# mourisl/T1K

Hardware: AMD Instinct MI355X
Metric: genotyped reads/sec (end-to-end genotyper stage, 2x150 bp HLA) (higher is better)
Workload: dtype u64

## Files before the change

include/t1k_gpu.h:

```cpp
#ifndef T1K_GPU_H
#define T1K_GPU_H

#include <stddef.h>
#include <stdint.h>

#ifdef __cplusplus
extern "C" {
#endif

typedef enum {
  T1K_OK = 0,
  T1K_ERR_ARG = -1,
  T1K_ERR_DEVICE = -2,
  T1K_ERR_CAPACITY = -3,
  T1K_ERR_IO = -4,
  T1K_ERR_STATE = -5,
  T1K_ERR_INTERNAL = -6,
  T1K_ERR_COMMITTED = -7
} t1k_status;

typedef struct t1k_ctx t1k_ctx;
typedef struct t1k_job t1k_job;
typedef struct t1k_rowset t1k_rowset;
typedef struct t1k_comm t1k_comm;
// ... 108 lines not shown
const char *t1k_readset_last_error(const t1k_readset *rs);
void t1k_readset_destroy(t1k_readset *rs);
int t1k_coverage_selected(t1k_ctx *ctx, t1k_readset *rs, const uint8_t *selected, uint64_t *nRecords);
typedef struct t1k_xwin t1k_xwin;
int t1k_xwin_create(t1k_ctx *owner, uint64_t maxReadEnds, uint32_t maxWindows, t1k_xwin **out);
void t1k_xwin_destroy(t1k_xwin *x);
const char *t1k_xwin_last_error(const t1k_xwin *x);
int t1k_xwin_link(t1k_xwin *x, t1k_ctx *reader, uint32_t window, uint32_t *nExternal);
int t1k_xwin_resolve(t1k_xwin *x, t1k_ctx *ctx, uint32_t window);

int t1k_ref_share(t1k_ctx *dst, const t1k_ctx *src);
uint64_t t1k_pool_release(void);
void *t1k_pinned_alloc(uint64_t bytes);
void t1k_pinned_free(void *p);
int t1k_reads_share(t1k_ctx *dst, const t1k_ctx *src);
int t1k_reads_attach(t1k_ctx *dst, const t1k_ctx *src, int storeSlot, int resetStore);
int t1k_coverage_absorb(t1k_ctx *dst, t1k_ctx *src);

int t1k_extract_batch(t1k_ctx *ctx, uint32_t endsPerFragment, uint8_t *good, uint64_t *stats);

int t1k_align_count_batch(t1k_ctx *ctx, const char *text, const uint32_t *tOff, const char *pat, const uint32_t *pOff, const uint32_t *len, uint32_t nJobs,
                          int32_t *nMatch);
int t1k_gap_count_batch(t1k_ctx *ctx, const char *text, const uint32_t *tOff, const uint32_t *tLen, const char *pat, const uint32_t *pOff,
                        const uint32_t *pLen, uint32_t nJobs, int32_t *nMatch);
int t1k_align_batch(t1k_ctx *ctx, const char *text, const uint32_t *tOff, const uint32_t *tLen, const char *pat, const uint32_t *pOff,
                    const uint32_t *pLen, uint32_t nJobs, int32_t *score, int32_t *nMatch, int32_t *nMismatch, int32_t *nIndel, int8_t *ops,
                    const uint32_t *opsOff, uint32_t *nOps);

typedef void (*t1k_allreduce_fn)(void *dev_f64, uint64_t n, void *user);
int t1k_em_setup(t1k_ctx *ctx, const uint64_t *rowPtr, const uint32_t *ecIdx, const double *count, const int32_t *ecLen, uint32_t nGroups,
                 uint32_t nEc, t1k_allreduce_fn allreduce, void *user);
int t1k_em_update(t1k_ctx *ctx, const double *x0, double *x1, double *ecReadCount, double *diff);
void t1k_em_limits(uint32_t out[2]);

int t1k_barcode_em(t1k_ctx *ctx, uint32_t nBarcodes, const uint64_t *bcAllelePtr, const uint32_t *bcAllele, const uint64_t *bcGroupPtr,
                   const double *groupCount, const uint64_t *groupEntryPtr, const uint32_t *entryLocal, const double *rho, uint32_t nAlleles,
                   double alpha, double tol, int32_t maxIter, double *nOut, int32_t *itersOut, double *kernelMs);

typedef struct {
  uint64_t distinct;
  uint64_t keys;
  uint64_t corrected;
  uint64_t split;
  uint64_t no_umi;
  double kernel_ms;
} t1k_umi_stats;
int t1k_umi_collapse(t1k_ctx *ctx, uint32_t nFrag, const uint32_t *fragRow, const uint64_t *fragUmi, const uint64_t *listPtr, const uint32_t *listAllele,
                     uint32_t nRows, const uint32_t *alleleGene, uint32_t nAlleles, uint32_t nGenes, int32_t mismatch, uint32_t *fragMol, uint32_t *nMol,
                     uint32_t *molRow, uint32_t *molFrags, uint64_t *molListPtr, uint32_t *molList, double *frac, int32_t *uniq, t1k_umi_stats *stats);

typedef struct {
  uint32_t allele, seq_start;
  uint64_t read_at, ops_at;
  uint32_t n_ops, w_all, w_uniq, reserved;
} t1k_pileup_aln;
int t1k_pileup_begin(t1k_ctx *ctx, uint32_t nAlleles, const uint64_t *alleleOff );
int t1k_pileup_add(t1k_ctx *ctx, const t1k_pileup_aln *aln, uint32_t n, const char *text, uint64_t textBytes, const int8_t *ops, uint64_t opsBytes,
                   double *kernelMs);
int t1k_pileup_get(t1k_ctx *ctx, int32_t *counts );
int t1k_pileup_end(t1k_ctx *ctx);

int t1k_sitepile_begin(t1k_ctx *ctx, uint32_t nAlleles, const uint64_t *alleleOff , uint64_t nSites, const uint32_t *siteAllele, const uint32_t *sitePos,
                       uint64_t nBarcodes);
int t1k_sitepile_add(t1k_ctx *ctx, const t1k_pileup_aln *aln, uint32_t n, const uint64_t *bookPtr , const uint32_t *book, const char *text, uint64_t textBytes,
                     const int8_t *ops, uint64_t opsBytes, double *kernelMs);
int t1k_sitepile_get(t1k_ctx *ctx, uint64_t *keys, int32_t *counts, uint64_t cap, uint64_t *nRuns);
int t1k_sitepile_stats(t1k_ctx *ctx, uint64_t *keysEmitted, uint64_t *folds, double *foldMs);
int t1k_sitepile_end(t1k_ctx *ctx);

int t1k_phase_begin(t1k_ctx *ctx, uint32_t nAlleles, const uint64_t *alleleOff , uint64_t nSites, const uint32_t *siteAllele, const uint32_t *sitePos);
int t1k_phase_add(t1k_ctx *ctx, const t1k_pileup_aln *aln, uint32_t n, uint32_t nBook, const uint32_t *bookRec , const uint8_t *bookUniq ,
                  const char *text, uint64_t textBytes, const int8_t *ops, uint64_t opsBytes, double *kernelMs);
int t1k_phase_get(t1k_ctx *ctx, uint64_t *keys, int32_t *counts, uint64_t cap, uint64_t *nRuns);
int t1k_phase_stats(t1k_ctx *ctx, uint64_t *observations, uint64_t *bookings, uint64_t *keysEmitted, uint64_t *discordant, uint64_t *folds, double *foldMs);
int t1k_phase_end(t1k_ctx *ctx);

typedef struct { uint32_t read_len, clip_front, strand; } t1k_support_rec;
typedef struct { uint32_t flags, t_start, t_end; } t1k_support_book;
int t1k_support_begin(t1k_ctx *ctx, uint32_t nAlleles, const uint64_t *alleleOff , uint64_t nSites, const uint32_t *siteAllele, const uint32_t *sitePos);
int t1k_support_add(t1k_ctx *ctx, const t1k_pileup_aln *aln, uint32_t n, const t1k_support_rec *rec , const uint64_t *bookPtr ,
                    const t1k_support_book *book, const char *text, uint64_t textBytes, const int8_t *ops, uint64_t opsBytes, double *kernelMs);
int t1k_support_get(t1k_ctx *ctx, uint64_t *keys, int32_t *counts, uint64_t cap, uint64_t *nRuns);
int t1k_support_stats(t1k_ctx *ctx, uint64_t *keysEmitted, uint64_t *folds, double *foldMs);
int t1k_support_end(t1k_ctx *ctx);

int t1k_indel_begin(t1k_ctx *ctx, uint32_t nAlleles, const uint64_t *alleleOff , const char *alleleText );
int t1k_indel_add(t1k_ctx *ctx, const t1k_pileup_aln *aln, uint32_t n, const uint8_t *strand , const uint64_t *bookPtr , const uint8_t *bookUniq,
                  const char *text, uint64_t textBytes, const int8_t *ops, uint64_t opsBytes, double *kernelMs);
int t1k_indel_get(t1k_ctx *ctx, uint64_t *keys, int32_t *counts, uint64_t cap, uint64_t *nRuns);
int t1k_indel_stats(t1k_ctx *ctx, uint64_t *events, uint64_t *shifted, uint64_t *edgeDelBooked, uint64_t *edgeInsBooked, uint64_t *keysEmitted, uint64_t *folds, double *foldMs);
int t1k_indel_end(t1k_ctx *ctx);

int t1k_cigar_batch(t1k_ctx *ctx, const t1k_pileup_aln *aln, uint32_t n, const uint32_t *clip ,
                    const int8_t *ops, uint64_t opsBytes, uint32_t nAlleles, const uint64_t *alleleOff , const char *alleleText ,
                    uint64_t *cigarPtr , char *cigar, uint64_t cigarCap, uint64_t *mdPtr , char *md, uint64_t mdCap,
                    uint32_t *nm , uint32_t *refSpan , double *kernelMs );

int t1k_alt_batch(t1k_ctx *ctx, uint64_t nGroups, const uint64_t *groupPtr , const uint32_t *entryAllele, const uint64_t *q , uint32_t nAlleles,
                  const uint32_t *alleleGene , uint32_t nGenes, const uint32_t *slotOf , uint64_t *tables , double *kernelMs );
uint64_t t1k_alt_pieces(uint64_t nGroups, const uint64_t *groupPtr);

int t1k_diplo_batch(t1k_ctx *ctx, uint64_t nGroups, const uint64_t *groupPtr , const uint32_t *entryCand, const uint64_t *q , uint32_t nGenes,
                    const uint32_t *candPtr , uint64_t *matrix, double *kernelMs );
uint64_t t1k_diplo_pieces(uint64_t nGroups, const uint64_t *groupPtr);

typedef struct {
  uint64_t read_ends, lookups, postings, hits, groups, candidates, extended, near_best, dp_calls, rows, batches;
  double ms_seed, ms_chain, ms_extend, ms_select, ms_fullalign, ms_pair, ms_em, ms_total;
  uint64_t read_ends_total, pair_overlaps, dp_cells;
  double ms_load, ms_device, ms_coalesce, ms_write;
} t1k_stats;
int t1k_stats_get(t1k_ctx *ctx, t1k_stats *out);

enum { T1K_ROUTE_GENERAL_LANE = 0,
       T1K_ROUTE_WAVE_SMALL = 1,
       T1K_ROUTE_WAVE_LARGE = 2,
       T1K_ROUTE_BIG_BY_SIZE = 3,
       T1K_ROUTE_BIG_BY_SCRATCH = 4,
       T1K_ROUTE_KINDS = 5 };
typedef struct {
  uint64_t ranges, ranges_nw5, ranges_nw10, ranges_xlong;
  uint64_t groups, fast, slow, jobs, retry, finish, general, wave, genjobs, big, eq, band, wide, extjobs, extretry;
} t1k_route_totals;
typedef struct {
  uint32_t read_end, allele, n;
  uint8_t strand;
  uint8_t near_done, simple;
  uint8_t route;
  uint8_t nw, xlong, reserved[2];
} t1k_route_rec;
int t1k_route_report_enable(t1k_ctx *ctx, int on);
int t1k_route_report_get(t1k_ctx *ctx, t1k_route_totals *totals , t1k_route_rec *recs , uint64_t cap, uint64_t *nRecs);

#define T1K_SEED_MASK_WORDS 10
typedef struct {
  uint32_t read_off, list_len;
  uint8_t strand, reserved[3];
} t1k_seed_used;
int t1k_seed_report_enable(t1k_ctx *ctx, int on);
int t1k_seed_report_get(t1k_ctx *ctx, uint8_t *seen, uint32_t *counts, uint32_t *masks, t1k_seed_used *used, uint64_t cap, uint64_t *nUsed);

enum { T1K_REF_BASES = 0, T1K_REF_NMASK, T1K_REF_EXON, T1K_REF_POSTED, T1K_REF_BASES_T, T1K_REF_BLOCK_T, T1K_REF_ALLELE_OFF, T1K_REF_ALLELE_LEN,
       T1K_REF_ALLELE_HAS_N, T1K_REF_SEP_START, T1K_REF_SEP_POS, T1K_REF_K_START, T1K_REF_K_HAS, T1K_REF_K_MULTI, T1K_REF_K_HAS_PRE,
       T1K_REF_K_DIR_IDX, T1K_REF_K_DIR, T1K_REF_K_DIR_MASK, T1K_REF_K_POST, T1K_REF_K_POST_ALLELE, T1K_REF_ARRAYS };
typedef struct {
  uint32_t n_alleles, k;
  uint64_t total_bases, n_words, n_postings, bases_t_len, n_sep;
  uint32_t dir_rows, dir_stride, dir_mask_words, has_bases_t;
  uint64_t len[T1K_REF_ARRAYS];
  uint32_t elem_bytes[T1K_REF_ARRAYS];
} t1k_ref_geometry;
int t1k_ref_view_geometry(t1k_ctx *ctx, t1k_ref_geometry *out);
int t1k_ref_view_copy(t1k_ctx *ctx, int array, uint64_t first, uint64_t count, void *out);

double t1k_alloc_ms(t1k_ctx *ctx, uint64_t *bytes);
uint64_t t1k_ctx_mem_report(t1k_ctx *ctx, const char *tag, int print);

int t1k_genotyper_main(int argc, char **argv);
int t1k_extractor_main(int argc, char **argv);
int t1k_bam_extractor_main(int argc, char **argv);
int t1k_analyzer_main(int argc, char **argv);

typedef struct {
  t1k_params dev;
  double filter_frac, filter_cov, cross_gene_rate, squarem_min_alpha;
  int32_t allele_digit_units;
  char allele_delimiter;
  int32_t threads;
  int32_t device;
  int32_t output_read_assignment;
  int32_t batch_fragments;
  int32_t alternatives;
  int32_t diplotypes;
  int32_t diplo_candidates;
} t1k_job_params;
void t1k_job_params_default(t1k_job_params *p);

int t1k_job_create(const t1k_job_params *p, const char *refFasta, t1k_job **out);
void t1k_job_destroy(t1k_job *job);
const char *t1k_job_last_error(const t1k_job *job);
int t1k_job_load_reads(t1k_job *job, const char *file1, const char *file2, const char *barcodeFile);
int t1k_job_load_reads_multi(t1k_job *job, const char *const *files1, uint32_t n1, const char *const *files2, uint32_t n2, const char *barcodeFile);
typedef struct t1k_reads t1k_reads;
int t1k_reads_open(const char *const *files1, uint32_t n1, const char *const *files2, uint32_t n2, const char *barcodeFile, int threads, t1k_reads **out);
int t1k_reads_open_stream(const char *const *files1, uint32_t n1, const char *const *files2, uint32_t n2, const char *barcodeFile, int threads, t1k_reads **out);
const char *t1k_reads_last_error(const t1k_reads *reads);
int t1k_reads_fragments(const t1k_reads *reads, uint64_t *nFragments);
void t1k_reads_close(t1k_reads *reads);
int t1k_job_attach_reads(t1k_job *job, t1k_reads *reads);
int t1k_job_set_reads(t1k_job *job, const char *seq1, const uint64_t *off1, const char *seq2, const uint64_t *off2, uint32_t nFragments);
int t1k_job_run(t1k_job *job);
int t1k_job_set_output_prefix(t1k_job *job, const char *prefix);
int t1k_job_write_outputs(t1k_job *job, const char *prefix);
int t1k_job_genotype_text(t1k_job *job, char *buf, uint64_t cap, uint64_t *needed);
int t1k_job_alternatives_text(t1k_job *job, char *buf, uint64_t cap, uint64_t *needed);
int t1k_job_diplotypes_text(t1k_job *job, char *buf, uint64_t cap, uint64_t *needed);
int t1k_job_allele_table(t1k_job *job, int32_t *gene, double *abundance, uint32_t *nAlleles);
int t1k_job_counts(t1k_job *job, uint64_t *fragments, uint64_t *assignedFragments, uint64_t *groups, uint64_t *ecs, int32_t *emIterations);
int t1k_job_stats(t1k_job *job, t1k_stats *out);
t1k_ctx *t1k_job_ctx(t1k_job *job);
int t1k_job_set_shard(t1k_job *job, int rank, int nRanks, t1k_comm *comm);
int t1k_job_share_reads(t1k_job *dst, t1k_job *src);
int t1k_job_run_local(t1k_job *job);
int t1k_job_finish(t1k_job *job);
int t1k_job_groups_serialize(t1k_job *job, void *buf, uint64_t cap, uint64_t *needed);
int t1k_job_groups_merge(t1k_job *job, const void *const *bufs, const uint64_t *lens, uint32_t n);
int t1k_job_coalesce_rows(t1k_job *job, const t1k_row_entry *rows, const uint32_t *rowCounts, const uint32_t *fragments, uint32_t nFragments);
int t1k_coverage_device(t1k_ctx *ctx, void **devPtr, uint64_t *count);

typedef struct {
  int32_t allele_idx;
  int32_t has_mate_pair, o1_from_r2;
  t1k_overlap o1, o2;
  uint64_t ops1, ops2;
  uint32_t n_ops1, n_ops2;
} t1k_frag_assignment;
int t1k_fragment_details(const t1k_overlap *l1, uint32_t n1, const t1k_overlap *l2, uint32_t n2, int paired, const int32_t *alleles, uint32_t nAlleles,
                         t1k_frag_assignment *out);
typedef struct {
  int32_t allele_idx, ref_pos, exon_pos;
  char ref, var;
  int32_t qual, group, output_group;
  double var_support, all_support, var_uniq_support;
} t1k_variant;
typedef struct t1k_variants t1k_variants;
int t1k_variants_call(t1k_job *job, const double *abundance, int32_t var_max_group, uint32_t nFragments, const uint64_t *asgPtr, const t1k_frag_assignment *asg,
                      const int8_t *ops, const char *const *read1, const uint32_t *len1, const char *const *read2, const uint32_t *len2, t1k_variants **out);
uint32_t t1k_variants_count(const t1k_variants *v);
int t1k_variants_get(const t1k_variants *v, t1k_variant *out );
int t1k_variants_vcf(const t1k_variants *v, char *buf, uint64_t cap, uint64_t *needed);
int t1k_variants_adjust(const t1k_variants *v, const t1k_frag_assignment *asg, uint32_t n, const int8_t *ops, const char *read1, uint32_t len1, const char *read2, uint32_t len2,
                        uint8_t *keep);
void t1k_variants_destroy(t1k_variants *v);

#ifdef __cplusplus
}
#endif
#endif
```

t1k_amd/capi.py:

```python
import ctypes as C
import gzip
import os

import numpy as np

_HERE = os.path.dirname(os.path.abspath(__file__))


def lib_path():
    return os.environ.get("T1K_GPU_LIB") or os.path.join(_HERE, "lib", "libt1k_gpu.so")


class T1kError(RuntimeError):
    pass


class Params(C.Structure):
    _fields_ = [("kmer_length", C.c_int32), ("radius", C.c_int32), ("hit_len_required", C.c_int32),
                ("ref_seq_similarity", C.c_double), ("relax_intron_align", C.c_int32), ("max_assign_cnt", C.c_int32),
                ("max_read_len", C.c_int32), ("workgroups", C.c_int32), ("group_cap", C.c_int64),
                ("cand_cap", C.c_int64), ("ovl_cap", C.c_int64), ("row_cap", C.c_int64), ("n_base_code", C.c_int32), ("store_chunk_mb", C.c_int32)]


class JobParams(C.Structure):
    _fields_ = [("dev", Params), ("filter_frac", C.c_double), ("filter_cov", C.c_double),
                ("cross_gene_rate", C.c_double), ("squarem_min_alpha", C.c_double), ("allele_digit_units", C.c_int32),
                ("allele_delimiter", C.c_char), ("threads", C.c_int32), ("device", C.c_int32),
                ("output_read_assignment", C.c_int32), ("batch_fragments", C.c_int32), ("alternatives", C.c_int32),
                ("diplotypes", C.c_int32), ("diplo_candidates", C.c_int32)]


class Stats(C.Structure):
    _fields_ = [(n, C.c_uint64) for n in ("read_ends", "lookups", "postings", "hits", "groups", "candidates", "extended",
                                          "near_best", "dp_calls", "rows", "batches")] + \
               [(n, C.c_double) for n in ("ms_seed", "ms_chain", "ms_extend", "ms_select", "ms_fullalign", "ms_pair", "ms_em", "ms_total")] + \
               [(n, C.c_uint64) for n in ("read_ends_total", "pair_overlaps", "dp_cells")] + \
               [(n, C.c_double) for n in ("ms_load", "ms_device", "ms_coalesce", "ms_write")]

    def as_dict(self):
        return {n: getattr(self, n) for n, _ in self._fields_}


class UmiStats(C.Structure):
    _fields_ = [(n, C.c_uint64) for n in ("distinct", "keys", "corrected", "split", "no_umi")] + [("kernel_ms", C.c_double)]


OVERLAP_DTYPE = np.dtype([("seq_idx", "<i4"), ("read_start", "<i4"), ("read_end", "<i4"), ("seq_start", "<i4"),
                          ("seq_end", "<i4"), ("strand", "<i4"), ("match_cnt", "<i4"), ("left_clip", "<i4"),
                          ("right_clip", "<i4"), ("relaxed_match_cnt", "<i4"), ("similarity", "<f8")])
ROW_DTYPE = np.dtype([("allele_idx", "<i4"), ("start", "<i4"), ("end", "<i4"), ("weight", "<f4"), ("qual", "<f4"),
                      ("adjust_weight", "<f4")])
GROUP_DTYPE = np.dtype([("allele", "<i4"), ("start", "<i4"), ("end", "<i4"), ("weight", "<f4"), ("adjust_weight", "<f4")])
assert OVERLAP_DTYPE.itemsize == 48 and ROW_DTYPE.itemsize == 24 and GROUP_DTYPE.itemsize == 20
FRAG_ASG_DTYPE = np.dtype([("allele_idx", "<i4"), ("has_mate_pair", "<i4"), ("o1_from_r2", "<i4"), ("_pad", "<i4"), ("o1", OVERLAP_DTYPE), ("o2", OVERLAP_DTYPE),
                           ("ops1", "<u8"), ("ops2", "<u8"), ("n_ops1", "<u4"), ("n_ops2", "<u4")])
VARIANT_DTYPE = np.dtype([("allele_idx", "<i4"), ("ref_pos", "<i4"), ("exon_pos", "<i4"), ("ref", "S1"), ("var", "S1"), ("_pad", "S2"), ("qual", "<i4"), ("group", "<i4"),
                          ("output_group", "<i4"), ("_pad2", "<i4"), ("var_support", "<f8"), ("all_support", "<f8"), ("var_uniq_support", "<f8")])
assert FRAG_ASG_DTYPE.itemsize == 136 and VARIANT_DTYPE.itemsize == 56

PILEUP_ALN_DTYPE = np.dtype([("allele", "<u4"), ("seq_start", "<u4"), ("read_at", "<u8"), ("ops_at", "<u8"), ("n_ops", "<u4"), ("w_all", "<u4"), ("w_uniq", "<u4"),
                             ("reserved", "<u4")])
PHASE_NO_MATE = 0xFFFFFFFF
PHASE_STATES = ("A", "C", "G", "T", "N", "-")
PILEUP_COUNTERS = ("A", "C", "G", "T", "N", "del", "ins", "A_uniq", "C_uniq", "G_uniq", "T_uniq", "N_uniq", "del_uniq", "ins_uniq")
assert PILEUP_ALN_DTYPE.itemsize == 40
SUPPORT_REC_DTYPE = np.dtype([("read_len", "<u4"), ("clip_front", "<u4"), ("strand", "<u4")])
SUPPORT_BOOK_DTYPE = np.dtype([("flags", "<u4"), ("t_start", "<u4"), ("t_end", "<u4")])
SUPPORT_STATES = ("A", "C", "G", "T", "N", "-", "+")
SUPPORT_FAMILY_B = 1 << 57
assert SUPPORT_REC_DTYPE.itemsize == 12 and SUPPORT_BOOK_DTYPE.itemsize == 12
ROUTE_TOTALS = ("ranges", "ranges_nw5", "ranges_nw10", "ranges_xlong", "groups", "fast", "slow", "jobs", "retry", "finish", "general", "wave", "genjobs", "big",
                "eq", "band", "wide", "extjobs", "extretry")
ROUTE_REC_DTYPE = np.dtype([("read_end", "<u4"), ("allele", "<u4"), ("n", "<u4"), ("strand", "u1"), ("near_done", "u1"), ("simple", "u1"), ("route", "u1"),
                            ("nw", "u1"), ("xlong", "u1"), ("reserved", "u1", (2,))])
ROUTE_NAMES = ("general_lane", "wave_small", "wave_large", "big_by_size", "big_by_scratch")
assert ROUTE_REC_DTYPE.itemsize == 20
SEED_USED_DTYPE = np.dtype([("read_off", "<u4"), ("list_len", "<u4"), ("strand", "u1"), ("reserved", "u1", (3,))])
SEED_MASK_WORDS = 10
assert SEED_USED_DTYPE.itemsize == 12
POSTING_DTYPE = np.dtype([("allele", "<u4"), ("offset", "<u4")])
REF_ARRAYS = (("bases", "<u8"), ("nmask", "<u8"), ("exon", "<u8"), ("posted", "<u8"), ("basesT", "<u8"), ("blockT", "<u4"), ("alleleOff", "<u8"), ("alleleLen", "<u4"),
              ("alleleHasN", "u1"), ("sepStart", "<u4"), ("sepPos", "<i4"), ("kStart", "<u4"), ("kHas", "<u4"), ("kMulti", "<u4"), ("kHasPre", "<u4"), ("kDirIdx", "<u4"),
              ("kDir", "<u4"), ("kDirMask", "<u8"), ("kPost", POSTING_DTYPE), ("kPostAllele", "<u4"))


class RefGeometry(C.Structure):
    _fields_ = [("n_alleles", C.c_uint32), ("k", C.c_uint32), ("total_bases", C.c_uint64), ("n_words", C.c_uint64), ("n_postings", C.c_uint64),
                ("bases_t_len", C.c_uint64), ("n_sep", C.c_uint64), ("dir_rows", C.c_uint32), ("dir_stride", C.c_uint32), ("dir_mask_words", C.c_uint32),
                ("has_bases_t", C.c_uint32), ("len", C.c_uint64 * len(REF_ARRAYS)), ("elem_bytes", C.c_uint32 * len(REF_ARRAYS))]


CIGAR_FILL = 0xAB
ALT_FILL = 0xCD
ALT_EMPTY = 0xFFFFFFFF
DIPLO_FILL = 0xD1

ALLREDUCE_FN = C.CFUNCTYPE(None, C.c_void_p, C.c_uint64, C.c_void_p)

_lib = None


def lib():
    global _lib
    if _lib is not None:
        return _lib
    p = lib_path()
    if not os.path.exists(p):
        raise T1kError("%s not found: run `python -c 'import __graft_entry__ as g; g.build()'` first" % p)
    L = C.CDLL(p)
    vp, u64p, u32p, u8p, i32p = C.c_void_p, C.POINTER(C.c_uint64), C.POINTER(C.c_uint32), C.POINTER(C.c_uint8), C.POINTER(C.c_int32)
    L.t1k_params_default.argtypes = [C.POINTER(Params)]
    L.t1k_ctx_create.argtypes = [C.c_int, C.POINTER(Params), C.POINTER(vp)]
    L.t1k_ctx_destroy.argtypes = [vp]
    L.t1k_last_error.argtypes = [vp]
    L.t1k_last_error.restype = C.c_char_p
    L.t1k_device_count.restype = C.c_int
    L.t1k_ref_upload.argtypes = [vp, C.c_char_p, vp, vp, C.c_uint32]
    L.t1k_reads_upload.argtypes = [vp, C.c_char_p, vp, vp, C.c_uint32]
    L.t1k_assign_batch.argtypes = [vp]
    L.t1k_assign_range.argtypes = [vp, C.c_uint64, C.c_uint32]
    L.t1k_overlaps_download.argtypes = [vp, vp, vp, C.c_uint64, u64p]
    L.t1k_pair_batch.argtypes = [vp, vp, vp, vp, C.c_uint32]
    L.t1k_rows_download.argtypes = [vp, vp, vp, vp, C.c_uint64, u64p]
    L.t1k_coverage_get.argtypes = [vp, vp, C.c_uint64]
    L.t1k_coverage_reset.argtypes = [vp]
    L.t1k_missing_coverage.argtypes = [vp, vp]
    L.t1k_coverage_absorb.argtypes = [vp, vp]
    L.t1k_align_batch.argtypes = [vp, C.c_char_p, vp, vp, C.c_char_p, vp, vp, C.c_uint32, vp, vp, vp, vp, vp, vp, vp]
    L.t1k_align_count_batch.argtypes = [vp, C.c_char_p, vp, C.c_char_p, vp, vp, C.c_uint32, vp]
    L.t1k_gap_count_batch.argtypes = [vp, C.c_char_p, vp, vp, C.c_char_p, vp, vp, C.c_uint32, vp]
    L.t1k_em_setup.argtypes = [vp, vp, vp, vp, vp, C.c_uint32, C.c_uint32, ALLREDUCE_FN, vp]
    L.t1k_em_update.argtypes = [vp, vp, vp, vp, vp]
    L.t1k_em_shard.argtypes = [vp, C.c_uint32, C.c_uint32, vp]
    L.t1k_em_limits.argtypes = [vp]
    L.t1k_em_limits.restype = None
    L.t1k_barcode_em.argtypes = [vp, C.c_uint32, vp, vp, vp, vp, vp, vp, vp, C.c_uint32, C.c_double, C.c_double, C.c_int32, vp, vp, C.POINTER(C.c_double)]
    L.t1k_umi_collapse.argtypes = [vp, C.c_uint32, vp, vp, vp, vp, C.c_uint32, vp, C.c_uint32, C.c_uint32, C.c_int32, vp, C.POINTER(C.c_uint32), vp, vp, vp, vp, vp, vp,
                                   C.POINTER(UmiStats)]
    L.t1k_pileup_begin.argtypes = [vp, C.c_uint32, vp]
    L.t1k_pileup_add.argtypes = [vp, vp, C.c_uint32, vp, C.c_uint64, vp, C.c_uint64, C.POINTER(C.c_double)]
    L.t1k_pileup_get.argtypes = [vp, vp]
    L.t1k_pileup_end.argtypes = [vp]
    L.t1k_sitepile_begin.argtypes = [vp, C.c_uint32, vp, C.c_uint64, vp, vp, C.c_uint64]
    L.t1k_sitepile_add.argtypes = [vp, vp, C.c_uint32, vp, vp, vp, C.c_uint64, vp, C.c_uint64, C.POINTER(C.c_double)]
    L.t1k_sitepile_get.argtypes = [vp, vp, vp, C.c_uint64, u64p]
    L.t1k_sitepile_stats.argtypes = [vp, u64p, u64p, C.POINTER(C.c_double)]
    L.t1k_sitepile_end.argtypes = [vp]
    L.t1k_support_begin.argtypes = [vp, C.c_uint32, vp, C.c_uint64, vp, vp]
    L.t1k_support_add.argtypes = [vp, vp, C.c_uint32, vp, vp, vp, vp, C.c_uint64, vp, C.c_uint64, C.POINTER(C.c_double)]
    L.t1k_support_get.argtypes = [vp, vp, vp, C.c_uint64, u64p]
    L.t1k_support_stats.argtypes = [vp, u64p, u64p, C.POINTER(C.c_double)]
    L.t1k_support_end.argtypes = [vp]
    L.t1k_indel_begin.argtypes = [vp, C.c_uint32, vp, vp]
    L.t1k_indel_add.argtypes = [vp, vp, C.c_uint32, vp, vp, vp, vp, C.c_uint64, vp, C.c_uint64, C.POINTER(C.c_double)]
    L.t1k_indel_get.argtypes = [vp, vp, vp, C.c_uint64, u64p]
    L.t1k_indel_stats.argtypes = [vp, u64p, u64p, u64p, u64p, u64p, u64p, C.POINTER(C.c_double)]
    L.t1k_indel_end.argtypes = [vp]
    L.t1k_phase_begin.argtypes = [vp, C.c_uint32, vp, C.c_uint64, vp, vp]
    L.t1k_phase_add.argtypes = [vp, vp, C.c_uint32, C.c_uint32, vp, vp, vp, C.c_uint64, vp, C.c_uint64, C.POINTER(C.c_double)]
    L.t1k_phase_get.argtypes = [vp, vp, vp, C.c_uint64, u64p]
    L.t1k_phase_stats.argtypes = [vp, u64p, u64p, u64p, u64p, u64p, C.POINTER(C.c_double)]
    L.t1k_phase_end.argtypes = [vp]
    L.t1k_cigar_batch.argtypes = [vp, vp, C.c_uint32, vp, vp, C.c_uint64, C.c_uint32, vp, vp, vp, vp, C.c_uint64, vp, vp, C.c_uint64, vp, vp, C.POINTER(C.c_double)]
    L.t1k_alt_batch.argtypes = [vp, C.c_uint64, vp, vp, vp, C.c_uint32, vp, C.c_uint32, vp, vp, C.POINTER(C.c_double)]
    L.t1k_ctx_mem_report.argtypes = [vp, C.c_char_p, C.c_int]
    L.t1k_ctx_mem_report.restype = C.c_uint64
    L.t1k_alt_pieces.argtypes = [C.c_uint64, vp]
    L.t1k_alt_pieces.restype = C.c_uint64
    L.t1k_job_alternatives_text.argtypes = [vp, C.c_char_p, C.c_uint64, u64p]
    L.t1k_diplo_batch.argtypes = [vp, C.c_uint64, vp, vp, vp, C.c_uint32, vp, vp, C.POINTER(C.c_double)]
    L.t1k_diplo_pieces.argtypes = [C.c_uint64, vp]
    L.t1k_diplo_pieces.restype = C.c_uint64
    L.t1k_job_diplotypes_text.argtypes = [vp, C.c_char_p, C.c_uint64, u64p]
    L.t1k_job_allele_table.argtypes = [vp, vp, vp, u32p]
    L.t1k_extract_batch.argtypes = [vp, C.c_uint32, vp, vp]
    L.t1k_extractor_main.argtypes = [C.c_int, C.POINTER(C.c_char_p)]
    L.t1k_stats_get.argtypes = [vp, C.POINTER(Stats)]
    L.t1k_route_report_enable.argtypes = [vp, C.c_int]
    L.t1k_route_report_get.argtypes = [vp, vp, vp, C.c_uint64, u64p]
    L.t1k_seed_report_enable.argtypes = [vp, C.c_int]
    L.t1k_seed_report_get.argtypes = [vp, vp, vp, vp, vp, C.c_uint64, u64p]
    L.t1k_ref_view_geometry.argtypes = [vp, vp]
    L.t1k_ref_view_copy.argtypes = [vp, C.c_int, C.c_uint64, C.c_uint64, vp]
    L.t1k_genotyper_main.argtypes = [C.c_int, C.POINTER(C.c_char_p)]
    L.t1k_job_params_default.argtypes = [C.POINTER(JobParams)]
    L.t1k_job_create.argtypes = [C.POINTER(JobParams), C.c_char_p, C.POINTER(vp)]
    L.t1k_job_destroy.argtypes = [vp]
    L.t1k_job_last_error.argtypes = [vp]
    L.t1k_job_last_error.restype = C.c_char_p
    L.t1k_job_load_reads.argtypes = [vp, C.c_char_p, C.c_char_p, C.c_char_p]
    L.t1k_job_set_reads.argtypes = [vp, C.c_char_p, vp, C.c_char_p, vp, C.c_uint32]
    L.t1k_job_run.argtypes = [vp]
    L.t1k_job_write_outputs.argtypes = [vp, C.c_char_p]
    L.t1k_pool_release.restype = C.c_uint64
    L.t1k_pool_release.argtypes = []
    L.t1k_job_load_reads_multi.argtypes = [vp, C.POINTER(C.c_char_p), C.c_uint32, C.POINTER(C.c_char_p), C.c_uint32, C.c_char_p]
    L.t1k_reads_open.argtypes = [C.POINTER(C.c_char_p), C.c_uint32, C.POINTER(C.c_char_p), C.c_uint32, C.c_char_p, C.c_int, C.POINTER(vp)]
    L.t1k_reads_open_stream.argtypes = [C.POINTER(C.c_char_p), C.c_uint32, C.POINTER(C.c_char_p), C.c_uint32, C.c_char_p, C.c_int, C.POINTER(vp)]
    L.t1k_reads_last_error.argtypes = [vp]
    L.t1k_reads_last_error.restype = C.c_char_p
    L.t1k_reads_fragments.argtypes = [vp, u64p]
    L.t1k_reads_close.argtypes = [vp]
    L.t1k_reads_close.restype = None
    L.t1k_job_attach_reads.argtypes = [vp, vp]
    L.t1k_job_genotype_text.argtypes = [vp, C.c_char_p, C.c_uint64, u64p]
    L.t1k_job_counts.argtypes = [vp, u64p, u64p, u64p, u64p, i32p]
    L.t1k_job_stats.argtypes = [vp, C.POINTER(Stats)]
    L.t1k_job_ctx.argtypes = [vp]
    L.t1k_job_ctx.restype = vp
    L.t1k_job_run_local.argtypes = [vp]
    L.t1k_job_finish.argtypes = [vp]
    L.t1k_job_groups_serialize.argtypes = [vp, vp, C.c_uint64, u64p]
    L.t1k_reads_dedupe.argtypes = [vp, vp, u32p]
    L.t1k_job_groups_merge.argtypes = [vp, vp, vp, C.c_uint32]
    L.t1k_job_coalesce_rows.argtypes = [vp, vp, vp, vp, C.c_uint32]
    L.t1k_variants_call.argtypes = [vp, vp, C.c_int32, C.c_uint32, vp, vp, vp, vp, vp, vp, vp, C.POINTER(vp)]
    L.t1k_fragment_details.argtypes = [vp, C.c_uint32, vp, C.c_uint32, C.c_int, vp, C.c_uint32, vp]
    L.t1k_variants_count.argtypes = [vp]
    L.t1k_variants_count.restype = C.c_uint32
    L.t1k_variants_get.argtypes = [vp, vp]
    L.t1k_variants_vcf.argtypes = [vp, vp, C.c_uint64, u64p]
    L.t1k_variants_adjust.argtypes = [vp, vp, C.c_uint32, vp, C.c_char_p, C.c_uint32, C.c_char_p, C.c_uint32, vp]
    L.t1k_variants_destroy.argtypes = [vp]
    L.t1k_job_set_shard.argtypes = [vp, C.c_int, C.c_int, vp]
    L.t1k_job_share_reads.argtypes = [vp, vp]
    L.t1k_job_ctx.restype = vp
    L.t1k_job_ctx.argtypes = [vp]
    L.t1k_comm_unique_id.argtypes = [vp]
    L.t1k_comm_init.argtypes = [vp, C.c_int, C.c_int, vp, vp, C.c_int, C.POINTER(vp)]
    L.t1k_comm_bind.argtypes = [vp, vp]
    L.t1k_comm_destroy.argtypes = [vp]
    L.t1k_comm_last_error.restype = C.c_char_p
    L.t1k_comm_last_error.argtypes = [vp]
    L.t1k_comm_is_rccl.argtypes = [vp]
    L.t1k_comm_group_create.restype = vp
    L.t1k_comm_group_create.argtypes = [C.c_int]
    L.t1k_comm_group_destroy.argtypes = [vp]
    L.t1k_coverage_device.argtypes = [vp, C.POINTER(vp), u64p]
    L.t1k_device_memory.argtypes = [C.c_int, u64p, u64p]
    L.t1k_ctx_set_coverage_mode.argtypes = [vp, C.c_int]
    L.t1k_readset_detach.argtypes = [vp, C.POINTER(vp)]
    L.t1k_readset_take_store.argtypes = [vp, vp, C.c_int]
    L.t1k_readset_bytes.argtypes = [vp]
    L.t1k_readset_bytes.restype = C.c_uint64
    L.t1k_readset_size.argtypes = [vp]
    L.t1k_readset_size.restype = C.c_uint32
    L.t1k_readset_destroy.argtypes = [vp]
    L.t1k_coverage_selected.argtypes = [vp, vp, vp, u64p]
    L.t1k_overlaps_upload.argtypes = [vp, vp, vp]
    L.t1k_pair_limits.argtypes = [vp]
    L.t1k_pair_limits.restype = None
    L.t1k_pair_direct_cap.argtypes = []
    L.t1k_pair_direct_cap.restype = C.c_uint32
    L.t1k_rowset_create.argtypes = [vp, C.c_uint64, vp, C.POINTER(vp)]
    L.t1k_rowset_destroy.argtypes = [vp]
    L.t1k_rowset_destroy.restype = None
    L.t1k_rowset_set_raw.argtypes = [vp, C.c_int]
    L.t1k_rowset_last_error.argtypes = [vp]
    L.t1k_rowset_last_error.restype = C.c_char_p
    L.t1k_pair_into.argtypes = [vp, vp, vp, vp, vp, C.c_uint32, C.c_uint64]
    L.t1k_rowset_rows_download.argtypes = [vp, C.c_uint64, C.c_uint32, vp, vp, C.c_uint64, u64p]
    L.t1k_rowset_assigned_range.argtypes = [vp, C.c_uint64, C.c_uint64, vp]
    L.t1k_rowset_coalesce.argtypes = [vp, u64p, u64p, u64p]
    L.t1k_rowset_groups_download.argtypes = [vp, vp, vp, vp]
    L.t1k_rowset_device_bytes.argtypes = [vp, u64p, u64p]
    L.t1k_coalesce_limits.argtypes = [vp]
    L.t1k_coalesce_limits.restype = None
    L.t1k_rowset_exchange.argtypes = [vp, vp, C.c_uint64]
    L.t1k_rowset_groups_gather.argtypes = [vp, vp, u64p, u64p, u64p]
    L.t1k_rowset_groups_download_all.argtypes = [vp, vp, vp, vp]
    L.t1k_comm_abort.argtypes = [vp]
    L.t1k_ref_share.argtypes = [vp, vp]
    L.t1k_reads_share.argtypes = [vp, vp]
    L.t1k_xwin_create.argtypes = [vp, C.c_uint64, C.c_uint32, C.POINTER(vp)]
    L.t1k_xwin_destroy.argtypes = [vp]
    L.t1k_xwin_destroy.restype = None
    L.t1k_xwin_last_error.argtypes = [vp]
    L.t1k_xwin_last_error.restype = C.c_char_p
    L.t1k_xwin_link.argtypes = [vp, vp, C.c_uint32, u32p]
    L.t1k_xwin_resolve.argtypes = [vp, vp, C.c_uint32]
    _lib = L
    return L


def _ptr(a):
    return a.ctypes.data_as(C.c_void_p) if a is not None else None


def _u8(text):
    return np.frombuffer(text, np.uint8) if isinstance(text, (bytes, bytearray)) else np.ascontiguousarray(text, np.uint8)


def _pieces(cuts, n):
    edges = [0] + [int(c) for c in cuts] + [int(n)]
    return zip(edges[:-1], edges[1:])


def _concat(seqs):
    offs = np.zeros(len(seqs) + 1, dtype=np.uint64)
    if len(seqs):
        offs[1:] = np.cumsum([len(s) for s in seqs], dtype=np.uint64)
    blob = "".join(seqs).encode("ascii")
    return blob, offs


class Context:

    def __init__(self, device=0, **kw):
        L = lib()
        p = Params()
        L.t1k_params_default(C.byref(p))
        for k, v in kw.items():
            setattr(p, k, v)
        self.params = p
        h = C.c_void_p()
        rc = L.t1k_ctx_create(device, C.byref(p), C.byref(h))
        if rc != 0:
            raise T1kError("t1k_ctx_create failed (%d): no usable GPU / bad parameters" % rc)
        self.h = h
        self.n_read_ends = 0
        self.allele_len = None

    def _check(self, rc, what):
        if rc != 0:
            raise T1kError("%s failed (%d): %s" % (what, rc, lib().t1k_last_error(self.h).decode()))

    def close(self):
        if self.h:
            lib().t1k_ctx_destroy(self.h)
            self.h = None

    def __del__(self):
        try:
            self.close()
        except Exception:
            pass

    def ref_upload(self, seqs, exon_masks=None):
        blob, offs = _concat(seqs)
        ex = None
        if exon_masks is not None:
            ex = np.concatenate([np.asarray(m, dtype=np.uint8) for m in exon_masks]) if len(seqs) else np.zeros(0, np.uint8)
        self.allele_len = np.array([len(s) for s in seqs], dtype=np.int64)
        self._check(lib().t1k_ref_upload(self.h, blob, _ptr(offs), _ptr(ex), len(seqs)), "t1k_ref_upload")

    def ref_share(self, src):
        self.allele_len = src.allele_len
        self._check(lib().t1k_ref_share(self.h, src.h), "t1k_ref_share")

    def reads_share(self, src):
        self.n_read_ends = src.n_read_ends
        self._check(lib().t1k_reads_share(self.h, src.h), "t1k_reads_share")

    def reads_upload(self, seqs, weights=None):
        blob, offs = _concat(seqs)
        w = None if weights is None else np.asarray(weights, dtype=np.uint32)
        self.n_read_ends = len(seqs)
        self._check(lib().t1k_reads_upload(self.h, blob, _ptr(offs), _ptr(w), len(seqs)), "t1k_reads_upload")

    def reads_dedupe(self):
        out = np.zeros(self.n_read_ends, dtype=np.uint32)
        nd = C.c_uint32()
        self._check(lib().t1k_reads_dedupe(self.h, _ptr(out), C.byref(nd)), "t1k_reads_dedupe")
        self.n_uploaded, self.n_read_ends = self.n_read_ends, nd.value
        return out

    def assign(self):
        self._check(lib().t1k_assign_batch(self.h), "t1k_assign_batch")

    def extract(self, ends_per_fragment=1):
        good = np.zeros(self.n_read_ends // ends_per_fragment, dtype=np.uint8)
        st = np.zeros(8, dtype=np.uint64)
        self._check(lib().t1k_extract_batch(self.h, ends_per_fragment, _ptr(good), _ptr(st)), "t1k_extract_batch")
        return good, dict(zip(("read_ends", "lookups", "postings", "read_ends_with_hits", "read_ends_chained", "screen_ns", "main_ns", "big_shape"), (int(x) for x in st)))

    def overlaps(self):
        n = self.n_read_ends
        counts = np.zeros(n, dtype=np.uint32)
        tot = C.c_uint64()
        self._check(lib().t1k_overlaps_download(self.h, _ptr(counts), None, 0, C.byref(tot)), "t1k_overlaps_download")
        out = np.zeros(tot.value, dtype=OVERLAP_DTYPE)
        self._check(lib().t1k_overlaps_download(self.h, _ptr(counts), _ptr(out), tot.value, C.byref(tot)), "t1k_overlaps_download")
        return counts, out

    def overlaps_upload(self, counts, ovl):
        c = np.ascontiguousarray(counts, dtype=np.uint32)
        o = np.ascontiguousarray(ovl, dtype=OVERLAP_DTYPE)
        assert len(c) == self.n_read_ends and int(c.sum()) == len(o)
        self._check(lib().t1k_overlaps_upload(self.h, _ptr(c), _ptr(o)), "t1k_overlaps_upload")

    def pair(self, end1, end2, has_n):
        e1 = np.asarray(end1, dtype=np.uint32)
        e2 = None if end2 is None else np.asarray(end2, dtype=np.uint32)
        hn = np.asarray(has_n, dtype=np.uint8)
        self.n_fragments = len(e1)
        self._check(lib().t1k_pair_batch(self.h, _ptr(e1), _ptr(e2), _ptr(hn), len(e1)), "t1k_pair_batch")

    def rows(self):
        n = self.n_fragments
        counts = np.zeros(n, dtype=np.uint32)
        assigned = np.zeros(n, dtype=np.uint8)
        tot = C.c_uint64()
        self._check(lib().t1k_rows_download(self.h, _ptr(counts), _ptr(assigned), None, 0, C.byref(tot)), "t1k_rows_download")
        out = np.zeros(tot.value, dtype=ROW_DTYPE)
        self._check(lib().t1k_rows_download(self.h, _ptr(counts), _ptr(assigned), _ptr(out), tot.value, C.byref(tot)), "t1k_rows_download")
        return counts, assigned, out

    def coverage(self):
        tot = int(self.allele_len.sum())
        out = np.zeros(tot, dtype=np.int32)
        self._check(lib().t1k_coverage_get(self.h, _ptr(out), tot), "t1k_coverage_get")
        return out

    def set_coverage_mode(self, deferred):
        self._check(lib().t1k_ctx_set_coverage_mode(self.h, 1 if deferred else 0), "t1k_ctx_set_coverage_mode")

    def detach_readset(self, slot=0):
        h = C.c_void_p()
        self._check(lib().t1k_readset_detach(self.h, C.byref(h)), "t1k_readset_detach")
        rs = Readset(h)
        self._check(lib().t1k_readset_take_store(rs.h, self.h, slot), "t1k_readset_take_store")
        return rs

    def coverage_selected(self, readset, selected):
        sel = np.ascontiguousarray(selected, dtype=np.uint8)
        n = C.c_uint64()
        self._check(lib().t1k_coverage_selected(self.h, readset.h, _ptr(sel), C.byref(n)), "t1k_coverage_selected")
        return n.value

    def coverage_reset(self):
        self._check(lib().t1k_coverage_reset(self.h), "t1k_coverage_reset")

    def missing_coverage(self):
        out = np.zeros(len(self.allele_len), dtype=np.int32)
        self._check(lib().t1k_missing_coverage(self.h, _ptr(out)), "t1k_missing_coverage")
        return out

    def stats(self):
        s = Stats()
        lib().t1k_stats_get(self.h, C.byref(s))
        return s.as_dict()

    def route_report_enable(self, on=True):
        self._check(lib().t1k_route_report_enable(self.h, 1 if on else 0), "t1k_route_report_enable")

    def route_report(self):
        n = C.c_uint64()
        self._check(lib().t1k_route_report_get(self.h, None, None, 0, C.byref(n)), "t1k_route_report_get")
        tot = np.zeros(len(ROUTE_TOTALS), np.uint64)
        recs = np.zeros(n.value, ROUTE_REC_DTYPE)
        self._check(lib().t1k_route_report_get(self.h, _ptr(tot), _ptr(recs), n.value, C.byref(n)), "t1k_route_report_get")
        return dict(zip(ROUTE_TOTALS, (int(x) for x in tot))), recs

    def assign_range(self, first, count):
        self._check(lib().t1k_assign_range(self.h, first, count), "t1k_assign_range")

    def seed_report_enable(self, on=True):
        self._check(lib().t1k_seed_report_enable(self.h, 1 if on else 0), "t1k_seed_report_enable")

    def seed_report(self):
        n = self.n_read_ends
        tot = C.c_uint64()
        self._check(lib().t1k_seed_report_get(self.h, None, None, None, None, 0, C.byref(tot)), "t1k_seed_report_get")
        seen = np.zeros(n, np.uint8)
        counts = np.zeros((n, 2), np.uint32)
        masks = np.zeros((n, 2, SEED_MASK_WORDS), np.uint32)
        used = np.zeros(tot.value, SEED_USED_DTYPE)
        self._check(lib().t1k_seed_report_get(self.h, _ptr(seen), _ptr(counts), _ptr(masks), _ptr(used), tot.value, C.byref(tot)), "t1k_seed_report_get")
        ptr = np.zeros(n + 1, np.int64)
        np.cumsum(counts.sum(axis=1, dtype=np.int64), out=ptr[1:])
        assert int(ptr[-1]) == len(used)
        return seen, counts, masks, ptr, used

    def ref_geometry(self):
        g = RefGeometry()
        self._check(lib().t1k_ref_view_geometry(self.h, C.byref(g)), "t1k_ref_view_geometry")
        out = {f: int(getattr(g, f)) for f, _ in RefGeometry._fields_[:11]}
        out["len"] = {name: int(g.len[i]) for i, (name, _) in enumerate(REF_ARRAYS)}
        assert all(g.elem_bytes[i] == np.dtype(t).itemsize for i, (_, t) in enumerate(REF_ARRAYS))
        return out

    def ref_array(self, name, first=0, count=None):
        i = [n for n, _ in REF_ARRAYS].index(name)
        if count is None:
            count = self.ref_geometry()["len"][name] - first
        out = np.zeros(max(count, 0), REF_ARRAYS[i][1])
        self._check(lib().t1k_ref_view_copy(self.h, i, first, count, _ptr(out)), "t1k_ref_view_copy")
        return out

    def align_batch(self, texts, pats, want_ops=True):
        n = len(texts)
        tb, toff = _concat(texts)
        pb, poff = _concat(pats)
        tlen = np.array([len(t) for t in texts], dtype=np.uint32)
        plen = np.array([len(p) for p in pats], dtype=np.uint32)
        toff32, poff32 = toff[:-1].astype(np.uint32), poff[:-1].astype(np.uint32)
        score = np.zeros(n, np.int32); nm = np.zeros(n, np.int32); nx = np.zeros(n, np.int32); ni = np.zeros(n, np.int32)
        ops_off = np.zeros(n, np.uint32)
        if n:
            ops_off[1:] = np.cumsum((tlen + plen + 2)[:-1], dtype=np.uint64).astype(np.uint32)
        ops = np.zeros(int((tlen + plen + 2).sum()) + 8, np.int8)
        nops = np.zeros(n, np.uint32)
        self._check(lib().t1k_align_batch(self.h, tb, _ptr(toff32), _ptr(tlen), pb, _ptr(poff32), _ptr(plen), n, _ptr(score), _ptr(nm),
                                          _ptr(nx), _ptr(ni), _ptr(ops) if want_ops else None, _ptr(ops_off), _ptr(nops)), "t1k_align_batch")
        op_list = [ops[ops_off[i]:ops_off[i] + nops[i]].copy() for i in range(n)] if want_ops else None
        return score, nm, nx, ni, op_list

    def align_count_batch(self, texts, pats):
        n = len(texts)
        tb, toff = _concat(texts)
        pb, poff = _concat(pats)
        ln = np.array([len(t) for t in texts], dtype=np.uint32)
        out = np.zeros(n, np.int32)
        self._check(lib().t1k_align_count_batch(self.h, tb, _ptr(toff[:-1].astype(np.uint32)), pb, _ptr(poff[:-1].astype(np.uint32)), _ptr(ln), n,
                                                _ptr(out)), "t1k_align_count_batch")
        return out

    def gap_count_batch(self, texts, pats, lead=""):
        n = len(texts)
        tb, toff = _concat([lead] + list(texts))
        pb, poff = _concat(pats)
        tlen = np.array([len(t) for t in texts], dtype=np.uint32)
        plen = np.array([len(p) for p in pats], dtype=np.uint32)
        out = np.zeros(n, np.int32)
        self._check(lib().t1k_gap_count_batch(self.h, tb, _ptr(toff[1:-1].astype(np.uint32)), _ptr(tlen), pb, _ptr(poff[:-1].astype(np.uint32)), _ptr(plen), n,
                                              _ptr(out)), "t1k_gap_count_batch")
        return out

    def em_setup(self, row_ptr, ec_idx, count, ec_len, allreduce=None, raw=False):
        self._em_keep = (np.ascontiguousarray(row_ptr, np.uint64), np.ascontiguousarray(ec_idx, np.uint32), np.ascontiguousarray(count, np.float64),
                         np.ascontiguousarray(ec_len, np.int32))
        rp, ei, ct, el = self._em_keep
        assert len(rp) == len(ct) + 1 and int(rp[-1]) == len(ei)
        self._em_cb = ALLREDUCE_FN(allreduce) if allreduce else C.cast(None, ALLREDUCE_FN)
        self._em_nec = len(el)
        rc = lib().t1k_em_setup(self.h, _ptr(rp), _ptr(ei), _ptr(ct), _ptr(el), len(ct), len(el), self._em_cb, None)
        if raw:
            return rc
        self._check(rc, "t1k_em_setup")

    def em_shard(self, row_begin, row_end, comm=None, raw=False):
        rc = lib().t1k_em_shard(self.h, row_begin, row_end, comm.h if comm is not None else None)
        if raw:
            return rc
        self._check(rc, "t1k_em_shard")

    def last_error(self):
        return lib().t1k_last_error(self.h).decode()

    def em_update(self, x0):
        x0 = np.ascontiguousarray(x0, dtype=np.float64)
        x1 = np.zeros(self._em_nec, np.float64)
        n = np.zeros(self._em_nec, np.float64)
        diff = C.c_double()
        self._check(lib().t1k_em_update(self.h, _ptr(x0), _ptr(x1), _ptr(n), C.byref(diff)), "t1k_em_update")
        return x1, n, diff.value

    def barcode_em(self, bc_allele_ptr, bc_allele, bc_group_ptr, group_count, group_entry_ptr, entry_local, rho, n_alleles, alpha=0.0, tol=1e-7,
                   max_iter=1000, raw=False):
        ap = np.ascontiguousarray(bc_allele_ptr, np.uint64)
        al = np.ascontiguousarray(bc_allele, np.uint32)
        gp = np.ascontiguousarray(bc_group_ptr, np.uint64)
        gc = np.ascontiguousarray(group_count, np.float64)
        ep = np.ascontiguousarray(group_entry_ptr, np.uint64)
        el = np.ascontiguousarray(entry_local, np.uint32)
        rh = None if rho is None else np.ascontiguousarray(rho, np.float64)
        nb = max(len(ap) - 1, 0)
        n = np.zeros(len(al), np.float64)
        iters = np.zeros(nb, np.int32)
        ms = C.c_double()
        rc = lib().t1k_barcode_em(self.h, nb, _ptr(ap), _ptr(al), _ptr(gp), _ptr(gc), _ptr(ep), _ptr(el), _ptr(rh), n_alleles, alpha, tol, max_iter,
                                  _ptr(n), _ptr(iters), C.byref(ms))
        if raw:
            return rc
        self._check(rc, "t1k_barcode_em")
        return n, iters, ms.value

    def umi_collapse(self, frag_row, frag_umi, list_ptr, list_allele, n_rows, allele_gene, n_genes, mismatch=1, raw=False):
        fr = np.ascontiguousarray(frag_row, np.uint32)
        fu = np.ascontiguousarray(frag_umi, np.uint64)
        lp = np.ascontiguousarray(list_ptr, np.uint64)
        la = np.ascontiguousarray(list_allele, np.uint32)
        ag = np.ascontiguousarray(allele_gene, np.uint32)
        nf, na = len(fr), len(ag)
        if len(fu) != nf or len(lp) != nf + 1:
            raise ValueError("umi_collapse: frag_row, frag_umi and list_ptr do not describe the same fragments")
        ne = int(lp[-1]) - int(lp[0]) if nf and int(lp[-1]) >= int(lp[0]) else 0
        ne = min(ne, len(la))
        frag_mol = np.zeros(nf, np.uint32)
        mol_row = np.zeros(nf, np.uint32)
        mol_frags = np.zeros(nf, np.uint32)
        mol_ptr = np.zeros(nf + 1, np.uint64)
        mol_list = np.zeros(max(ne, 1), np.uint32)
        frac = np.zeros((int(n_rows), na), np.float64)
        uniq = np.zeros((int(n_rows), na), np.int32)
        n_mol = C.c_uint32()
        st = UmiStats()
        rc = lib().t1k_umi_collapse(self.h, nf, _ptr(fr), _ptr(fu), _ptr(lp), _ptr(la), int(n_rows), _ptr(ag), na, int(n_genes), int(mismatch), _ptr(frag_mol), C.byref(n_mol),
                                    _ptr(mol_row), _ptr(mol_frags), _ptr(mol_ptr), _ptr(mol_list), _ptr(frac), _ptr(uniq), C.byref(st))
        if raw:
            return rc
        self._check(rc, "t1k_umi_collapse")
        m = n_mol.value
        mol_row, mol_frags, mol_ptr = mol_row[:m], mol_frags[:m], mol_ptr[:m + 1].astype(np.int64)
        first = np.full(m, nf, np.int64)
        np.minimum.at(first, frag_mol, np.arange(nf))
        order = np.lexsort((first, mol_row))
        rank = np.empty(m, np.uint32)
        rank[order] = np.arange(m, dtype=np.uint32)
        lens = np.diff(mol_ptr)[order]
        new_ptr = np.concatenate([[0], np.cumsum(lens)]).astype(np.uint64)
        take = np.repeat(mol_ptr[:-1][order] - new_ptr[:-1].astype(np.int64), lens) + np.arange(int(lens.sum()))
        return dict(frag_mol=rank[frag_mol], mol_row=mol_row[order], mol_frags=mol_frags[order], mol_list_ptr=new_ptr, mol_list=mol_list[take] if m else mol_list[:0],
                    frac=frac, uniq=uniq,
                    stats=dict(distinct=int(st.distinct), keys=int(st.keys), corrected=int(st.corrected), split=int(st.split), no_umi=int(st.no_umi), kernel_ms=float(st.kernel_ms)))

    def pileup_begin(self, allele_off, raw=False):
        off = np.ascontiguousarray(allele_off, np.uint64)
        rc = lib().t1k_pileup_begin(self.h, max(len(off) - 1, 0), _ptr(off))
        if rc == 0:
            self._pileup_total = int(off[-1])
        if raw:
            return rc
        self._check(rc, "t1k_pileup_begin")

    def pileup_add(self, aln, text, ops, raw=False):
        a = np.ascontiguousarray(aln, PILEUP_ALN_DTYPE)
        t, o = _u8(text), np.ascontiguousarray(ops, np.int8)
        ms = C.c_double()
        rc = lib().t1k_pileup_add(self.h, _ptr(a), len(a), _ptr(t), len(t), _ptr(o), len(o), C.byref(ms))
        if raw:
            return rc
        self._check(rc, "t1k_pileup_add")
        return ms.value

    def pileup_get(self):
        counts = np.zeros((14, getattr(self, "_pileup_total", 0)), np.int32)
        self._check(lib().t1k_pileup_get(self.h, _ptr(counts)), "t1k_pileup_get")
        return counts

    def pileup_end(self, raw=False):
        rc = lib().t1k_pileup_end(self.h)
# ... 778 lines not shown
```

t1k_amd/csrc/t1k_assign.hip:

```cpp
#include "t1k_dev.h"
#include "t1k_launch.h"
#include "t1k_memo.h"
#include "t1k_select_rule.h"

#define WG 256
#define GA_BIG_MAX 2048
#define GA_SCRATCH_INTS (6 * (GA_BIG_MAX + 4))


__global__ void k_pack_reads(const char *ascii, const uint64_t *offs, uint32_t n, int S, uint64_t *bases, uint64_t *nmask, uint16_t *lens, int nCode) {
  uint64_t gid = (uint64_t)blockIdx.x * blockDim.x + threadIdx.x;
  uint64_t total = (uint64_t)n * S;
  if (gid >= total) return;
  uint32_t re = (uint32_t)(gid / S);
  int w = (int)(gid % S);
  uint64_t o = offs[re];
  int len = (int)(offs[re + 1] - o);
  if (w == 0) lens[re] = (uint16_t)len;
  uint64_t fb = 0, fn = 0, rb = 0, rn = 0;
  for (int q = 0; q < 32; ++q) {
    int i = w * 32 + q;
    if (i >= len) break;
    char c = ascii[o + i];
    int code = c == 'A' ? 0 : c == 'C' ? 1 : c == 'G' ? 2 : c == 'T' ? 3 : 4;
    if (code == 4) { fn |= 1ull << (2 * q); fb |= (uint64_t)nCode << (2 * q); } else fb |= (uint64_t)code << (2 * q);
    char d = ascii[o + len - 1 - i];
    int dc = d == 'A' ? 3 : d == 'C' ? 2 : d == 'G' ? 1 : d == 'T' ? 0 : 4;
    if (dc == 4) { rn |= 1ull << (2 * q); rb |= (uint64_t)nCode << (2 * q); } else rb |= (uint64_t)dc << (2 * q);
  }
  uint64_t base = (uint64_t)re * 2 * S;
  bases[base + w] = fb; nmask[base + w] = fn;
  bases[base + S + w] = rb; nmask[base + S + w] = rn;
}


__device__ __forceinline__ bool sepInRange(const T1kRefDev &ref, uint32_t allele, int s, int e) {
  int len = (int)ref.alleleLen[allele];
  if (s <= -1 && e >= -1) return true;
  if (s <= len && e >= len) return true;
  uint32_t b = ref.sepStart[allele], en = ref.sepStart[allele + 1];
  for (uint32_t i = b; i < en; ++i) {
    int p = ref.sepPos[i];
    if (p >= s && p <= e) return true;
  }
  return false;
}


template <bool DEFER>
__device__ __forceinline__ bool extendOne(const ExtendArgs &P, uint64_t gid, unsigned int &extendDp) {
  T1kCand c = P.cand[gid];
  T1kExt x{};
  const uint32_t allele = c.allele & 0x7FFFFFFFu;
  const int pass = (c.allele >> 31) ? 0 : 1;
  const int S = P.reads.S;
  const uint64_t *rb = P.reads.bases + ((uint64_t)c.re * 2 + pass) * S;
  const uint64_t *rn = P.reads.nmask + ((uint64_t)c.re * 2 + pass) * S;
  const int len = P.reads.len[c.re];
  const int rs = (int)(c.readSE & 0xFFFF), re = (int)(c.readSE >> 16);
  const int ss = c.seqStart, se = c.seqEnd;
  const int matchCnt = (int)(c.match >> 16);
  uint16_t flags = 0;
  if (sepInRange(P.ref, allele, ss, se)) flags |= T1K_F_SEPSEED;
  if (sepInRange(P.ref, allele, ss - rs, se + (len - re - 1))) flags |= T1K_F_NEEDCLIP;
  if (flags & T1K_F_SEPSEED) { x.flags = flags; P.ext[gid] = x; return true; }
  const int alleleLen = (int)P.ref.alleleLen[allele];
  const int64_t goff = (int64_t)P.ref.alleleOff[allele];
  int lo = rs < ss ? rs : ss;
  int leftClip = rs > ss ? rs - ss : 0, rightClip = 0;
  {
    uint32_t b = P.ref.sepStart[allele], en = P.ref.sepStart[allele + 1];
    int bestP = -1;
    for (uint32_t i = b; i < en; ++i) {
      int p = P.ref.sepPos[i];
      if (p < ss && p >= ss - lo && p > bestP) bestP = p;
    }
    if (bestP >= 0) { int i = ss - 1 - bestP; leftClip = lo - i; lo = i; }
  }
  unsigned int dpLocal = 0;
  const ReadCtx rc{rb, rn, len, P.ref.bases, P.ref.nmask, goff, alleleLen, P.ref.anyN != 0};
  const GapSink sink{P.memo + (uint64_t)c.re * GAP_CACHE, P.jobStr, P.counters, c.re * GAP_CACHE, P.jobSegCap, T1K_AR_EXTJOBS};
  uint32_t slot = 0;
  bool pending = false;
  int match = gapMatchesCached<DEFER>(rc, rs - lo, goff + ss - lo, lo, lo, pass, sink, &dpLocal, &slot);
  if (match < 0) { pending = true; match = 0; }
  int ro = (len - 1 - re) < (alleleLen - 1 - se) ? (len - 1 - re) : (alleleLen - 1 - se);
  if (len - 1 - re > alleleLen - 1 - se) rightClip = len - 1 - re - (alleleLen - 1 - se);
  {
    uint32_t b = P.ref.sepStart[allele], en = P.ref.sepStart[allele + 1];
    int bestP = 0x7FFFFFFF;
    for (uint32_t i = b; i < en; ++i) {
      int p = P.ref.sepPos[i];
      if (p > se && p <= se + ro && p < bestP) bestP = p;
    }
    if (bestP != 0x7FFFFFFF) { int i = bestP - se - 1; rightClip = ro - i; ro = i; }
  }
  {
    const int mr = gapMatchesCached<DEFER>(rc, re + 1, goff + se + 1, ro, ro, pass, sink, &dpLocal, &slot);
    if (mr < 0) pending = true; else match += mr;
  }
  extendDp = dpLocal;
  if (pending) return false;
  int eMatch = 2 * match + matchCnt;
  int ers = rs - lo, ere = re + ro, ess = ss - lo, ese = se + ro;
  double esim = (double)eMatch / (double)(ere - ers + 1 + ese - ess + 1);
  if (!(esim < P.sim)) flags |= T1K_F_EXTOK;
  if (leftClip > 0 || rightClip > 0) eMatch += 2 * leftClip + 2 * rightClip;
  x.seqStart = ess; x.seqEnd = ese; x.readStart = (uint16_t)ers; x.readEnd = (uint16_t)ere;
  x.matchCnt = (uint16_t)eMatch; x.leftClip = (uint16_t)leftClip; x.rightClip = (uint16_t)rightClip; x.flags = flags;
  P.ext[gid] = x;
  return true;
}

#if T1K_EXTEND_WAVES > 0
#define T1K_EXTEND_ATTR T1K_WAVES_ATTR_(T1K_EXTEND_WAVES)
#else
#define T1K_EXTEND_ATTR
#endif
__global__ __launch_bounds__(WG) T1K_EXTEND_ATTR void k_extend(ExtendArgs P) {
  const uint64_t gid = (uint64_t)blockIdx.x * blockDim.x + threadIdx.x;
  unsigned int dp = 0;
  bool done = true;
  if (gid < P.nCand) done = extendOne<true>(P, gid, dp);
  if (!done) {
    const uint32_t q = t1k_arena_append(P.counters, T1K_AR_EXTRETRY, P.retrySegCap);
    if (q != T1K_ARENA_FULL) P.retryStr[q] = (uint32_t)gid;
  }
  t1k_stat_add(P.counters, T1K_STAT_EXTEND_DP, dp);
}

__global__ __launch_bounds__(WG) void k_extend_retry(ExtendArgs P, const uint32_t *list, uint32_t nItems, const unsigned long long *nDev) {
  if (nDev) nItems = (uint32_t)*nDev;
  unsigned int dp = 0;
  for (uint32_t q = blockIdx.x * blockDim.x + threadIdx.x; q < nItems; q += gridDim.x * blockDim.x) {
    unsigned int d1 = 0;
    extendOne<false>(P, list[q], d1);
    dp += d1;
  }
  t1k_stat_add(P.counters, T1K_STAT_EXTEND_DP, dp);
}


__device__ __forceinline__ uint64_t shflXor64(uint64_t v, int laneMask) {
  const int lo = __shfl_xor((int)(uint32_t)v, laneMask, 64), hi = __shfl_xor((int)(uint32_t)(v >> 32), laneMask, 64);
  return ((uint64_t)(uint32_t)hi << 32) | (uint32_t)lo;
}
__device__ inline void bitonicSortSimple(uint64_t *key, uint32_t np2) {
  __syncthreads();
  for (uint32_t size = 2; size <= np2; size <<= 1) {
    for (uint32_t stride = size >> 1; stride > 0; stride >>= 1) {
      for (uint32_t t = threadIdx.x; t < np2 / 2; t += blockDim.x) {
        uint32_t lo = 2 * t - (t & (stride - 1));
        uint32_t hi = lo + stride;
        bool up = (lo & size) == 0;
        uint64_t a = key[lo], b = key[hi];
        bool sw = up ? (a > b) : (a < b);
        if (sw) { key[lo] = b; key[hi] = a; }
      }
      __syncthreads();
    }
  }
}
__device__ inline void bitonicSort(uint64_t *key, uint32_t np2) {
  constexpr int E = 8;
  if (np2 < E || np2 > blockDim.x * E) { bitonicSortSimple(key, np2); return; }
  const uint32_t t = threadIdx.x;
  const bool act = t * E < np2;
  uint64_t a[E];
  __syncthreads();
  if (act) {
#pragma unroll
    for (int e = 0; e < E; ++e) a[e] = key[t * E + e];
  }
  for (uint32_t size = 2; size <= np2; size <<= 1) {
    for (uint32_t stride = size >> 1; stride > 0; stride >>= 1) {
      if (stride >= 64 * E) {
        if (act) {
#pragma unroll
          for (int e = 0; e < E; ++e) key[t * E + e] = a[e];
        }
        __syncthreads();
        if (act) {
          const uint32_t pt = t ^ (stride / E);
#pragma unroll
          for (int e = 0; e < E; ++e) {
            const uint32_t i = t * E + e;
            const uint64_t b = key[pt * E + e];
            const bool up = (i & size) == 0, lower = (i & stride) == 0;
            const bool keepMin = up == lower;
            a[e] = keepMin ? (a[e] < b ? a[e] : b) : (a[e] > b ? a[e] : b);
          }
        }
        __syncthreads();
      } else if (stride >= E) {
        if (act) {
          const int lm = (int)(stride / E);
#pragma unroll
          for (int e = 0; e < E; ++e) {
            const uint32_t i = t * E + e;
            const uint64_t b = shflXor64(a[e], lm);
            const bool up = (i & size) == 0, lower = (i & stride) == 0;
            const bool keepMin = up == lower;
            a[e] = keepMin ? (a[e] < b ? a[e] : b) : (a[e] > b ? a[e] : b);
          }
        }
      } else if (act) {
#pragma unroll
        for (int s = E / 2; s > 0; s >>= 1) {
          if (stride == (uint32_t)s) {
#pragma unroll
            for (int e = 0; e < E; ++e) {
              if ((e & s) == 0) {
                const uint32_t i = t * E + e;
                const bool up = (i & size) == 0;
                const uint64_t x = a[e], y = a[e + s];
                const bool sw = up ? (x > y) : (x < y);
                a[e] = sw ? y : x; a[e + s] = sw ? x : y;
              }
            }
          }
        }
      }
    }
  }
  if (act) {
#pragma unroll
    for (int e = 0; e < E; ++e) key[t * E + e] = a[e];
  }
  __syncthreads();
}
#define CS_SLOTS 512
struct CsTables {
  uint32_t hKey[CS_SLOTS];
  uint8_t hRank[CS_SLOTS];
  uint32_t dList[256];
  uint32_t nDistinct, overflow;
};
__device__ __forceinline__ uint32_t csHash(uint32_t c) { return (c * 2654435761u) >> 23; }
__device__ __forceinline__ uint32_t csRankOf(const CsTables &T, uint32_t cls) {
  const uint32_t want = cls + 1;
  uint32_t h = csHash(cls);
  while (T.hKey[h] != want) h = (h + 1) & (CS_SLOTS - 1);
  return T.hRank[h];
}
template <int NT>
__device__ inline bool ldsClassRanks(const uint64_t *key, uint32_t n, int classShift, CsTables &T) {
  const int tid = threadIdx.x;
  for (int q = tid; q < CS_SLOTS; q += NT) T.hKey[q] = 0;
  if (tid == 0) { T.nDistinct = 0; T.overflow = 0; }
// ... 380 lines not shown
        const uint64_t kk = key[i];
        const bool emit = selEmit((uint32_t)kk & 7u, seedOf(kk), good);
        if (emit) { ++mine; const int xm = (int)P.ext[c0 + i].matchCnt; if (xm > myBest) myBest = xm; }
        key[i] = (kk & ~7ull) | (emit ? SEL_M_EMIT : 0u);
      }
    }
    atomicMax(&sBest, myBest);
    uint32_t tot;
    t1k_block_scan_exclusive_n<NT / 64>(mine, warpSums, &tot);
    auto makeOvl = [&](uint32_t ci, int bestMatch) {
      const T1kCand c = P.cand[ci];
      const T1kExt x = P.ext[ci];
      T1kOvl o;
      o.allele = c.allele & 0x7FFFFFFFu;
      o.seqStart = x.seqStart; o.seqEnd = x.seqEnd; o.readStart = x.readStart; o.readEnd = x.readEnd;
      o.matchCnt = x.matchCnt; o.leftClip = x.leftClip; o.rightClip = x.rightClip; o.re = re;
      o.flags = ((int)x.matchCnt >= bestMatch - 10 ? 1u : 0u) | ((c.allele >> 31) ? 0u : 2u);
      o.relaxed = (!P.relax && (o.flags & 1)) ? x.matchCnt : (uint16_t)0;
      return o;
    };
    auto storePacked = [&](uint64_t at, const T1kOvl &o) {
      T1kOvlP p;
      if (!t1k_ovl_pack(o, p)) atomicOr(&P.counters[T1K_CTR_ERR], (unsigned long long)ERR_PACK);
      P.store[at] = p;
    };
    uint32_t keep = tot;
    const bool cutList = CUT && tot > SELECT_CUT_LEN;
    T1K_SELECT_ROUTE_COUNT();
    if (CUT && !cutList) orderBySelect(false);
    if (cutList) {
      __syncthreads();
      const int bestMatch = sBest;
      const uint32_t nWords = (n + 63) / 64;
      uint64_t *emitBits = (uint64_t *)sCnt;
      uint32_t *wordBase = (uint32_t *)(emitBits + nWords);
      for (uint32_t i0 = 0; i0 < n; i0 += NT) {
        const uint32_t i = i0 + tid;
        const uint64_t bal = __ballot(i < n && marked(key[i]));
        if ((tid & 63) == 0 && i < n) emitBits[i >> 6] = bal;
      }
      __syncthreads();
      {
        uint32_t t2;
        const uint32_t ex = t1k_block_scan_exclusive_n<NT / 64>((uint32_t)tid < nWords ? (uint32_t)__popcll(emitBits[tid]) : 0u, warpSums, &t2);
        if ((uint32_t)tid < nWords) wordBase[tid] = ex;
      }
      __syncthreads();
      const KeyW TW = truncWidths<XL>((int)P.reads.len[re]);
      for (uint32_t i = tid; i < n; i += NT) {
        if (!((emitBits[i >> 6] >> (i & 63)) & 1ull)) continue;
        const T1kExt x = P.ext[c0 + i];
        const int rspan = x.readEnd - x.readStart;
        const int d = rspan + 1 + x.seqEnd - x.seqStart + 1 + 2 * x.leftClip + 2 * x.rightClip;
        uint64_t kk;
        if (!packSortKey(TW, (int)x.matchCnt, d, rspan, P.cand[c0 + i].allele & 0x7FFFFFFFu, i, P.alleleBits, iBits, &kk)) { atomicOr(&P.counters[T1K_CTR_ERR], (unsigned long long)ERR_SORTCAP); kk = i; }
        if ((int)x.matchCnt >= bestMatch - 10) ++nbLocal;
        key[selBitPos(emitBits, wordBase, i)] = kk;
      }
      uint32_t np2t = 8;
      while (np2t < tot) np2t <<= 1;
      for (uint32_t i = tot + tid; i < np2t; i += NT) key[i] = ~0ull;
      __syncthreads();
      if (key != sKey || !ldsClassRanks<NT>(key, tot, P.alleleBits + iBits, sCs)) bitonicSort(key, np2t);
      else ldsCountingPass<NT>(key, tot, sCnt, warpSums, [&](uint64_t kk) { return csRankOf(sCs, (uint32_t)(kk >> (P.alleleBits + iBits))); });
      if (tid == 0) { sTie = 0; sLatch = (int)tot; }
      __syncthreads();
      for (uint32_t i = 1 + tid; i < tot; i += NT)
        if ((key[i] >> iBits) == (key[i - 1] >> iBits)) sTie = 1;
      __syncthreads();
      if (sTie && tid == 0) {
        auto before = [&](uint32_t ia, uint32_t ib) {
          const T1kExt xa = P.ext[c0 + ia], xb = P.ext[c0 + ib];
          if (xa.readStart != xb.readStart) return xa.readStart < xb.readStart;
          if (xa.readEnd != xb.readEnd) return xa.readEnd < xb.readEnd;
          if (xa.seqStart != xb.seqStart) return xa.seqStart < xb.seqStart;
          if (xa.seqEnd != xb.seqEnd) return xa.seqEnd < xb.seqEnd;
          const T1kCand a = P.cand[c0 + ia], b = P.cand[c0 + ib];
          const int ma = (int)(a.match >> 16), mb = (int)(b.match >> 16);
          if (ma != mb) return ma > mb;
          const int ra = (int)(a.readSE >> 16) - (int)(a.readSE & 0xFFFF), rb = (int)(b.readSE >> 16) - (int)(b.readSE & 0xFFFF);
          const int da = ra + 1 + a.seqEnd - a.seqStart + 1, db = rb + 1 + b.seqEnd - b.seqStart + 1;
          if (da != db) return da < db;
          if (ra != rb) return ra > rb;
          if (candBeforeFull(a, b)) return true;
          if (candBeforeFull(b, a)) return false;
          return ia < ib;
        };
        for (uint32_t i = 1; i < tot; ++i) {
          if ((key[i] >> iBits) != (key[i - 1] >> iBits)) continue;
          uint32_t j = i;
          while (j > 0 && (key[j - 1] >> iBits) == (key[j] >> iBits) && before((uint32_t)(key[j] & iMask), (uint32_t)(key[j - 1] & iMask))) {
            uint64_t t = key[j]; key[j] = key[j - 1]; key[j - 1] = t;
            --j;
          }
        }
      }
      __syncthreads();
      {
        const int tmMax = (1 << TW.MB) - 1, tdMax = (1 << TW.DB) - 1, dShift = TW.RB + P.alleleBits + iBits;
        auto simOf = [&](uint64_t kk) { return (double)(tmMax - (int)((kk >> (dShift + TW.DB)) & (uint64_t)tmMax)) / (double)(int)((kk >> dShift) & (uint64_t)tdMax); };
        const double s0 = simOf(key[0]);
        uint32_t first = tot;
        for (uint32_t j = 1 + tid; j < tot; j += NT)
          if (simOf(key[j]) < s0 - 0.1) { first = j; break; }
        if (first < tot) atomicMin(&sLatch, (int)first);
      }
      __syncthreads();
      keep = (uint32_t)sLatch;
    }
    if (tid == 0) {
      unsigned long long b = atomicAdd(&P.counters[T1K_CTR_OVL], (unsigned long long)keep);
      emitTotal += tot;
      if (b + keep > P.ovlCap) { atomicOr(&P.counters[T1K_CTR_ERR], (unsigned long long)ERR_OVLCAP); sBase = 0xFFFFFFFFu; publishEmpty(re); }
      else { sBase = (uint32_t)b; publish(re, (uint32_t)b, keep); }
    }
    __syncthreads();
    const int bestMatch = sBest;
    if (sBase != 0xFFFFFFFFu) {
      if (cutList) {
        for (uint32_t i = tid; i < keep; i += NT) storePacked((uint64_t)sBase + i, makeOvl(c0 + (uint32_t)(key[i] & iMask), bestMatch));
      } else {
        for (uint32_t i0 = 0; i0 < live; i0 += NT) {
          uint32_t i = i0 + tid;
          uint32_t flag = (i < live && marked(key[i])) ? 1u : 0u;
          uint32_t t2;
          uint32_t off = t1k_block_scan_exclusive_n<NT / 64>(flag, warpSums, &t2);
          if (flag) {
            const T1kOvl o = makeOvl(c0 + idxOf(key[i]), bestMatch);
            if (o.flags & 1) ++nbLocal;
            if (PK) storePacked((uint64_t)sBase + written + off, o);
            else P.ovl[(uint64_t)sBase + written + off] = o;
          }
          written += t2;
        }
      }
    }
    nbTotal += nbLocal;
    __syncthreads();
  }
  if (PK && tid == 0 && emitTotal) atomicAdd(&P.counters[T1K_CTR_EMITTED], emitTotal);
  t1k_stat_add(P.counters, T1K_STAT_NEARBEST, nbTotal);
}


__global__ __launch_bounds__(WG) void k_fullalign(FullArgs P) {
  uint64_t gid = (uint64_t)blockIdx.x * blockDim.x + threadIdx.x;
  if (gid >= P.nOvl) return;
  T1kOvl o = P.ovl[gid];
  if (!(o.flags & 1)) { P.ovl[gid].relaxed = 0; return; }
  const int pass = (o.flags & 2) ? 1 : 0;
  const int S = P.reads.S;
  const uint64_t *rb = P.reads.bases + ((uint64_t)o.re * 2 + pass) * S;
  const uint64_t *rn = P.reads.nmask + ((uint64_t)o.re * 2 + pass) * S;
  const int64_t goff = (int64_t)P.ref.alleleOff[o.allele];
  const int L = o.readEnd - o.readStart + 1, Ls = o.seqEnd - o.seqStart + 1;
  const int w = P.noCov ? 0 : (P.undo ? -(int)P.reads.weight[o.re] : (int)P.reads.weight[o.re]);
  bool slow = (L != Ls) || L > T1K_MAX_READ_LEN;
  int x = 0, exonMis = 0;
  uint64_t covw[10];
  if (!slow && L <= 160) {
    typedef uint64_t u64x2 __attribute__((ext_vector_type(2), aligned(8)));
    uint64_t gB[6], gN[6], rB[6], rN[6], gE[6];
    const int64_t gpos = goff + o.seqStart;
    const int64_t gw = gpos >> 5, rw = o.readStart >> 5;
    const int gsh = (int)(gpos & 31) * 2, rsh = (o.readStart & 31) * 2;
    const bool hasN = P.ref.alleleHasN[o.allele] != 0;
#pragma unroll
    for (int q = 0; q < 3; ++q) {
      const u64x2 a = *(const u64x2 *)(P.ref.bases + gw + 2 * q), b = *(const u64x2 *)(rb + rw + 2 * q), c = *(const u64x2 *)(rn + rw + 2 * q);
      gB[2 * q] = a.x; gB[2 * q + 1] = a.y; rB[2 * q] = b.x; rB[2 * q + 1] = b.y; rN[2 * q] = c.x; rN[2 * q + 1] = c.y;
      gN[2 * q] = 0; gN[2 * q + 1] = 0; gE[2 * q] = 0; gE[2 * q + 1] = 0;
    }
    if (hasN) {
#pragma unroll
      for (int q = 0; q < 3; ++q) { const u64x2 a = *(const u64x2 *)(P.ref.nmask + gw + 2 * q); gN[2 * q] = a.x; gN[2 * q + 1] = a.y; }
    }
    if (P.relax) {
#pragma unroll
      for (int q = 0; q < 3; ++q) { const u64x2 a = *(const u64x2 *)(P.ref.exon + gw + 2 * q); gE[2 * q] = a.x; gE[2 * q + 1] = a.y; }
    }
    auto piece = [](const uint64_t *W, int wi, int sh) { return (W[wi] >> sh) | ((W[wi + 1] << 1) << (63 - sh)); };
#pragma unroll
    for (int wi = 0; wi < 10; ++wi) {
      const int off = wi * 32;
      covw[wi] = 0;
      if (wi < 5 && off < L) {
        const uint64_t lm = t1k_lowmask(L - off);
        const uint64_t rnn = piece(rN, wi, rsh), gnn = piece(gN, wi, gsh);
        const uint64_t xo = piece(rB, wi, rsh) ^ piece(gB, wi, gsh);
        const uint64_t mm = (xo | (xo >> 1)) & T1K_EVEN & ~(rnn | gnn) & lm;
        x += __popcll(mm);
        if (P.relax) exonMis += __popcll(mm & piece(gE, wi, gsh));
        covw[wi] = T1K_EVEN & lm & ~mm & ~rnn & ~gnn;
      }
    }
    if (x > 3) slow = true;
  } else if (!slow) {
#pragma unroll
    for (int wi = 0; wi < 10; ++wi) {
      const int off = wi * 32;
      covw[wi] = 0;
      if (off < L) {
        const uint64_t lm = t1k_lowmask(L - off);
        const uint64_t rnn = t1k_get32(rn, o.readStart + off), gnn = t1k_get32(P.ref.nmask, goff + o.seqStart + off);
        const uint64_t xo = t1k_get32(rb, o.readStart + off) ^ t1k_get32(P.ref.bases, goff + o.seqStart + off);
        const uint64_t mm = (xo | (xo >> 1)) & T1K_EVEN & ~(rnn | gnn) & lm;
        x += __popcll(mm);
        if (P.relax) exonMis += __popcll(mm & t1k_get32(P.ref.exon, goff + o.seqStart + off));
        covw[wi] = T1K_EVEN & lm & ~mm & ~rnn & ~gnn;
      }
    }
    if (x > 3) slow = true;
  }
  if (slow) {
    if (P.undo) return;
    const int dl = L > Ls ? L - Ls : Ls - L;
    unsigned long long key = 0;
    if (dl <= 4) {
      uint64_t hsh = 0x9E3779B97F4A7C15ull;
      for (int off = 0; off < Ls; off += 32) {
        const uint64_t lm = t1k_lowmask(Ls - off);
        hsh = (hsh ^ (t1k_get32(P.ref.bases, goff + o.seqStart + off) & lm) ^ ((t1k_get32(P.ref.nmask, goff + o.seqStart + off) & lm) << 1)) * 0xD6E8FEB86659FD93ull;
        hsh ^= hsh >> 32;
      }
      key = ((unsigned long long)o.re << 44) | ((unsigned long long)pass << 43) | ((unsigned long long)o.readStart << 34) | ((unsigned long long)L << 25) |
            ((unsigned long long)(Ls - L + 4) << 21) | (hsh & 0x1FFFFFull);
    }
    if (L == Ls) {
      const uint32_t q = t1k_arena_append(P.counters, T1K_AR_EQ, P.segCap);
      if (q != T1K_ARENA_FULL) { P.eqStr[q] = (uint32_t)gid; P.eqKeyStr[q] = key; }
    } else if (dl <= 4) {
      const uint32_t q = t1k_arena_append(P.counters, T1K_AR_BAND, P.segCap);
      if (q != T1K_ARENA_FULL) { P.bandStr[q] = (uint32_t)gid; P.bandKeyStr[q] = key; }
    } else {
      const uint32_t q = t1k_arena_append(P.counters, T1K_AR_WIDE, P.segCap);
      if (q != T1K_ARENA_FULL) P.wideStr[q] = (uint32_t)gid;
    }
    return;
  }
  if (w) {
    int32_t *diff = P.ref.covDiff + goff + o.seqStart, *hole = diff + P.ref.covStride;
    if (L == P.fullLen) atomicAdd(&diff[2 * P.ref.covStride], w);
    else { atomicAdd(&diff[0], w); atomicAdd(&diff[L], -w); }
#pragma unroll
    for (int wi = 0; wi < 10; ++wi) {
      const int off = wi * 32;
      if (off < L) {
        uint64_t un = T1K_EVEN & t1k_lowmask(L - off) & ~covw[wi];
        while (un) {
          const int b = __ffsll((long long)un) - 1;
          un &= un - 1;
          atomicAdd(&hole[off + (b >> 1)], w);
        }
      }
    }
  }
  int relaxed = P.relax ? 2 * (L - exonMis) : (int)o.matchCnt;
  P.ovl[gid].relaxed = (uint16_t)relaxed;
}


__global__ __launch_bounds__(64) void k_fullalign_slow(SlowArgs P) {
  __shared__ int rows[GA_SCRATCH_INTS];
  if (threadIdx.x != 0) return;
  uint32_t t = blockIdx.x;
  uint32_t nThreads = gridDim.x;
  uint8_t *mine = P.scratch + (uint64_t)t * P.perThread;
  int8_t *ops = (int8_t *)(mine + GA_SCRATCH_INTS * 4);
  uint8_t *trace = mine + GA_SCRATCH_INTS * 4 + 4224;
  for (uint32_t q = t; q < P.nSlow; q += nThreads) {
    uint32_t gid = P.slowQueue[q];
    T1kOvl o = P.ovl[gid];
    const int pass = (o.flags & 2) ? 1 : 0;
    const int S = P.reads.S;
    const uint64_t *rb = P.reads.bases + ((uint64_t)o.re * 2 + pass) * S;
    const uint64_t *rn = P.reads.nmask + ((uint64_t)o.re * 2 + pass) * S;
    const int64_t goff = (int64_t)P.ref.alleleOff[o.allele];
    const int lp = o.readEnd - o.readStart + 1, lt = o.seqEnd - o.seqStart + 1;
    const int w = P.noCov ? 0 : (int)P.reads.weight[o.re];
    if ((lp + 1) * (lt + 1) > P.maxCells || lt > GA_BIG_MAX) { atomicOr(&P.counters[T1K_CTR_ERR], (unsigned long long)ERR_SLOWCAP); continue; }
    T1kSeqView T{P.ref.bases, P.ref.nmask, goff + o.seqStart}, Pv{rb, rn, (int64_t)o.readStart};
    t1k_ga_general(T, lt, Pv, lp, rows, trace, nullptr);
    int n = t1k_ga_traceback(trace, lt, lp, ops);
    int m = 0, refPos = o.seqStart, readPos = o.readStart;
    int32_t *cov = P.ref.covDiff + goff;
    for (int i = 0; i < n; ++i) {
      int op = ops[i];
      bool ex = refPos < (int)P.ref.alleleLen[o.allele] ? t1k_bit(P.ref.exon, goff + refPos) != 0 : false;
      if (P.relax) { if (ex) { if (op == 0) ++m; } else ++m; }
      if (op == 0 && w) {
        if (!t1k_bit(rn, readPos) && !t1k_bit(P.ref.nmask, goff + refPos)) { atomicAdd(&cov[refPos], w); atomicAdd(&cov[refPos + 1], -w); }
      }
      if (op != 2) ++refPos;
      if (op != 3) ++readPos;
    }
    P.ovl[gid].relaxed = (uint16_t)(P.relax ? 2 * m : (int)o.matchCnt);
  }
}

struct T1kWinBits {
  const uint64_t *p;
  int64_t off;
  int base;
  uint64_t w;
  __device__ T1kWinBits(const uint64_t *p_, int64_t off_) : p(p_), off(off_), base(1 << 30), w(0) {}
  __device__ __forceinline__ int bit(int pos) {
    if (pos < base || pos >= base + 32) { base = pos > 31 ? pos - 31 : 0; w = t1k_get32(p, off + base); }
    return (int)((w >> (2 * (pos - base))) & 1);
  }
};

struct T1kWinCodes {
  const uint64_t *p;
  int64_t off;
  int base;
  uint64_t w;
  __device__ T1kWinCodes(const uint64_t *p_, int64_t off_) : p(p_), off(off_), base(1 << 30), w(0) {}
  __device__ __forceinline__ int code(int pos) {
    if (pos < base || pos >= base + 32) { base = pos > 31 ? pos - 31 : 0; w = t1k_get32(p, off + base); }
    return (int)((w >> (2 * (pos - base))) & 3);
  }
};

__global__ __launch_bounds__(WG) void k_align_flags(SlowArgs P, uint32_t *flags) {
  const uint32_t q = blockIdx.x * blockDim.x + threadIdx.x;
  if (q >= P.nSlow) return;
  uint32_t fl = 1;
  if (q > 0) {
    const T1kOvl o = P.ovl[P.slowQueue[q]], p = P.ovl[P.slowQueue[q - 1]];
    const int lt = o.seqEnd - o.seqStart + 1;
    if (o.re == p.re && ((o.flags ^ p.flags) & 2) == 0 && o.readStart == p.readStart && o.readEnd == p.readEnd && lt == p.seqEnd - p.seqStart + 1 &&
        t1k_same_window(P.ref.bases, P.ref.nmask, (int64_t)P.ref.alleleOff[p.allele] + p.seqStart, (int64_t)P.ref.alleleOff[o.allele] + o.seqStart, lt, P.ref.anyN != 0))
      fl = 0;
  }
  flags[q] = fl;
}
__global__ __launch_bounds__(WG) void k_align_reps(const uint32_t *flags, const uint32_t *runOf, uint32_t *rep, uint32_t n) {
  const uint32_t q = blockIdx.x * blockDim.x + threadIdx.x;
  if (q < n && flags[q]) rep[runOf[q] - 1] = q;
}

template <bool EQ>
__global__ __launch_bounds__(WG) void k_align_fill(SlowArgs P) {
  const uint32_t u = blockIdx.x * blockDim.x + threadIdx.x;
  unsigned long long cells = 0;
  if (u < P.nRuns) {
    const uint32_t q = P.rep[u];
    const uint32_t gid = P.slowQueue[q];
    const T1kOvl o = P.ovl[gid];
    const int pass = (o.flags & 2) ? 1 : 0;
    const int S = P.reads.S;
    const uint64_t *rb = P.reads.bases + ((uint64_t)o.re * 2 + pass) * S;
    const uint64_t *rn = P.reads.nmask + ((uint64_t)o.re * 2 + pass) * S;
    const int64_t goff = (int64_t)P.ref.alleleOff[o.allele];
    const int lp = o.readEnd - o.readStart + 1, lt = o.seqEnd - o.seqStart + 1;
    T1kSeqView T{P.ref.bases, P.ref.nmask, goff + o.seqStart}, Pv{rb, rn, (int64_t)o.readStart};
    uint64_t *trace = (uint64_t *)P.scratch + u;
    if (EQ) t1k_ga_equal_traced(T, Pv, lp, trace, P.traceStride);
    else t1k_ga_band<4, true>(T, lt, Pv, lp, trace, P.traceStride);
    cells = (unsigned long long)lp * (EQ ? 11u : 9u);
  }
#pragma unroll
  for (int o = 32; o > 0; o >>= 1) cells += __shfl_xor(cells, o, 64);
  if ((threadIdx.x & 63) == 0 && cells) atomicAdd(&P.counters[T1K_CTR_DP_CELLS], cells);
}

__global__ __launch_bounds__(WG) void k_align_apply_eq(SlowArgs P) {
  const uint32_t q = blockIdx.x * blockDim.x + threadIdx.x;
  if (q >= P.nSlow) return;
  const size_t nThreads = P.traceStride;
  const uint64_t *trace = (const uint64_t *)P.scratch + (P.runOf[q] - 1);
  {
    const uint32_t gid = P.slowQueue[q];
    const T1kOvl o = P.ovl[gid];
    const int pass = (o.flags & 2) ? 1 : 0;
    const int S = P.reads.S;
    const uint64_t *rb = P.reads.bases + ((uint64_t)o.re * 2 + pass) * S;
    const uint64_t *rn = P.reads.nmask + ((uint64_t)o.re * 2 + pass) * S;
    const int64_t goff = (int64_t)P.ref.alleleOff[o.allele];
    const int L = o.readEnd - o.readStart + 1;
    const int w = P.noCov ? 0 : (int)P.reads.weight[o.re];
    int32_t *cov = P.ref.covDiff + goff;
    T1kWinBits exW(P.ref.exon, goff), gnW(P.ref.nmask, goff), rnW(rn, 0);
    const int alleleLen = (int)P.ref.alleleLen[o.allele];
    int relaxed = 0;
    int runLo = -1, runHi = -1;
    int ti = L, tj = L, mat = 0;
    while (ti > 0 || tj > 0) {
      int bits;
      if (ti > 0 && tj > 0) bits = (int)((trace[(size_t)ti * nThreads] >> (5 * (tj - ti + 5))) & 31);
      else if (ti == 0) bits = 2 | (tj == 1 ? 8 : 0);
      else bits = (ti == 1 ? 4 : 0);
      int op;
      int refPos;
      if (mat == 0) {
        if (ti > 0 && tj > 0 && (bits & 1)) { op = (bits & 16) ? 0 : 1; refPos = o.seqStart + tj - 1; --ti; --tj; }
        else { mat = (bits & 2) ? 2 : 1; continue; }
      } else if (mat == 1) {
        op = 2; refPos = o.seqStart + tj;
        if (ti > 0) { if (bits & 4) mat = 0; --ti; } else mat = 2;
      } else {
        op = 3; refPos = o.seqStart + tj - 1;
        if (tj > 0) { if (bits & 8) mat = 0; --tj; } else mat = 1;
      }
      if (P.relax) {
        bool ex = refPos < alleleLen ? exW.bit(refPos) != 0 : false;
        if (!ex || op == 0) ++relaxed;
      }
      if (op == 0 && w) {
        const int readPos = o.readStart + ti;
        if (!rnW.bit(readPos) && !gnW.bit(refPos)) {
          if (refPos == runLo - 1) runLo = refPos;
          else if (refPos == runLo - 2 && runLo >= 0) { atomicAdd(&cov[P.ref.covStride + runLo - 1], w); runLo = refPos; }
          else {
            if (runLo >= 0) { atomicAdd(&cov[runLo], w); atomicAdd(&cov[runHi + 1], -w); }
            runLo = runHi = refPos;
          }
        }
      }
    }
    if (runLo >= 0) { atomicAdd(&cov[runLo], w); atomicAdd(&cov[runHi + 1], -w); }
    P.ovl[gid].relaxed = (uint16_t)(P.relax ? 2 * relaxed : (int)o.matchCnt);
  }
}

__global__ __launch_bounds__(WG) void k_align_apply_band(SlowArgs P) {
  const uint32_t q = blockIdx.x * blockDim.x + threadIdx.x;
  if (q >= P.nSlow) return;
  const size_t nThreads = P.traceStride;
  const uint64_t *trace = (const uint64_t *)P.scratch + (P.runOf[q] - 1);
  {
    const uint32_t gid = P.slowQueue[q];
    const T1kOvl o = P.ovl[gid];
    const int pass = (o.flags & 2) ? 1 : 0;
    const int S = P.reads.S;
    const uint64_t *rb = P.reads.bases + ((uint64_t)o.re * 2 + pass) * S;
    const uint64_t *rn = P.reads.nmask + ((uint64_t)o.re * 2 + pass) * S;
    const int64_t goff = (int64_t)P.ref.alleleOff[o.allele];
    const int lp = o.readEnd - o.readStart + 1, lt = o.seqEnd - o.seqStart + 1;
    const int LB = 5 + (lp > lt ? lp - lt : 0);
    const int w = P.noCov ? 0 : (int)P.reads.weight[o.re];
    T1kSeqView T{P.ref.bases, P.ref.nmask, goff + o.seqStart}, Pv{rb, rn, (int64_t)o.readStart};
    int32_t *cov = P.ref.covDiff + goff;
    T1kWinBits exW(P.ref.exon, goff), gnW(P.ref.nmask, goff), rnW(rn, 0);
    T1kWinCodes gbW(P.ref.bases, goff), rbW(rb, 0);
    const int alleleLen = (int)P.ref.alleleLen[o.allele];
    int relaxed = 0, runLo = -1, runHi = -1;
    int ti = lp, tj = lt, mat = 0;
    while (ti > 0 || tj > 0) {
      int bits;
      if (ti > 0 && tj > 0) bits = (int)((trace[(size_t)ti * nThreads] >> (4 * (tj - ti + LB))) & 15);
      else if (ti == 0) bits = 2 | (tj == 1 ? 8 : 0);
      else bits = (ti == 1 ? 4 : 0);
      int op, refPos;
      if (mat == 0) {
        if (ti > 0 && tj > 0 && (bits & 1)) {
          const int ct = gnW.bit(o.seqStart + tj - 1) ? 4 : gbW.code(o.seqStart + tj - 1);
          const int cp = rnW.bit(o.readStart + ti - 1) ? 4 : rbW.code(o.readStart + ti - 1);
          op = t1k_eq(ct, cp) ? 0 : 1; refPos = o.seqStart + tj - 1; --ti; --tj;
        }
        else { mat = (bits & 2) ? 2 : 1; continue; }
      } else if (mat == 1) {
        op = 2; refPos = o.seqStart + tj;
        if (ti > 0) { if (bits & 4) mat = 0; --ti; } else mat = 2;
      } else {
        op = 3; refPos = o.seqStart + tj - 1;
        if (tj > 0) { if (bits & 8) mat = 0; --tj; } else mat = 1;
      }
      if (P.relax) {
        bool ex = refPos < alleleLen ? exW.bit(refPos) != 0 : false;
        if (!ex || op == 0) ++relaxed;
      }
      if (op == 0 && w) {
        const int readPos = o.readStart + ti;
        if (!rnW.bit(readPos) && !gnW.bit(refPos)) {
          if (refPos == runLo - 1) runLo = refPos;
          else if (refPos == runLo - 2 && runLo >= 0) { atomicAdd(&cov[P.ref.covStride + runLo - 1], w); runLo = refPos; }
          else {
            if (runLo >= 0) { atomicAdd(&cov[runLo], w); atomicAdd(&cov[runHi + 1], -w); }
            runLo = runHi = refPos;
          }
        }
      }
    }
    if (runLo >= 0) { atomicAdd(&cov[runLo], w); atomicAdd(&cov[runHi + 1], -w); }
    P.ovl[gid].relaxed = (uint16_t)(P.relax ? 2 * relaxed : (int)o.matchCnt);
  }
}


__device__ __forceinline__ double ovlSimilarity(const T1kOvl &o) {
  int spans = o.readEnd - o.readStart + 1 + o.seqEnd - o.seqStart + 1 + 2 * o.leftClip + 2 * o.rightClip;
  return (double)o.matchCnt / (double)spans;
}

__device__ inline bool ovlBeforeFull(const T1kOvl &a, const T1kOvl &b) {
  if (a.readStart != b.readStart) return a.readStart < b.readStart;
  if (a.readEnd != b.readEnd) return a.readEnd < b.readEnd;
  if (a.seqStart != b.seqStart) return a.seqStart < b.seqStart;
  return a.seqEnd < b.seqEnd;
}

#if T1K_TRUNC_SMALL_WAVES > 0 || T1K_TRUNC_LARGE_WAVES > 0
#define T1K_TRUNC_ATTR __attribute__((amdgpu_waves_per_eu(SELECT_LDS_CAP == SELECT_SMALL ? (T1K_TRUNC_SMALL_WAVES > 0 ? T1K_TRUNC_SMALL_WAVES : 1) : (T1K_TRUNC_LARGE_WAVES > 0 ? T1K_TRUNC_LARGE_WAVES : 1))))
#else
#define T1K_TRUNC_ATTR
#endif
template <int SELECT_LDS_CAP, int NT, bool XL>
__global__ __launch_bounds__(NT) T1K_TRUNC_ATTR void k_truncate(TruncArgs P) {
  extern __shared__ uint64_t dynLds[];
  uint64_t *sKey = dynLds;
  __shared__ uint32_t sCut, sTie2;
  __shared__ uint32_t warpSums[NT / 64];
  __shared__ CsTables sCs;
  __shared__ uint16_t sCnt[256 * (NT / 64)];
  const int tid = threadIdx.x;
  __shared__ uint32_t sNextRe;
  uint32_t hoNext = 0, hoLeft = 0;
  for (;;) {
    __syncthreads();
    if (tid == 0) {
      constexpr uint32_t HO = SELECT_LDS_CAP == SELECT_SMALL ? T1K_TRUNC_SMALL_HANDOUT : T1K_TRUNC_LARGE_HANDOUT;
      if (hoLeft == 0) { hoNext = (uint32_t)atomicAdd(&P.counters[SELECT_LDS_CAP == SELECT_SMALL ? T1K_CTR_TRUNC_HANDOUT : T1K_CTR_TRUNC_HANDOUT + 1], (unsigned long long)HO); hoLeft = HO; }
      sNextRe = hoNext++; --hoLeft;
    }
    __syncthreads();
    const uint32_t re = sNextRe;
    if (re >= P.reads.nReadEnds) break;
    const uint32_t n = P.ovlCount[re], o0 = P.ovlStart[re];
    if (n <= 1000) continue;
    if ((n > SELECT_SMALL) != (SELECT_LDS_CAP == SELECT_LARGE)) continue;
    uint32_t np2 = 8;
    while (np2 < n) np2 <<= 1;
    uint64_t *key;
    uint64_t *wgScratch = P.sortScratch + (uint64_t)blockIdx.x * ((uint64_t)P.sortCap * 6);
    if (np2 <= SELECT_LDS_CAP) key = sKey;
    else if (np2 <= P.sortCap) key = wgScratch;
    else { if (tid == 0) atomicOr(&P.counters[T1K_CTR_ERR], (unsigned long long)ERR_SORTCAP); continue; }
    T1kOvl *stage = (T1kOvl *)(wgScratch + P.sortCap * 2);
    if (n > P.sortCap) { if (tid == 0) atomicOr(&P.counters[T1K_CTR_ERR], (unsigned long long)ERR_SORTCAP); continue; }
    int iBits = 1;
    while ((1u << iBits) < n) ++iBits;
    const uint64_t iMask = (1ull << iBits) - 1;
    const KeyW W = truncWidths<XL>((int)P.reads.len[re]);
    for (uint32_t i = tid; i < np2; i += NT) {
      uint64_t kk = ~0ull;
      if (i < n) {
        const T1kOvl o = P.ovl[o0 + i];
        int rspan = o.readEnd - o.readStart;
        int d = rspan + 1 + o.seqEnd - o.seqStart + 1 + 2 * o.leftClip + 2 * o.rightClip;
        if (!packSortKey(W, (int)o.matchCnt, d, rspan, o.allele, i, P.alleleBits, iBits, &kk)) { atomicOr(&P.counters[T1K_CTR_ERR], (unsigned long long)ERR_SORTCAP); kk = i; }
        stage[i] = o;
      }
      key[i] = kk;
    }
    __syncthreads();
    if (key != sKey || !ldsClassRanks<NT>(key, n, P.alleleBits + iBits, sCs)) bitonicSort(key, np2);
    else {
      for (int sh = 0; sh < P.alleleBits; sh += 8)
        ldsCountingPass<NT>(key, n, sCnt, warpSums, [&](uint64_t kk) { return (uint32_t)(kk >> (iBits + sh)) & (P.alleleBits - sh >= 8 ? 0xFFu : ((1u << (P.alleleBits - sh)) - 1u)); });
      ldsCountingPass<NT>(key, n, sCnt, warpSums, [&](uint64_t kk) { return csRankOf(sCs, (uint32_t)(kk >> (P.alleleBits + iBits))); });
    }
    if (tid == 0) { sCut = n; sTie2 = 0; }
    __syncthreads();
    for (uint32_t i = 1 + tid; i < n; i += NT)
      if ((key[i] >> iBits) == (key[i - 1] >> iBits)) sTie2 = 1;
    __syncthreads();
    if (sTie2 && tid == 0) {
      for (uint32_t i = 1; i < n; ++i) {
        if ((key[i] >> iBits) != (key[i - 1] >> iBits)) continue;
        uint32_t j = i;
        while (j > 0 && (key[j - 1] >> iBits) == (key[j] >> iBits) && ovlBeforeFull(stage[key[j] & iMask], stage[key[j - 1] & iMask])) {
          uint64_t t = key[j]; key[j] = key[j - 1]; key[j - 1] = t;
          --j;
        }
      }
    }
    __syncthreads();
    {
      const double s0 = ovlSimilarity(stage[key[0] & iMask]);
      uint32_t mine = n;
      for (uint32_t j = 1 + tid; j < n; j += NT)
        if (ovlSimilarity(stage[key[j] & iMask]) < s0 - 0.1) { mine = j; break; }
      if (mine < n) atomicMin(&sCut, mine);
    }
    __syncthreads();
    const uint32_t cut = sCut;
    for (uint32_t i = tid; i < cut; i += NT) P.ovl[o0 + i] = stage[key[i] & iMask];
    if (tid == 0) P.ovlCount[re] = cut;
    __syncthreads();
  }
}

__global__ __launch_bounds__(WG) void k_coverage_scan(T1kRefDev ref, int32_t *out, const uint64_t *outOff) {
  uint32_t a = blockIdx.x;
  if (a >= ref.nAlleles) return;
  __shared__ uint32_t warpSums[4];
  __shared__ int32_t sCarry;
  const int len = (int)ref.alleleLen[a];
// ... 165 lines not shown
```

t1k_amd/csrc/t1k_capi.hip:

```cpp
#include <sys/mman.h>
#include <map>
#include <mutex>
#include <unordered_map>
#include <algorithm>
#include <memory>
#include <thread>
#include <chrono>
#include <cstring>
#include <cstdio>
#include <cstdlib>
#include "t1k_dev.h"
#include "t1k_launch.h"

namespace {
struct DevPool {
  std::mutex m;
  std::map<int, std::multimap<size_t, void *>> freeBlocks;
  std::unordered_map<void *, std::pair<size_t, int>> live;
  size_t pooled = 0;
};
DevPool &devPool() { static DevPool *p = new DevPool(); return *p; }
}

hipError_t t1k_dev_malloc(void **out, size_t bytes) {
// ... 1036 lines not shown
  uint64_t tot = 0;
  for (uint32_t i = 0; i < n; ++i) tot += counts[i];
  if (tot && !ovl) return t1k_fail(ctx, T1K_ERR_ARG, "t1k_overlaps_upload: bad arguments");
  std::vector<T1kOvlP> packed(tot);
  for (uint64_t g = 0; g < tot; ++g) {
    const t1k_overlap &r = ovl[g];
    const bool fits = r.seq_idx >= 0 && (uint32_t)r.seq_idx < ctx->ref.nAlleles && (r.strand == 1 || r.strand == -1) && r.read_start >= 0 && r.read_end >= 0 && r.read_start < 65536 &&
                      r.read_end < 65536 && r.match_cnt >= 0 && r.match_cnt < 65536 && r.relaxed_match_cnt >= 0 && r.relaxed_match_cnt < 65536 && r.left_clip >= 0 &&
                      r.left_clip < 65536 && r.right_clip >= 0 && r.right_clip < 65536 && r.read_start <= r.read_end && r.seq_start >= 0 && r.seq_start <= r.seq_end &&
                      r.seq_idx >= 0 && (uint32_t)r.seq_idx < ctx->ref.nAlleles && (uint32_t)r.seq_end < ctx->hAlleleLen[r.seq_idx];
    T1kOvl o{};
    o.allele = (uint32_t)r.seq_idx; o.seqStart = r.seq_start; o.seqEnd = r.seq_end; o.readStart = (uint16_t)r.read_start; o.readEnd = (uint16_t)r.read_end;
    o.matchCnt = (uint16_t)r.match_cnt; o.relaxed = (uint16_t)r.relaxed_match_cnt; o.leftClip = (uint16_t)r.left_clip; o.rightClip = (uint16_t)r.right_clip;
    o.flags = r.strand == -1 ? 2u : 0u;
    if (!fits || !t1k_ovl_pack(o, packed[g])) return t1k_fail(ctx, T1K_ERR_ARG, "t1k_overlaps_upload: record " + std::to_string(g) + " lies outside its allele or does not fit the packed overlap fields");
  }
  int rc;
  if ((rc = t1k_ensure(ctx, ctx->bOvlUpload, (size_t)tot * sizeof(T1kOvlP) + 16))) return rc;
  std::vector<unsigned long long> ptr(n);
  uint64_t at = 0;
  for (uint32_t i = 0; i < n; ++i) { ptr[i] = (unsigned long long)((const T1kOvlP *)ctx->bOvlUpload.p + at); at += counts[i]; }
  if (tot) T1K_HIP(ctx, hipMemcpyAsync(ctx->bOvlUpload.p, packed.data(), (size_t)tot * sizeof(T1kOvlP), hipMemcpyHostToDevice, ctx->stream));
  if (n) {
    T1K_HIP(ctx, hipMemcpyAsync(ctx->reads.listPtr, ptr.data(), (size_t)n * 8, hipMemcpyHostToDevice, ctx->stream));
    T1K_HIP(ctx, hipMemcpyAsync(ctx->reads.listCount, counts, (size_t)n * 4, hipMemcpyHostToDevice, ctx->stream));
  }
  T1K_HIP(ctx, hipStreamSynchronize(ctx->stream));
  return T1K_OK;
}

double t1k_alloc_ms(t1k_ctx *ctx, uint64_t *bytes) {
  if (!ctx) return 0;
  if (bytes) *bytes = ctx->bytesAlloc;
  return ctx->msAlloc;
}

int t1k_stats_get(t1k_ctx *ctx, t1k_stats *out) {
  if (!ctx || !out) return T1K_ERR_ARG;
  *out = ctx->stats;
  return T1K_OK;
}

int t1k_route_report_enable(t1k_ctx *ctx, int on) {
  if (!ctx) return T1K_ERR_ARG;
  ctx->route.on = on != 0;
  ctx->route.kept = t1k_route_totals{};
  ctx->route.keptRecs.clear(); ctx->route.passRecs.clear();
  return T1K_OK;
}

int t1k_route_report_get(t1k_ctx *ctx, t1k_route_totals *totals, t1k_route_rec *recs, uint64_t cap, uint64_t *nRecs) {
  if (!ctx || !nRecs) return T1K_ERR_ARG;
  if (!ctx->route.on) return t1k_fail(ctx, T1K_ERR_STATE, "t1k_route_report_get: the route report is off (t1k_route_report_enable)");
  *nRecs = ctx->route.keptRecs.size();
  if (totals) *totals = ctx->route.kept;
  if (recs) {
    if (cap < *nRecs) return t1k_fail(ctx, T1K_ERR_ARG, "t1k_route_report_get: room for " + std::to_string(cap) + " records, " + std::to_string(*nRecs) + " held");
    if (*nRecs) memcpy(recs, ctx->route.keptRecs.data(), *nRecs * sizeof(t1k_route_rec));
  }
  return T1K_OK;
}

int t1k_seed_report_enable(t1k_ctx *ctx, int on) {
  if (!ctx) return T1K_ERR_ARG;
  ctx->seedRep.on = on != 0;
  ctx->seedRep.passValid = false;
  ctx->seedRep.pass = t1k_ctx::SeedRange{};
  ctx->seedRep.kept.clear();
  return T1K_OK;
}

int t1k_seed_report_get(t1k_ctx *ctx, uint8_t *seen, uint32_t *counts, uint32_t *masks, t1k_seed_used *used, uint64_t cap, uint64_t *nUsed) {
  if (!ctx || !nUsed) return T1K_ERR_ARG;
  if (!ctx->seedRep.on) return t1k_fail(ctx, T1K_ERR_STATE, "t1k_seed_report_get: the seed report is off (t1k_seed_report_enable)");
  const uint64_t n = ctx->reads.nReadEnds;
  constexpr uint32_t MW = 2 * T1K_SEED_MASK_WORDS;
  std::vector<uint32_t> owner(n, 0xFFFFFFFFu);
  const auto &kept = ctx->seedRep.kept;
  for (size_t r = 0; r < kept.size(); ++r)
    for (uint64_t i = kept[r].first; i < kept[r].first + kept[r].count && i < n; ++i) owner[i] = (uint32_t)r;
  uint64_t total = 0;
  for (uint64_t i = 0; i < n; ++i)
    if (owner[i] != 0xFFFFFFFFu) { const auto &k = kept[owner[i]]; const uint64_t j = i - k.first; total += k.usedPtr[j + 1] - k.usedPtr[j]; }
  *nUsed = total;
  if (used && cap < total) return t1k_fail(ctx, T1K_ERR_ARG, "t1k_seed_report_get: room for " + std::to_string(cap) + " used entries, " + std::to_string(total) + " held");
  uint64_t at = 0;
  for (uint64_t i = 0; i < n; ++i) {
    const bool have = owner[i] != 0xFFFFFFFFu;
    if (seen) seen[i] = have ? 1 : 0;
    if (counts) { counts[2 * i] = 0; counts[2 * i + 1] = 0; }
    if (masks) std::fill_n(masks + i * MW, MW, 0u);
    if (!have) continue;
    const auto &k = kept[owner[i]];
    const uint64_t j = i - k.first;
    if (counts) { counts[2 * i] = k.counts[2 * j]; counts[2 * i + 1] = k.counts[2 * j + 1]; }
    if (masks) std::copy_n(&k.masks[j * MW], MW, masks + i * MW);
    if (used) std::copy(k.used.begin() + k.usedPtr[j], k.used.begin() + k.usedPtr[j + 1], used + at);
    at += k.usedPtr[j + 1] - k.usedPtr[j];
  }
  return T1K_OK;
}

static void refViewArrays(const t1k_ctx *ctx, const void *ptr[T1K_REF_ARRAYS], uint64_t len[T1K_REF_ARRAYS], uint32_t bytes[T1K_REF_ARRAYS]) {
  const T1kRefDev &r = ctx->ref;
  const auto &z = ctx->refSizes;
  const int k = ctx->prm.kmer_length;
  const uint64_t nKeys = 1ull << (2 * k), nPre = 1ull << (2 * std::max(1, k - 2)), A = r.nAlleles;
  auto set = [&](int x, const void *p, uint64_t n, uint32_t b) { ptr[x] = p; len[x] = n; bytes[x] = b; };
  set(T1K_REF_BASES, r.bases, z.nWords, 8); set(T1K_REF_NMASK, r.nmask, z.nWords, 8); set(T1K_REF_EXON, r.exon, z.nWords, 8); set(T1K_REF_POSTED, r.posted, z.nWords, 8);
  set(T1K_REF_BASES_T, r.basesT, r.basesT ? z.basesTLen : 0, 8); set(T1K_REF_BLOCK_T, r.blockT, r.basesT ? z.nBlocksT : 0, 4);
  set(T1K_REF_ALLELE_OFF, r.alleleOff, A, 8); set(T1K_REF_ALLELE_LEN, r.alleleLen, A, 4); set(T1K_REF_ALLELE_HAS_N, r.alleleHasN, A, 1);
  set(T1K_REF_SEP_START, r.sepStart, A + 1, 4); set(T1K_REF_SEP_POS, r.sepPos, z.nSep, 4);
  set(T1K_REF_K_START, r.kStart, nKeys + 1, 4); set(T1K_REF_K_HAS, r.kHas, (nKeys + 31) / 32, 4); set(T1K_REF_K_MULTI, r.kMulti, (nKeys + 31) / 32, 4);
  set(T1K_REF_K_HAS_PRE, r.kHasPre, (nPre + 31) / 32, 4);
  set(T1K_REF_K_DIR_IDX, r.kDirIdx, nKeys, 4); set(T1K_REF_K_DIR, r.kDir, (uint64_t)z.dirRows * r.kDirStride, 4);
  set(T1K_REF_K_DIR_MASK, r.kDirMask, (uint64_t)z.dirRows * r.kDirMaskWords, 8);
  set(T1K_REF_K_POST, r.kPost, z.nPost, (uint32_t)sizeof(T1kPosting)); set(T1K_REF_K_POST_ALLELE, r.kPostAllele, z.nPost, 4);
}

int t1k_ref_view_geometry(t1k_ctx *ctx, t1k_ref_geometry *out) {
  if (!ctx || !out) return T1K_ERR_ARG;
  if (!ctx->ref.bases) return t1k_fail(ctx, T1K_ERR_ARG, "t1k_ref_view_geometry: no reference uploaded");
  const void *ptr[T1K_REF_ARRAYS];
  t1k_ref_geometry g{};
  refViewArrays(ctx, ptr, g.len, g.elem_bytes);
  g.n_alleles = ctx->ref.nAlleles; g.k = (uint32_t)ctx->prm.kmer_length;
  g.total_bases = ctx->ref.totalBases; g.n_words = ctx->refSizes.nWords; g.n_postings = ctx->refSizes.nPost;
  g.bases_t_len = g.len[T1K_REF_BASES_T]; g.n_sep = ctx->refSizes.nSep;
  g.dir_rows = ctx->refSizes.dirRows; g.dir_stride = ctx->ref.kDirStride; g.dir_mask_words = ctx->ref.kDirMaskWords;
  g.has_bases_t = ctx->ref.basesT ? 1u : 0u;
  *out = g;
  return T1K_OK;
}

int t1k_ref_view_copy(t1k_ctx *ctx, int array, uint64_t first, uint64_t count, void *out) {
  if (!ctx) return T1K_ERR_ARG;
  if (!ctx->ref.bases) return t1k_fail(ctx, T1K_ERR_ARG, "t1k_ref_view_copy: no reference uploaded");
  if (array < 0 || array >= T1K_REF_ARRAYS) return t1k_fail(ctx, T1K_ERR_ARG, "t1k_ref_view_copy: no array " + std::to_string(array));
  const void *ptr[T1K_REF_ARRAYS];
  uint64_t len[T1K_REF_ARRAYS];
  uint32_t bytes[T1K_REF_ARRAYS];
  refViewArrays(ctx, ptr, len, bytes);
  if (first > len[array] || count > len[array] - first)
    return t1k_fail(ctx, T1K_ERR_ARG, "t1k_ref_view_copy: array " + std::to_string(array) + " holds " + std::to_string(len[array]) + " elements, asked for [" +
                                          std::to_string(first) + ", " + std::to_string(first) + " + " + std::to_string(count) + ")");
  if (!count) return T1K_OK;
  if (!out) return t1k_fail(ctx, T1K_ERR_ARG, "t1k_ref_view_copy: no room given");
  T1K_HIP(ctx, hipSetDevice(ctx->device));
  T1K_HIP(ctx, hipMemcpyAsync(out, (const char *)ptr[array] + first * bytes[array], count * bytes[array], hipMemcpyDeviceToHost, ctx->stream));
  T1K_HIP(ctx, hipStreamSynchronize(ctx->stream));
  return T1K_OK;
}

}
```

t1k_amd/csrc/t1k_chain.hip:

```cpp
#include <algorithm>
#include "t1k_dev.h"
#include "t1k_launch.h"
#include "t1k_memo.h"
#include "t1k_group.h"
#include "t1k_chain_rec.h"

#define GROUP_FAST_MAXLEN 320
#define GENERAL_CAP 128
#define BIG_CAP 16384
#define GA_BIG_MAX 2048
#define GA_SCRATCH_INTS (6 * (GA_BIG_MAX + 4))

struct CandOut {
  uint32_t *dst;
  int n;
  int stride = 3;
  int cap = 0x7FFFFFFF;
  bool overflow = false;
  __device__ void push(int rs, int re, int ss, int se, int m0, int m) {
    if (n >= cap) { overflow = true; return; }
    dst[stride * n + 0] = (uint32_t)rs | ((uint32_t)re << 12);
    dst[stride * n + 1] = (uint32_t)ss | ((uint32_t)m0 << 20);
    dst[stride * n + 2] = (uint32_t)se | ((uint32_t)m << 20);
    if (stride == 6) dst[6 * n + 3] = dst[6 * n + 4] = dst[6 * n + 5] = 0;
// ... 213 lines not shown
      int gs = nextClear(pos);
      if (gs >= spanEnd) break;
      int ge = nextSet(gs);
      if (ge > spanEnd) ge = spanEnd;
      int x = mmIn(gs, ge);
      if (x <= 3) sumSmall += x; else ++nBig;
      pos = ge;
    }
    const int upper = 2 * (span - sumSmall - nBig);
#ifdef T1K_WALK_STATS
    { const int cls = nBig == 0 ? 0 : ((double)upper / (double)(2 * span) < simThreshold) ? 1 : 2;
      for (int c = 0; c < 3; ++c) { const unsigned long long mk = __ballot(cls == c); if (mk && (int)(threadIdx.x & 63) == __ffsll((long long)mk) - 1) atomicAdd(&sink.counters[T1K_WIN_WALK_STATS + c], (unsigned long long)__popcll(mk)); } }
#endif
    if (nBig == 0) matchCnt = upper;
    else if ((double)upper / (double)(2 * span) < simThreshold) matchCnt = upper;
    else {
      int gapMatch = 0, nref = 0;
      bool again = false;
      pos = first;
      while (true) {
        int gs = nextClear(pos);
        if (gs >= spanEnd) break;
        int ge = nextSet(gs);
        if (ge > spanEnd) ge = spanEnd;
        int x = mmIn(gs, ge);
        if (x <= 3) gapMatch += (ge - gs) - x;
        else {
          uint32_t slot = 0;
          int r = gapMatchesCached<DEFER>(c, gs, c.goff + (gs - diag), ge - gs, ge - gs, strandBit, sink, dpCounter, &slot);
          if (r >= 0) gapMatch += r;
          else if (r == -1 && nref < GROUP_MAX_REFS) { refs[nref >> 1] |= slot << (16 * (nref & 1)); ++nref; }
          else again = true;
        }
        pos = ge;
      }
      if (again) return 2;
      matchCnt = 2 * cov + 2 * gapMatch;
      if (nref) { *nRefs = nref; result = 3; }
    }
  }
  out.push(first, last + k - 1, first - diag, last - diag + k - 1, 2 * cov, matchCnt);
  return result;
}

template <class Arr>
__device__ inline void chainRun(const ReadCtx &c, int k, int hitLenRequired, Arr A, Arr B, Arr C, int s, int m, int *gaScratch, int gaMax, CandOut &out,
                                unsigned int *dpCounter, unsigned long long *errFlags, bool *needScratch, const GapSink *sink, int strandBit, bool chainReady = false) {
    int ret, lenR, lenS;
    if (!t1k_run_lis(A, B, C, s, m, k, hitLenRequired, &ret, &lenR, &lenS, chainReady)) return;
    uint32_t refs[3] = {0, 0, 0};
    int nref = 0;
    auto gapM = [&](int ra, int ga, int lp, int lt) -> int {
      if (!sink) return gapMatches(c, ra, ga, lp, lt, gaScratch, gaMax, dpCounter, errFlags, needScratch);
      if (lp <= 0 || lt <= 0) return 0;
      const int diff = lt > lp ? lt - lp : lp - lt;
      if (diff > 4) { *needScratch = true; return 0; }
      uint32_t slot = 0;
      const int r = gapMatchesCached<true>(c, ra, c.goff + ga, lp, lt, strandBit, *sink, dpCounter, &slot);
      if (r >= 0) return r;
      if (r == -1 && nref < GROUP_MAX_REFS) { refs[nref >> 1] |= slot << (16 * (nref & 1)); ++nref; return 0; }
      if (dpCounter) ++*dpCounter;
      return gapAlign(c, ra, c.goff + ga, lp, lt);
    };
    int matchCnt = 2 * k;
    for (int i = 1; i < ret; ++i) {
      int pa = (int)(A[s + i - 1] & 0xFFF), pb = (int)(A[s + i - 1] >> 12), qa = (int)(A[s + i] & 0xFFF), qb = (int)(A[s + i] >> 12);
      bool sameDiag = (pb - pa) == (qb - qa);
      bool readOv = pa + k - 1 >= qa, seqOv = pb + k - 1 >= qb;
      if (sameDiag) {
        if (readOv) matchCnt += 2 * (qa - pa);
        else matchCnt += 2 * k + 2 * gapM(pa + k, pb + k, qa - (pa + k), qb - (pb + k));
      } else {
        if (readOv && !seqOv) matchCnt += 2 * (qa - pa);
        else if (!readOv && seqOv) matchCnt += 2 * (qb - pb);
        else if (readOv && seqOv) matchCnt += 2 * ((qa - pa) < (qb - pb) ? (qa - pa) : (qb - pb));
        else matchCnt += 2 * k + 2 * gapM(pa + k, pb + k, qa - (pa + k), qb - (pb + k));
      }
    }
    int rs = (int)(A[s] & 0xFFF), ss = (int)(A[s] >> 12);
    int re = (int)(A[s + ret - 1] & 0xFFF) + k - 1, se = (int)(A[s + ret - 1] >> 12) + k - 1;
    out.push(rs, re, ss, se, 2 * lenR, matchCnt);
    out.setRefs(refs, nref);
}

template <class Arr>
__device__ inline void groupGeneral(const uint32_t *h, int n, const ReadCtx &c, int k, int radius, int hitLenRequired, Arr A, Arr B,
                                     Arr C, int *gaScratch, int gaMax, CandOut &out, unsigned int *dpCounter, unsigned long long *errFlags, bool *needScratch,
                                     const GapSink *sink = nullptr, int strandBit = 0) {
  for (int i = 0; i < n; ++i) {
    uint32_t x = h[i];
    int j = i - 1;
    while (j >= 0 && hitKeyLess(x, A[j])) { A[j + 1] = A[j]; --j; }
    A[j + 1] = x;
  }
  for (int s = 0; s < n;) {
    auto diagOf = [](uint32_t x) { return (int)(x & 0xFFF) - (int)(x >> 12); };
    int curDiff = diagOf(A[s]), curCnt = 1, domCnt = 0, dominant = 0;
    int e = s + 1;
    for (; e < n; ++e) {
      int d = diagOf(A[e]) - diagOf(A[e - 1]);
      if (d < 0) d = -d;
      if (d > radius) break;
      if (d == 0) ++curCnt;
      else {
        if (curCnt > domCnt) { dominant = curDiff; domCnt = curCnt; }
        curDiff = diagOf(A[e]); curCnt = 1;
      }
    }
    if (curCnt > domCnt) dominant = curDiff;
    if (e - s < 3 || (e - s) * k < hitLenRequired) { s = e; continue; }
    int m = 0;
    for (int q = s; q < e; ++q) {
      int a = (int)(A[q] & 0xFFF);
      int dq = diagOf(A[q]) - dominant; if (dq < 0) dq = -dq;
      bool keep = true;
      for (int r = s; r < e; ++r) {
        if ((int)(A[r] & 0xFFF) != a) continue;
        int dr = diagOf(A[r]) - dominant; if (dr < 0) dr = -dr;
        if (dr < dq) { keep = false; break; }
      }
      if (keep) {
        uint32_t x = A[q];
        int j = m - 1;
        while (j >= 0 && x < B[j]) { B[j + 1] = B[j]; --j; }
        B[j + 1] = x;
        ++m;
      }
    }
    chainRun(c, k, hitLenRequired, A, B, C, s, m, gaScratch, gaMax, out, dpCounter, errFlags, needScratch, sink, strandBit);
    s = e;
  }
}

template <class Arr>
__device__ inline void groupSimple(const uint32_t *h, int n, const ReadCtx &c, int k, int hitLenRequired, Arr A, CandOut &out, unsigned int *dpCounter,
                                   unsigned long long *errFlags, bool *needScratch, const GapSink *sink, int strandBit) {
  for (int i = 0; i < n; ++i) A[i] = h[i];
  if (n < 3 || n * k < hitLenRequired) return;
  chainRun(c, k, hitLenRequired, A, A, A, 0, n, nullptr, 0, out, dpCounter, errFlags, needScratch, sink, strandBit, true);
}

struct VoteKey {
  uint64_t hi, lo;
  __device__ bool operator<(const VoteKey &o) const { return hi != o.hi ? hi < o.hi : lo < o.lo; }
};
__device__ __forceinline__ VoteKey voteKey(int matchCnt0, int rs, int re, uint32_t allele, int strandPlus, int ss, int se) {
  VoteKey k;
  k.hi = ((uint64_t)(4095 - matchCnt0) << 40) | ((uint64_t)(4095 - (re - rs)) << 26) | ((uint64_t)allele << 1) | (uint64_t)strandPlus;
  k.lo = ((uint64_t)rs << 52) | ((uint64_t)re << 40) | ((uint64_t)ss << 20) | (uint64_t)se;
  return k;
}


__device__ __forceinline__ ReadCtx makeCtx(const ChainArgs &P, uint32_t re, int pass, uint32_t allele) {
  const int S = P.reads.S;
  ReadCtx c{P.reads.bases + ((uint64_t)re * 2 + pass) * S, P.reads.nmask + ((uint64_t)re * 2 + pass) * S, (int)P.reads.len[re], P.ref.bases, P.ref.nmask,
            (int64_t)P.ref.alleleOff[allele], (int)P.ref.alleleLen[allele], P.ref.anyN != 0};
  if (P.ref.basesT) c.gT = P.ref.basesT + (uint64_t)P.ref.blockT[allele >> 6] + (allele & 63u);
  return c;
}

template <int NW, int MODE>
__global__ __launch_bounds__(WG) void k_chain_fast(ChainArgs P, const uint32_t *list, uint32_t nItems, const unsigned long long *nDev) {
  constexpr bool DEFER = MODE != 2;
  constexpr bool LOOP = MODE != 0;
  unsigned int dpLocal = 0, fastLocal = 0;
  if (nDev && P.counters[T1K_CTR_ERR]) return;
  const uint32_t limit = list ? (nDev ? (uint32_t)*nDev : nItems)
                              : (uint32_t)min(*t1k_arena_cursor(P.counters, T1K_AR_GROUPS, blockIdx.y), (unsigned long long)P.groupSegCap);
  const uint32_t step = gridDim.x * WG;
#pragma unroll 1
  for (uint32_t base = blockIdx.x * WG; base < limit; base += step) {
  int kind = 0;
  uint32_t gi = 0;
  const uint32_t gid = base + threadIdx.x;
  const bool valid = gid < limit;
  if (valid) gi = list ? list[gid] : blockIdx.y * P.groupSegCap + gid;
  if (valid) {
    uint32_t *rec = P.recs + (uint64_t)gi * P.recStride;
    constexpr int RW = NW == 5 ? 8 : 16;
    uint32_t rv[RW];
#pragma unroll
    for (int w = 0; w < RW / 4; ++w) {
      const uint4 q4 = ((const uint4 *)rec)[w];
      rv[4 * w] = q4.x; rv[4 * w + 1] = q4.y; rv[4 * w + 2] = q4.z; rv[4 * w + 3] = q4.w;
    }
    const uint32_t re = rv[0] & 0x7FFFFFFFu, allele = rv[1];
    const int pass = (rv[0] >> 31) ? 0 : 1;
    const bool general = recIsGeneral(rv[2]);
    if (general) kind = 4;
    else {
      uint32_t Mw[NW];
#pragma unroll
      for (int w = 0; w < NW; ++w) Mw[w] = rv[3 + w];
      ReadCtx c = makeCtx(P, re, pass, allele);
      if (MODE != 0) c.gT = nullptr;
      uint32_t cbuf[3];
      CandOut out{cbuf, 0};
      const GapSink sink{P.memo + (uint64_t)re * GAP_CACHE, P.jobStr, P.counters, re * GAP_CACHE, P.jobSegCap, T1K_AR_JOBS};
      uint32_t refs[2] = {0, 0};
      int nRefs = 0;
      kind = groupFastPath<NW, DEFER, MODE == 0>(Mw, recDiag(rv[2]), c, P.ref.alleleHasN[allele] != 0, P.k, P.hitLenRequired, P.sim, out, &dpLocal, pass, sink, refs, &nRefs, P.earlyPrune);
      if (kind == 3) {
        ((uint2 *)rec)[1] = make_uint2((uint32_t)nRefs, cbuf[0]);
        ((uint2 *)rec)[2] = make_uint2(cbuf[1], cbuf[2]);
        ((uint2 *)rec)[3] = make_uint2(refs[0], refs[1]);
      } else if (kind == 1) {
        ++fastLocal;
        if (out.n) { ((uint2 *)rec)[1] = make_uint2(REC_DONE | 1u, cbuf[0]); ((uint2 *)rec)[2] = make_uint2(cbuf[1], cbuf[2]); }
        else if (MODE != 0) rec[2] = REC_DONE;
      }
    }
  }
  if (kind == 2) { const uint32_t q = t1k_arena_append(P.counters, T1K_AR_RETRY, P.listSegCap); if (q != T1K_ARENA_FULL) P.retryStr[q] = gi; }
  if (kind == 3) { const uint32_t q = t1k_arena_append(P.counters, T1K_AR_FINISH, P.listSegCap); if (q != T1K_ARENA_FULL) P.finishStr[q] = gi; }
  if (kind == 4) { const uint32_t q = t1k_arena_append(P.counters, T1K_AR_GENERAL, P.rareSegCap); if (q != T1K_ARENA_FULL) P.generalStr[q] = gi; }
  if (kind == 5) { const uint32_t q = t1k_arena_append(P.counters, T1K_AR_SLOW, P.listSegCap); if (q != T1K_ARENA_FULL) P.slowStr[q] = gi; }
  if (!LOOP) break;
  }
  t1k_stat_add(P.counters, T1K_STAT_DP, dpLocal);
  t1k_stat_add(P.counters, T1K_STAT_FAST, fastLocal);
}

__global__ __launch_bounds__(WG) void k_dp_dense(ChainArgs P, const uint32_t *jobs, uint32_t nJobs, const unsigned long long *nDev) {
  if (nDev) { if (P.counters[T1K_CTR_ERR]) return; nJobs = (uint32_t)*nDev; }
  unsigned int dpLocal = 0;
  for (uint32_t q = blockIdx.x * blockDim.x + threadIdx.x; q < nJobs; q += gridDim.x * blockDim.x) {
    const uint32_t tag = jobs[q];
    const uint32_t re = tag / GAP_CACHE;
    unsigned long long *slot = P.memo + tag;
    const unsigned long long e = __hip_atomic_load(slot, __ATOMIC_RELAXED, __HIP_MEMORY_SCOPE_AGENT);
    const int sb = (int)(e & 1), d = (int)((e >> 1) & 0xF) - 4, lp = (int)((e >> 5) & 0x1FF), readPos = (int)((e >> 14) & 0x7FF);
    const int S = P.reads.S;
    ReadCtx c{P.reads.bases + ((uint64_t)re * 2 + sb) * S, P.reads.nmask + ((uint64_t)re * 2 + sb) * S, 0, P.ref.bases, P.ref.nmask, 0, 0, P.ref.anyN != 0};
    const int m = gapAlign<true>(c, readPos, GAP_GPOS(e), lp, lp + d);
    ++dpLocal;
    __hip_atomic_store(slot, (e & ~(GAP_PENDING << 25)) | ((unsigned long long)m << 25), __ATOMIC_RELAXED, __HIP_MEMORY_SCOPE_AGENT);
  }
  t1k_stat_add(P.counters, T1K_STAT_DP, dpLocal);
}

__device__ inline int gatherHits(const ChainArgs &P, uint32_t re, int pass, uint32_t allele, uint32_t *h, int cap) {
  const int maxK = (int)P.maxK;
  const uint32_t nPlus = P.usedCount[2 * re], nMinus = P.usedCount[2 * re + 1];
  const uint32_t b = pass == 0 ? 0 : nPlus, e = pass == 0 ? nPlus : nPlus + nMinus;
  const uint32_t *uo = P.usedOut + (uint64_t)re * maxK * 4;
  int n = 0;
  for (uint32_t u = b; u < e; ++u) {
    const uint32_t rOff = uo[4 * u], st = uo[4 * u + 1], ln = uo[4 * u + 2];
    uint32_t l = 0, r = ln;
    while (l < r) { uint32_t m = (l + r) >> 1; if (P.ref.kPost[st + m].allele < allele) l = m + 1; else r = m; }
    for (; l < ln; ++l) {
      const T1kPosting pst = P.ref.kPost[st + l];
      if (pst.allele != allele) break;
      if (n < cap) h[n] = (pst.offset << 12) | rOff;
      ++n;
    }
  }
  return n;
}

#define GENERAL_SMALL 32
#define WAVE_CAP 4096
__device__ __forceinline__ uint32_t evenBits32(uint64_t x) {
  x &= 0x5555555555555555ull;
  x = (x | (x >> 1)) & 0x3333333333333333ull; x = (x | (x >> 2)) & 0x0F0F0F0F0F0F0F0Full; x = (x | (x >> 4)) & 0x00FF00FF00FF00FFull;
  x = (x | (x >> 8)) & 0x0000FFFF0000FFFFull; x = (x | (x >> 16)) & 0xFFFFFFFFull;
  return (uint32_t)x;
}
template <int NW>
__global__ __launch_bounds__(WG) void k_near_hits(ChainArgs P, uint32_t nItems, const unsigned long long *nDev) {
  constexpr int NQ = NW + 1;
  if (nDev) { if (P.counters[T1K_CTR_ERR]) return; nItems = (uint32_t)*nDev; }
  for (uint32_t qb = blockIdx.x * WG; qb < nItems; qb += gridDim.x * WG) {
  const uint32_t q = qb + threadIdx.x;
  bool toWave = false;
  uint32_t gi = 0;
  if (q < nItems) {
    gi = P.generalList[q];
    uint32_t *rec = P.recs + (uint64_t)gi * P.recStride;
    constexpr int RW = NW == 5 ? 8 : 16;
    uint32_t rv[RW];
#pragma unroll
    for (int w = 0; w < RW / 4; ++w) { const uint4 q4 = ((const uint4 *)rec)[w]; rv[4 * w] = q4.x; rv[4 * w + 1] = q4.y; rv[4 * w + 2] = q4.z; rv[4 * w + 3] = q4.w; }
    const uint32_t re = rv[0] & 0x7FFFFFFFu, allele = rv[1];
    const int pass = (rv[0] >> 31) ? 0 : 1;
    const int d0 = recDiag(rv[2]), k = P.k, R = P.radius;
    const uint32_t nearCnt = recNear(rv[2]);
    uint32_t onDiag = 0;
#pragma unroll
    for (int w = 0; w < NW; ++w) onDiag += __popc(rv[3 + w]);
    const int64_t goff = (int64_t)P.ref.alleleOff[allele];
    const int alleleLen = (int)P.ref.alleleLen[allele];
    const int64_t W0 = goff - d0 - R;
    const int64_t lastWord = (W0 >> 5) + NQ + 2;
    bool ok = recFar(rv[2]) == 0 && nearCnt > 0 && nearCnt < 31 && R <= 15 && W0 >= 0 && (uint64_t)lastWord < (P.ref.totalBases >> 5) + 7;
    uint32_t base = T1K_ARENA_FULL;
    const uint32_t n = onDiag + nearCnt;
    if (ok) { base = t1k_arena_alloc(P.counters, T1K_AR_GENHITS, n, P.genHitSegCap); ok = base != T1K_ARENA_FULL; }
    if (ok) {
      const int S = P.reads.S;
      const uint64_t *rb = P.reads.bases + ((uint64_t)re * 2 + pass) * S;
      const uint32_t *um = P.usedMask + ((uint64_t)re * 2 + pass) * T1K_USED_MASK_WORDS;
      uint64_t Rr[NQ], G[NQ + 2], PG[NQ + 2];
#pragma unroll
      for (int j = 0; j < NQ; ++j) Rr[j] = j < S ? rb[j] : 0ull;
      const uint64_t *gb = P.ref.bases + (W0 >> 5), *pb = P.ref.posted + (W0 >> 5);
#pragma unroll
      for (int j = 0; j < NQ + 2; ++j) { G[j] = gb[j]; PG[j] = pb[j]; }
      const int sh0 = (int)(W0 & 31);
      uint32_t w = base, cntNear = 0;
      bool same0 = false;
      int nearDiags = 0, d1 = 0;
      uint32_t M1[NW];
#pragma unroll
      for (int j = 0; j < NW; ++j) M1[j] = 0;
      for (int dl = -R; dl <= R; ++dl) {
        const int d = d0 + dl;
        const int o = sh0 + (R - dl);
        const bool up = o >= 32;
        const int bsh = (o & 31) * 2;
        uint64_t acc[NQ], pst[NQ];
#pragma unroll
        for (int j = 0; j < NQ; ++j) {
          const uint64_t lo = up ? G[j + 1] : G[j], hi = up ? G[j + 2] : G[j + 1];
          const uint64_t g = bsh ? ((lo >> bsh) | (hi << (64 - bsh))) : lo;
          const uint64_t x = g ^ Rr[j];
          acc[j] = ~(x | (x >> 1)) & 0x5555555555555555ull;
          const uint64_t pl = up ? PG[j + 1] : PG[j], ph = up ? PG[j + 2] : PG[j + 1];
          pst[j] = bsh ? ((pl >> bsh) | (ph << (64 - bsh))) : pl;
        }
        auto andShifted = [&](int m) {
          const int b = 2 * m;
#pragma unroll
          for (int j = 0; j < NQ; ++j) { const uint64_t nx = j + 1 < NQ ? acc[j + 1] : 0ull; acc[j] &= (acc[j] >> b) | (nx << (64 - b)); }
        };
        {
          int have = 1;
          while (2 * have <= k) { andShifted(have); have *= 2; }
          if (have < k) andShifted(k - have);
        }
        const int aLo = d > 0 ? d : 0, aHi = d + alleleLen - k;
#pragma unroll
        for (int j = 0; j < NW; ++j) {
          uint32_t m = evenBits32(acc[j] & pst[j]) & um[j];
          const int p0 = 32 * j;
          if (aLo > p0) m &= aLo - p0 >= 32 ? 0u : ~0u << (aLo - p0);
          if (aHi < p0 + 31) m &= aHi < p0 ? 0u : ~0u >> (31 - (aHi - p0));
          if (dl == 0) { if (j == 0) same0 = true; same0 = same0 && m == rv[3 + j]; continue; }
          if (m) {
            if (nearDiags == 0 || d1 != d) { ++nearDiags; if (nearDiags == 1) d1 = d; }
            if (nearDiags == 1) M1[j] = m;
          }
          cntNear += __popc(m);
          while (m) {
            const int p = __ffs((int)m) - 1;
            m &= m - 1;
            const uint32_t a = (uint32_t)(p0 + p);
            if (w < base + n) P.genHits[w] = ((uint32_t)((int)a - d) << 12) | a;
            ++w;
          }
        }
      }
      ok = same0 && cntNear == nearCnt;
      bool simple = false;
      if (ok && P.nearSimple && nearDiags == 1 && n >= 3 && (int)n * k >= P.hitLenRequired) {
        int lo0 = -1, hi0 = -1, lo1 = -1, hi1 = -1;
#pragma unroll
        for (int j = 0; j < NW; ++j) {
          if (rv[3 + j]) { if (lo0 < 0) lo0 = 32 * j + __ffs((int)rv[3 + j]) - 1; hi0 = 32 * j + 31 - __clz((int)rv[3 + j]); }
          if (M1[j]) { if (lo1 < 0) lo1 = 32 * j + __ffs((int)M1[j]) - 1; hi1 = 32 * j + 31 - __clz((int)M1[j]); }
        }
        const bool first0 = hi0 < lo1 && hi0 - d0 < lo1 - d1, first1 = hi1 < lo0 && hi1 - d1 < lo0 - d0;
        if (first0 || first1) {
          simple = true;
          w = base;
          for (int part = 0; part < 2; ++part) {
            const bool zero = (part == 0) == first0;
            const int dd = zero ? d0 : d1;
#pragma unroll
            for (int j = 0; j < NW; ++j) {
              uint32_t m = zero ? rv[3 + j] : M1[j];
              while (m) {
                const int p = __ffs((int)m) - 1;
                m &= m - 1;
                const uint32_t a = (uint32_t)(32 * j + p);
                P.genHits[w++] = ((uint32_t)((int)a - dd) << 12) | a;
              }
            }
          }
        }
      }
      if (ok && simple) { rec[3] = base; rec[4] = n; rec[6] = 1u; toWave = n > 3 * GENERAL_SMALL; }
      else if (ok) {
        rec[6] = 0u;
#pragma unroll
        for (int j = 0; j < NW; ++j) {
          uint32_t m = rv[3 + j];
          while (m) {
            const int p = __ffs((int)m) - 1;
            m &= m - 1;
            const uint32_t a = (uint32_t)(32 * j + p);
            P.genHits[w++] = ((uint32_t)((int)a - d0) << 12) | a;
          }
        }
        rec[3] = base; rec[4] = n;
        toWave = n > GENERAL_SMALL;
      }
    }
    rec[5] = ok ? REC_NEAR_DONE : 0u;
    if (!ok) rec[6] = 0u;
#ifdef T1K_NEAR_STATS
    {
      int cls = T1K_NEAR_FALLBACK;
      if (recFar(rv[2]) != 0) cls = T1K_NEAR_FAR; else if (nearCnt == 31) cls = T1K_NEAR_SATURATED; else if (ok) cls = rec[6] == 1u ? (n > 96 ? T1K_NEAR_CHAIN_LARGE : T1K_NEAR_CHAIN_SMALL) : (n > 32 ? T1K_NEAR_NOCHAIN_LARGE : T1K_NEAR_NOCHAIN_SMALL);
      atomicAdd(&P.counters[T1K_WIN_NEAR_STATS + cls], 1ull);
    }
#endif
  }
  if (toWave) { const uint32_t wq = t1k_arena_append(P.counters, T1K_AR_WAVE, P.rareSegCap); if (wq != T1K_ARENA_FULL) P.waveStr[wq] = gi; }
  }
}

template <int ROUNDS>
__global__ __launch_bounds__(WG) void k_gather_general(ChainArgs P, uint32_t nItems, int skipDone, const unsigned long long *nDev) {
  if (nDev) { if (P.counters[T1K_CTR_ERR]) return; nItems = (uint32_t)*nDev; }
  const int lane = threadIdx.x & 63;
  const uint32_t wave = (blockIdx.x * WG + threadIdx.x) >> 6, nWaves = gridDim.x * (WG / 64);
  const int maxK = (int)P.maxK;
  static_assert(ROUNDS * 64 >= GROUP_FAST_MAXLEN, "lists of one strand");
  for (uint32_t q = wave; q < nItems; q += nWaves) {
    const uint32_t gi = P.generalList[q];
    uint32_t *rec = P.recs + (uint64_t)gi * P.recStride;
    if (skipDone && rec[5] == REC_NEAR_DONE) continue;
    const uint32_t re = rec[0] & 0x7FFFFFFFu, allele = rec[1];
    const int pass = (rec[0] >> 31) ? 0 : 1;
    const uint32_t nPlus = P.usedCount[2 * re], nMinus = P.usedCount[2 * re + 1];
    const uint32_t b = pass == 0 ? 0 : nPlus, e = pass == 0 ? nPlus : nPlus + nMinus;
    const uint32_t *uo = P.usedOut + (uint64_t)re * maxK * 4;
    uint32_t first[ROUNDS], cnt[ROUNDS], mine = 0;
#pragma unroll
    for (int r = 0; r < ROUNDS; ++r) {
      const uint32_t u = b + lane + 64 * r;
      first[r] = 0; cnt[r] = 0;
      if (u < e) {
        const uint32_t st = uo[4 * u + 1], ln = uo[4 * u + 2], dr = uo[4 * u + 3];
// ... 796 lines not shown
```

t1k_amd/csrc/t1k_dev.h:

```cpp
#pragma once
#include <hip/hip_runtime.h>
#include <stdint.h>
#include <string>
#include <type_traits>
#include <vector>
#include "../../include/t1k_gpu.h"
#include "t1k_counters.h"

#define T1K_MAX_READ_LEN 320
#define T1K_LONG_READ_LEN 1000
#define T1K_EVEN 0x5555555555555555ull
#define T1K_NEG_BIG (-(1 << 28))

struct T1kPosting { uint32_t allele, offset; };

struct T1kCand {
  uint32_t allele;
  uint32_t readSE;
  int32_t seqStart, seqEnd;
  uint32_t match;
  uint32_t re;
};

struct T1kExt {
  int32_t seqStart, seqEnd;
  uint16_t readStart, readEnd;
  uint16_t matchCnt;
  uint16_t leftClip, rightClip;
  uint16_t flags;
  uint32_t pad;
};
enum { T1K_F_DROP = 1, T1K_F_SEPSEED = 2, T1K_F_NEEDCLIP = 4, T1K_F_EXTOK = 8 };

struct T1kOvl {
  uint32_t allele;
  int32_t seqStart, seqEnd;
  uint16_t readStart, readEnd;
  uint16_t matchCnt, relaxed;
  uint16_t leftClip, rightClip;
  uint32_t re;
  uint32_t flags;
};

struct T1kOvlP { unsigned long long lo, hi; };
__host__ __device__ __forceinline__ bool t1k_ovl_pack(const T1kOvl &o, T1kOvlP &p) {
  const int span = o.seqEnd - o.seqStart;
  const bool ok = o.allele < (1u << 24) && o.seqStart >= 0 && o.seqStart < (1 << 20) && span >= 0 && span < 4096 && o.readStart < 1024 && o.readEnd < 1024 &&
                  o.matchCnt < 4096 && o.relaxed < 4096 && o.leftClip < 1024 && o.rightClip < 1024;
  p.lo = (unsigned long long)o.allele | ((unsigned long long)(uint32_t)o.seqStart << 24) | ((unsigned long long)(uint32_t)span << 44) | ((unsigned long long)((o.flags >> 1) & 1u) << 56) |
         ((unsigned long long)(o.flags & 1u) << 57);
  p.hi = (unsigned long long)o.readStart | ((unsigned long long)o.readEnd << 10) | ((unsigned long long)o.matchCnt << 20) | ((unsigned long long)o.relaxed << 32) |
         ((unsigned long long)o.leftClip << 44) | ((unsigned long long)o.rightClip << 54);
  return ok;
}
__host__ __device__ __forceinline__ T1kOvl t1k_ovl_unpack(const T1kOvlP &p) {
  T1kOvl o;
  o.allele = (uint32_t)(p.lo & 0xFFFFFFu);
  o.seqStart = (int32_t)((p.lo >> 24) & 0xFFFFFu);
  o.seqEnd = o.seqStart + (int32_t)((p.lo >> 44) & 0xFFFu);
  o.flags = ((uint32_t)((p.lo >> 56) & 1u) << 1) | (uint32_t)((p.lo >> 57) & 1u);
  o.readStart = (uint16_t)(p.hi & 0x3FFu); o.readEnd = (uint16_t)((p.hi >> 10) & 0x3FFu);
  o.matchCnt = (uint16_t)((p.hi >> 20) & 0xFFFu); o.relaxed = (uint16_t)((p.hi >> 32) & 0xFFFu);
  o.leftClip = (uint16_t)((p.hi >> 44) & 0x3FFu); o.rightClip = (uint16_t)((p.hi >> 54) & 0x3FFu);
  o.re = 0;
  return o;
}

#ifndef T1K_SEED_CHUNK
#define T1K_SEED_CHUNK 512
#endif
#define T1K_DIR_MINLEN 32
#define T1K_NO_DIR 0xFFFFFFFFu
struct T1kRefDev {
  uint32_t nAlleles;
  uint64_t totalBases;
  const uint64_t *bases, *nmask, *exon;
  const uint64_t *basesT;
  const uint32_t *blockT;
  const uint64_t *posted;
  const uint64_t *alleleOff;
  const uint32_t *alleleLen;
  const uint8_t *alleleHasN;
  uint32_t anyN;
  const uint32_t *sepStart;
  const int32_t *sepPos;
  const uint32_t *kStart;
  const uint32_t *kHas;
  const uint32_t *kMulti;
  const uint32_t *kHasPre;
  const uint32_t *kDirIdx;
  const uint32_t *kDir;
  uint32_t kDirStride;
  const unsigned long long *kDirMask;
  uint32_t kDirMaskWords;
  const T1kPosting *kPost;
  const uint32_t *kPostAllele;
  int32_t *covDiff;
  uint64_t covStride;
};

struct T1kReadsDev {
  uint32_t nReadEnds;
  int S;
  const uint64_t *bases;
  const uint64_t *nmask;
  const uint16_t *len;
  const uint32_t *weight;
  unsigned long long *listPtr;
  uint32_t *listCount;
  const uint8_t *skip;
};

typedef uint64_t t1k_u64x2 __attribute__((ext_vector_type(2), aligned(8)));
__device__ __forceinline__ uint64_t t1k_get32(const uint64_t *w, int64_t pos) {
  int64_t wi = pos >> 5;
  int sh = (int)(pos & 31) * 2;
  const t1k_u64x2 v = *(const t1k_u64x2 *)(w + wi);
  return (v.x >> sh) | ((v.y << 1) << (63 - sh));
}
__host__ __device__ __forceinline__ uint32_t t1k_code_revcomp(uint32_t code, int k) {
  uint32_t x = code;
  x = ((x >> 16) | (x << 16));
  x = ((x & 0xFF00FF00u) >> 8) | ((x & 0x00FF00FFu) << 8);
  x = ((x & 0xF0F0F0F0u) >> 4) | ((x & 0x0F0F0F0Fu) << 4);
  x = ((x & 0xCCCCCCCCu) >> 2) | ((x & 0x33333333u) << 2);
  return (~x) >> (32 - 2 * k);
}
__device__ __forceinline__ uint64_t t1k_lowmask(int nPos) {
  return nPos >= 32 ? ~0ull : ((1ull << (2 * nPos)) - 1);
}
__device__ __forceinline__ int t1k_base(const uint64_t *w, int64_t pos) { return (int)((w[pos >> 5] >> ((pos & 31) * 2)) & 3); }
__device__ __forceinline__ int t1k_bit(const uint64_t *w, int64_t pos) { return (int)((w[pos >> 5] >> ((pos & 31) * 2)) & 1); }

__device__ __forceinline__ uint64_t t1k_mm32(const uint64_t *rb, const uint64_t *rn, int64_t rpos, const uint64_t *gb, const uint64_t *gn,
                                               int64_t gpos) {
  uint64_t x = t1k_get32(rb, rpos) ^ t1k_get32(gb, gpos);
  uint64_t m = (x | (x >> 1)) & T1K_EVEN;
  return m & ~(t1k_get32(rn, rpos) | t1k_get32(gn, gpos));
}

__device__ __forceinline__ int t1k_hamming(const uint64_t *rb, const uint64_t *rn, int64_t rpos, const uint64_t *gb, const uint64_t *gn,
                                            int64_t gpos, int L) {
  int x = 0;
  for (int o = 0; o < L; o += 32) {
    uint64_t m = t1k_mm32(rb, rn, rpos + o, gb, gn, gpos + o) & t1k_lowmask(L - o);
    x += __popcll(m);
  }
  return x;
}

__device__ inline bool t1k_low_complexity(const uint64_t *rb, const uint64_t *rn, int rs, int re) {
  int cnt[4] = {0, 0, 0, 0};
  int L = re - rs + 1;
  for (int o = 0; o < L; o += 32) {
    uint64_t x = t1k_get32(rb, rs + o), nn = t1k_get32(rn, rs + o);
    uint64_t valid = T1K_EVEN & ~nn & t1k_lowmask(L - o);
    uint64_t lo = x & T1K_EVEN, hi = (x >> 1) & T1K_EVEN;
    cnt[0] += __popcll(~lo & ~hi & valid);
    cnt[1] += __popcll(lo & ~hi & valid);
    cnt[2] += __popcll(~lo & hi & valid);
    cnt[3] += __popcll(lo & hi & valid);
  }
  int low = 0, lowTotal = 0;
  for (int i = 0; i < 4; ++i)
    if (cnt[i] <= 2) { ++low; lowTotal += cnt[i]; }
  if (lowTotal * 7 >= L) return false;
  return low >= 2;
}

__device__ inline bool t1k_same_window(const uint64_t *gb, const uint64_t *gn, int64_t a, int64_t b, int L, bool anyN = true) {
  if (a == b) return true;
  for (int o = 0; o < L; o += 32) {
    uint64_t lm = t1k_lowmask(L - o);
    uint64_t x = t1k_get32(gb, a + o) ^ t1k_get32(gb, b + o);
    if (anyN) x |= t1k_get32(gn, a + o) ^ t1k_get32(gn, b + o);
    if (x & lm) return false;
  }
  return true;
}

struct T1kSeqView {
  const uint64_t *b, *n;
  int64_t pos;
  bool anyN = true;
  __device__ __forceinline__ int code(int i) const {
    int64_t p = pos + i;
    return t1k_bit(n, p) ? 4 : t1k_base(b, p);
  }
};
__device__ __forceinline__ bool t1k_eq(int a, int b) { return a == b || a == 4 || b == 4; }

__device__ inline int t1k_ga_matches_equal(const T1kSeqView &T, const T1kSeqView &P, int L, int *scoreOut) {
  const int negInf = (L + 1) * (L + 1) * -4;
  int m[13], e[13], cm[13], ce[13];
#pragma unroll
  for (int s = 0; s < 13; ++s) {
    int j = s - 6;
    if (j == 0) { m[s] = 0; e[s] = 0; }
    else { m[s] = -4 - 4 * j; e[s] = -4 - 4 * (L + 1); }
    cm[s] = 0; ce[s] = 0;
  }
  uint64_t pwB = 0, pwN = 0;
  auto row = [&](int i, auto interiorTag) {
    constexpr bool INTERIOR = decltype(interiorTag)::value;
    if (((i - 1) & 31) == 0) { pwB = t1k_get32(P.b, P.pos + i - 1); pwN = t1k_get32(P.n, P.pos + i - 1); }
    const int pq = ((i - 1) & 31) * 2;
    const bool pIsN = (pwN >> pq) & 1;
    const int pc = pIsN ? 4 : (int)((pwB >> pq) & 3);
    const int t0 = i - 6 > 0 ? i - 6 : 0;
    const uint64_t twB = t1k_get32(T.b, T.pos + t0), twN = t1k_get32(T.n, T.pos + t0);
    uint64_t eqm = 0;
    if (INTERIOR) {
      const uint64_t x = twB ^ ((uint64_t)(pc & 3) * T1K_EVEN);
      eqm = pIsN ? ~0ull : (~((x | (x >> 1))) | twN);
    }
    int fLeft = negInf, mLeft = negInf, cfLeft = 0, cmLeft = 0;
#pragma unroll
    for (int s = 0; s < 13; ++s) {
      int j = i + s - 6;
      int nm, ne, nf, ncm, nce, ncf;
      if (!INTERIOR && j < 0) { nm = ne = nf = negInf; ncm = nce = ncf = 0; }
      else if (!INTERIOR && j == 0) { nm = -4 - 4 * i; ne = -4 - i; nf = -4 - 4 * i; ncm = nce = ncf = 0; }
      else if (s == 0 || s == 12 || (!INTERIOR && j > L)) { nm = ne = nf = negInf; ncm = nce = ncf = 0; }
      else {
        int eu = e[s + 1] - 1, mu = m[s + 1] - 5;
        ne = eu > mu ? eu : mu;
        nce = (mu == ne) ? cm[s + 1] : ce[s + 1];
        int fl = fLeft - 1, ml = mLeft - 5;
        nf = fl > ml ? fl : ml;
        ncf = (ml == nf) ? cmLeft : cfLeft;
        bool eq;
        if (INTERIOR) eq = (eqm >> (2 * (s - 1))) & 1;
        else {
          const int tq = (j - 1 - t0) * 2;
          const int tc = ((twN >> tq) & 1) ? 4 : (int)((twB >> tq) & 3);
          eq = t1k_eq(tc, pc);
        }
        int dg = m[s] + (eq ? 2 : -2);
        nm = dg;
        if (ne > nm) nm = ne;
        if (nf > nm) nm = nf;
        if (dg == nm) ncm = cm[s] + (eq ? 1 : 0);
        else if (nf >= ne) ncm = ncf;
        else ncm = nce;
      }
      m[s] = nm; e[s] = ne; cm[s] = ncm; ce[s] = nce;
      fLeft = nf; mLeft = nm; cfLeft = ncf; cmLeft = ncm;
    }
  };
  int i = 1;
  for (; i <= L && i < 7; ++i) row(i, std::false_type{});
  for (; i <= L - 5; ++i) row(i, std::true_type{});
// ... 619 lines not shown
```

t1k_amd/csrc/t1k_refindex.hip:

```cpp
#include <algorithm>
#include <chrono>
#include <cstdio>
#include <cstdlib>
#include <cstring>
#include <thread>
#include "t1k_dev.h"
#include "t1k_launch.h"

namespace {

__global__ void k_ref_pack(const char *ascii, const uint8_t *exon, const uint64_t *srcOff, const uint64_t *alleleOff, const uint32_t *alleleLen, const uint32_t *wordAllele,
                           uint64_t nWords, uint64_t *bases, uint64_t *nmask, uint64_t *exonm, int nCode) {
  const uint64_t w = (uint64_t)blockIdx.x * blockDim.x + threadIdx.x;
  if (w >= nWords) return;
  const uint32_t a = wordAllele[w];
  uint64_t b = 0, n = 0, e = 0;
  if (a != 0xFFFFFFFFu) {
    const uint64_t first = w * 32 - alleleOff[a];
    const uint32_t len = alleleLen[a];
    const char *s = ascii + srcOff[a];
    const uint8_t *x = exon ? exon + srcOff[a] : nullptr;
    for (int q = 0; q < 32; ++q) {
      const uint64_t i = first + q;
      if (i >= len) break;
      const char c = s[i];
      const int code = c == 'A' ? 0 : c == 'C' ? 1 : c == 'G' ? 2 : c == 'T' ? 3 : 4;
      if (code == 4) { n |= 1ull << (2 * q); b |= (uint64_t)nCode << (2 * q); } else b |= (uint64_t)code << (2 * q);
      if (x && x[i]) e |= 1ull << (2 * q);
    }
  }
  bases[w] = b; nmask[w] = n; exonm[w] = e;
}

__global__ void k_ref_transpose(const uint64_t *bases, const uint64_t *alleleOff, const uint32_t *alleleLen, const uint32_t *blockT, uint32_t nBlocks, uint32_t nAlleles, uint64_t totalT,
                                uint64_t *basesT) {
  const uint64_t t = (uint64_t)blockIdx.x * blockDim.x + threadIdx.x;
  if (t >= totalT) return;
  uint32_t lo = 0, hi = nBlocks - 1;
  while (lo < hi) { const uint32_t mid = (lo + hi + 1) >> 1; if ((uint64_t)blockT[mid] <= t) lo = mid; else hi = mid - 1; }
  const uint64_t rel = t - blockT[lo];
  const uint32_t a = lo * 64 + (uint32_t)(rel & 63);
  const uint64_t w = rel >> 6;
  uint64_t v = 0;
  if (a < nAlleles && w < ((uint64_t)alleleLen[a] + 31) / 32) v = bases[(alleleOff[a] >> 5) + w];
  basesT[t] = v;
}

__device__ __forceinline__ uint32_t windowBits(const uint64_t *w, uint64_t p, int k) {
  const uint64_t wi = p >> 5;
  const int sh = (int)(p & 31) * 2;
  uint64_t v = w[wi] >> sh;
  if (sh) v |= w[wi + 1] << (64 - sh);
  return (uint32_t)(v & ((1ull << (2 * k)) - 1));
}

__global__ void k_ref_codes(const uint64_t *bases, const uint64_t *nmask, const uint64_t *alleleOff, const uint32_t *alleleLen, const uint32_t *wordAllele, uint64_t total,
                            int k, uint32_t *flag, uint32_t *code) {
  const uint64_t g = (uint64_t)blockIdx.x * blockDim.x + threadIdx.x;
  if (g >= total) return;
  uint32_t f = 0, c = 0;
  const uint32_t a = wordAllele[g >> 5];
  if (a != 0xFFFFFFFFu) {
    const uint64_t i = g - alleleOff[a];
    if (i < alleleLen[a] && i + 1 >= (uint64_t)k) {
      const uint64_t start = g + 1 - k;
      c = windowBits(bases, start, k);
      const bool valid = windowBits(nmask, start, k) == 0;
      const uint32_t prev = i + 1 == (uint64_t)k ? 0u : windowBits(bases, start - 1, k);
      f = valid && (i == (uint64_t)k || c != prev) ? 1u : 0u;
    }
  }
  flag[g] = f; code[g] = c;
}
__global__ void k_ref_posted(const uint32_t *flag, uint64_t total, int k, uint64_t nWords, uint64_t *posted) {
  const uint64_t w = (uint64_t)blockIdx.x * blockDim.x + threadIdx.x;
  if (w >= nWords) return;
  uint64_t v = 0;
  for (int q = 0; q < 32; ++q) {
    const uint64_t e = w * 32 + q + (uint64_t)(k - 1);
    if (e < total && flag[e]) v |= 1ull << (2 * q);
  }
  posted[w] = v;
}
__global__ void k_ref_compact(const uint32_t *flag, const uint32_t *pos, const uint32_t *code, unsigned long long *key, uint32_t *val, uint64_t total) {
  const uint64_t g = (uint64_t)blockIdx.x * blockDim.x + threadIdx.x;
  if (g < total && flag[g]) { key[pos[g] - 1] = code[g]; val[pos[g] - 1] = (uint32_t)g; }
}
__global__ void k_ref_postings(const unsigned long long *key, const uint32_t *val, const uint64_t *alleleOff, const uint32_t *wordAllele, int k, T1kPosting *post,
                               uint32_t *postAllele, uint32_t *count, uint32_t m) {
  const uint32_t j = blockIdx.x * blockDim.x + threadIdx.x;
  if (j >= m) return;
  const uint32_t g = val[j];
  const uint32_t a = wordAllele[g >> 5];
  post[j] = T1kPosting{a, (uint32_t)(g - alleleOff[a]) - (uint32_t)(k - 1)};
  postAllele[j] = a;
  atomicAdd(&count[(uint32_t)key[j]], 1u);
}
__global__ void k_ref_flags(const uint32_t *kStart, const uint32_t *postAllele, uint64_t nKeys, int k, uint32_t *has, uint32_t *multi, uint32_t *hasPre, uint32_t *needDir) {
  const uint64_t c = (uint64_t)blockIdx.x * blockDim.x + threadIdx.x;
  if (c >= nKeys) return;
  const uint32_t st = kStart[c], ln = kStart[c + 1] - st;
  needDir[c] = ln > T1K_DIR_MINLEN ? 1u : 0u;
  if (!ln) return;
  atomicOr(&has[c >> 5], 1u << (c & 31));
  const int kp = k - 2 > 1 ? k - 2 : 1;
  const uint32_t rc = t1k_code_revcomp((uint32_t)c, k);
  const uint32_t pc = ((uint32_t)c < rc ? (uint32_t)c : rc) & (uint32_t)((1ull << (2 * kp)) - 1);
  atomicOr(&hasPre[pc >> 5], 1u << (pc & 31));
  for (uint32_t i = 1; i < ln; ++i)
    if (postAllele[st + i] == postAllele[st + i - 1]) { atomicOr(&multi[c >> 5], 1u << (c & 31)); break; }
}
__global__ void k_ref_diridx(const uint32_t *needDir, const uint32_t *rowOf, uint32_t *dirIdx, uint32_t *rowCode, uint64_t nKeys) {
  const uint64_t c = (uint64_t)blockIdx.x * blockDim.x + threadIdx.x;
  if (c >= nKeys) return;
  if (needDir[c]) { dirIdx[c] = rowOf[c] - 1; rowCode[rowOf[c] - 1] = (uint32_t)c; }
  else dirIdx[c] = T1K_NO_DIR;
}
__global__ void k_ref_dir(const uint32_t *rowCode, const uint32_t *kStart, const uint32_t *postAllele, uint32_t stride, uint64_t nCells, uint32_t *dir) {
  const uint64_t t = (uint64_t)blockIdx.x * blockDim.x + threadIdx.x;
  if (t >= nCells) return;
  const uint32_t row = (uint32_t)(t / stride), cidx = (uint32_t)(t % stride);
  const uint32_t c = rowCode[row];
  const uint32_t st = kStart[c], ln = kStart[c + 1] - st;
  const uint32_t bound = cidx * T1K_SEED_CHUNK;
  uint32_t lo = 0, hi = ln;
  while (lo < hi) { const uint32_t mid = (lo + hi) / 2; if (postAllele[st + mid] < bound) lo = mid + 1; else hi = mid; }
  dir[t] = lo;
}

__global__ void k_ref_dirmask(const uint32_t *dir, uint32_t stride, uint32_t rows, uint32_t words, unsigned long long *mask) {
  const uint64_t t = (uint64_t)blockIdx.x * blockDim.x + threadIdx.x;
  if (t >= (uint64_t)rows * words) return;
  const uint32_t row = (uint32_t)(t / words), w = (uint32_t)(t % words);
  const uint32_t *d = dir + (uint64_t)row * stride;
  unsigned long long m = 0;
  for (uint32_t b = 0; b < 64; ++b) {
    const uint32_t c = 64 * w + b;
    if (c + 1 < stride && d[c + 1] > d[c]) m |= 1ull << b;
  }
  mask[t] = m;
}

static inline int asciiCode(char c) { return c == 'A' ? 0 : c == 'C' ? 1 : c == 'G' ? 2 : c == 'T' ? 3 : 4; }

int keep(t1k_ctx *ctx, size_t bytes, void **out) {
  T1kDevBuf b;
  int rc = t1k_ensure(ctx, b, bytes);
  if (rc) return rc;
  ctx->refBufs.push_back(b);
  *out = b.p;
  return 0;
}

}

extern "C" int t1k_ref_upload(t1k_ctx *ctx, const char *seqs, const uint64_t *offsets, const uint8_t *exon, uint32_t nAlleles) {
  if (!ctx || !seqs || !offsets || nAlleles == 0 || nAlleles >= (1u << 24)) return t1k_fail(ctx, T1K_ERR_ARG, "t1k_ref_upload: bad arguments");
  if (offsets[nAlleles] - offsets[0] >= (1ull << 29)) return t1k_fail(ctx, T1K_ERR_ARG, "t1k_ref_upload: reference larger than 512 Mbases");
  T1K_HIP(ctx, hipSetDevice(ctx->device));
  hipStream_t st = ctx->stream;
  (void)hipStreamSynchronize(st);
  for (auto &b : ctx->refBufs) if (b.p) (void)t1k_dev_free(b.p);
  ctx->refBufs.clear();
  ctx->ref = T1kRefDev{};
  ctx->refSizes = t1k_ctx::RefSizes{};
  const int k = ctx->prm.kmer_length;
  const int nCode = ctx->prm.n_base_code & 3;
  const bool dbgPhases = getenv("T1K_DEBUG_PHASES") != nullptr;
  auto tLap = std::chrono::steady_clock::now();
  auto lap = [&](const char *what) {
    if (!dbgPhases) return;
    (void)hipStreamSynchronize(st);
    const auto now = std::chrono::steady_clock::now();
    fprintf(stderr, "[t1k] ref_upload %s: %.3f s\n", what, std::chrono::duration<double>(now - tLap).count());
    tLap = now;
  };
  std::vector<uint64_t> alleleOff(nAlleles), srcOff(nAlleles);
  std::vector<uint32_t> alleleLen(nAlleles);
  uint64_t total = 0;
  for (uint32_t a = 0; a < nAlleles; ++a) {
    const uint64_t len = offsets[a + 1] - offsets[a];
    if (len >= (1u << 20)) return t1k_fail(ctx, T1K_ERR_ARG, "allele longer than 2^20 bases");
    alleleOff[a] = total; alleleLen[a] = (uint32_t)len; srcOff[a] = offsets[a] - offsets[0];
    total += (len + 32) / 32 * 32;
  }
  total += 64;
  const uint64_t nWords = total / 32 + 2;
  std::vector<uint32_t> wordAllele(nWords, 0xFFFFFFFFu);
  for (uint32_t a = 0; a < nAlleles; ++a)
    for (uint64_t w = alleleOff[a] / 32; w < (alleleOff[a] + alleleLen[a] + 31) / 32; ++w) wordAllele[w] = a;
  std::vector<uint32_t> sepStart(nAlleles + 1, 0);
  std::vector<uint8_t> alleleHasN(nAlleles, 0);
  std::vector<int32_t> sepPos;
  t1k_ctx::RefSizes sizes;
  {
    const unsigned T = std::max(1u, std::min({16u, std::thread::hardware_concurrency(), nAlleles}));
    std::vector<std::vector<int32_t>> part(T);
    std::vector<uint32_t> cnt(nAlleles, 0);
    std::vector<std::thread> th;
    for (unsigned t = 0; t < T; ++t)
      th.emplace_back([&, t] {
        const uint32_t a0 = (uint32_t)((uint64_t)nAlleles * t / T), a1 = (uint32_t)((uint64_t)nAlleles * (t + 1) / T);
        for (uint32_t a = a0; a < a1; ++a) {
          const char *s = seqs + offsets[a];
          for (uint32_t i = 0; i < alleleLen[a]; ++i)
            if (asciiCode(s[i]) == 4) { part[t].push_back((int32_t)i); ++cnt[a]; alleleHasN[a] = 1; }
        }
      });
    for (auto &x : th) x.join();
    for (uint32_t a = 0; a < nAlleles; ++a) sepStart[a + 1] = sepStart[a] + cnt[a];
    for (auto &p : part) sepPos.insert(sepPos.end(), p.begin(), p.end());
    sizes.nSep = sepPos.size();
    if (sepPos.empty()) sepPos.push_back(0);
  }
  lap("layout + separator scan (host)");
  ctx->hAlleleOff = alleleOff;
  ctx->hAlleleLen = alleleLen;
  T1kRefDev r{};
  r.nAlleles = nAlleles;
  r.totalBases = total;
  int rc;
  void *dBases, *dN, *dExon, *dAlleleOff, *dAlleleLen, *dHasN, *dSepStart, *dSepPos, *dPosted;
  if ((rc = keep(ctx, (nWords + 8) * 8, &dPosted)) || (rc = keep(ctx, (nWords + 8) * 8, &dBases)) || (rc = keep(ctx, (nWords + 8) * 8, &dN)) || (rc = keep(ctx, (nWords + 8) * 8, &dExon))
      || (rc = keep(ctx, (size_t)nAlleles * 8, &dAlleleOff)) ||
      (rc = keep(ctx, (size_t)nAlleles * 4, &dAlleleLen)) || (rc = keep(ctx, nAlleles, &dHasN)) || (rc = keep(ctx, (size_t)(nAlleles + 1) * 4, &dSepStart)) ||
      (rc = keep(ctx, sepPos.size() * 4, &dSepPos)))
    return rc;
  const uint64_t textBytes = offsets[nAlleles] - offsets[0];
  T1kDevBuf bText, bExonB, bSrcOff, bWordAllele, bFlag, bPos, bCode;
  auto freeScratch = [&] { (void)hipStreamSynchronize(st); for (T1kDevBuf *b : {&bText, &bExonB, &bSrcOff, &bWordAllele, &bFlag, &bPos, &bCode}) if (b->p) { (void)t1k_dev_free(b->p); b->p = nullptr; } };
  if ((rc = t1k_ensure(ctx, bText, textBytes + 16)) || (exon && (rc = t1k_ensure(ctx, bExonB, textBytes + 16))) || (rc = t1k_ensure(ctx, bSrcOff, (size_t)nAlleles * 8)) ||
      (rc = t1k_ensure(ctx, bWordAllele, nWords * 4)) || (rc = t1k_ensure(ctx, bFlag, (total + 1) * 4)) || (rc = t1k_ensure(ctx, bPos, (total + 1) * 4)) ||
      (rc = t1k_ensure(ctx, bCode, (total + 1) * 4))) { freeScratch(); return rc; }
#define RU_HIP(call) do { hipError_t e_ = (call); if (e_ != hipSuccess) { freeScratch(); return t1k_fail(ctx, T1K_ERR_DEVICE, std::string(#call) + ": " + hipGetErrorString(e_)); } } while (0)
  RU_HIP(hipMemcpyAsync(bText.p, seqs + offsets[0], textBytes, hipMemcpyHostToDevice, st));
  if (exon) RU_HIP(hipMemcpyAsync(bExonB.p, exon + offsets[0], textBytes, hipMemcpyHostToDevice, st));
  RU_HIP(hipMemcpyAsync(bSrcOff.p, srcOff.data(), (size_t)nAlleles * 8, hipMemcpyHostToDevice, st));
  RU_HIP(hipMemcpyAsync(bWordAllele.p, wordAllele.data(), nWords * 4, hipMemcpyHostToDevice, st));
  RU_HIP(hipMemcpyAsync(dAlleleOff, alleleOff.data(), (size_t)nAlleles * 8, hipMemcpyHostToDevice, st));
  RU_HIP(hipMemcpyAsync(dAlleleLen, alleleLen.data(), (size_t)nAlleles * 4, hipMemcpyHostToDevice, st));
  RU_HIP(hipMemcpyAsync(dHasN, alleleHasN.data(), nAlleles, hipMemcpyHostToDevice, st));
  RU_HIP(hipMemcpyAsync(dSepStart, sepStart.data(), (size_t)(nAlleles + 1) * 4, hipMemcpyHostToDevice, st));
  RU_HIP(hipMemcpyAsync(dSepPos, sepPos.data(), sepPos.size() * 4, hipMemcpyHostToDevice, st));
  hipLaunchKernelGGL(k_ref_pack, dim3((unsigned)((nWords + 255) / 256)), dim3(256), 0, st, (const char *)bText.p, exon ? (const uint8_t *)bExonB.p : nullptr,
                     (const uint64_t *)bSrcOff.p, (const uint64_t *)dAlleleOff, (const uint32_t *)dAlleleLen, (const uint32_t *)bWordAllele.p, nWords, (uint64_t *)dBases,
                     (uint64_t *)dN, (uint64_t *)dExon, nCode);
  void *dBasesT = nullptr, *dBlockT = nullptr;
  {
    static const bool on = [] { const char *e = getenv("T1K_REF_TRANSPOSE"); return !e || atoi(e) != 0; }();
    const uint32_t nBlocks = (nAlleles + 63) / 64;
    std::vector<uint32_t> blockT(nBlocks);
    uint64_t totalT = 0;
    for (uint32_t b = 0; b < nBlocks; ++b) {
      uint32_t words = 0;
      for (uint32_t a = b * 64; a < std::min(nAlleles, b * 64 + 64); ++a) words = std::max(words, (alleleLen[a] + 31) / 32);
      blockT[b] = (uint32_t)totalT;
      totalT += (uint64_t)(words + 2) * 64;
    }
    if (on && nBlocks && totalT + 512 < (1ull << 32)) {
      if ((rc = keep(ctx, (totalT + 512) * 8, &dBasesT)) || (rc = keep(ctx, (size_t)nBlocks * 4, &dBlockT))) { freeScratch(); return rc; }
      RU_HIP(hipMemcpyAsync(dBlockT, blockT.data(), (size_t)nBlocks * 4, hipMemcpyHostToDevice, st));
      RU_HIP(hipMemsetAsync((char *)dBasesT + totalT * 8, 0, 512 * 8, st));
      hipLaunchKernelGGL(k_ref_transpose, dim3((unsigned)((totalT + 255) / 256)), dim3(256), 0, st, (const uint64_t *)dBases, (const uint64_t *)dAlleleOff, (const uint32_t *)dAlleleLen,
                         (const uint32_t *)dBlockT, nBlocks, nAlleles, totalT, (uint64_t *)dBasesT);
      RU_HIP(hipStreamSynchronize(st));
      sizes.basesTLen = totalT + 512; sizes.nBlocksT = nBlocks;
    }
  }
  lap("text upload + pack");
  hipLaunchKernelGGL(k_ref_codes, dim3((unsigned)((total + 255) / 256)), dim3(256), 0, st, (const uint64_t *)dBases, (const uint64_t *)dN, (const uint64_t *)dAlleleOff,
                     (const uint32_t *)dAlleleLen, (const uint32_t *)bWordAllele.p, total, k, (uint32_t *)bFlag.p, (uint32_t *)bCode.p);
  RU_HIP(hipMemsetAsync(dPosted, 0, (nWords + 8) * 8, st));
  hipLaunchKernelGGL(k_ref_posted, dim3((unsigned)((nWords + 255) / 256)), dim3(256), 0, st, (const uint32_t *)bFlag.p, total, k, nWords, (uint64_t *)dPosted);
  if ((rc = t1k_inclusive_sum(ctx, (const uint32_t *)bFlag.p, (uint32_t *)bPos.p, (uint32_t)total))) { freeScratch(); return rc; }
  uint32_t M = 0;
  RU_HIP(hipMemcpyAsync(&M, (uint32_t *)bPos.p + (total - 1), 4, hipMemcpyDeviceToHost, st));
  RU_HIP(hipStreamSynchronize(st));
  const uint64_t nKeys = 1ull << (2 * k);
  const uint32_t Mx = std::max(M, 1u);
  T1kDevBuf bKey, bKeyS, bVal, bValS, bNeed, bRowOf, bRowCode;
  auto freeScratch2 = [&] { freeScratch(); for (T1kDevBuf *b : {&bKey, &bKeyS, &bVal, &bValS, &bNeed, &bRowOf, &bRowCode}) if (b->p) { (void)t1k_dev_free(b->p); b->p = nullptr; } };
#undef RU_HIP
#define RU_HIP(call) do { hipError_t e_ = (call); if (e_ != hipSuccess) { freeScratch2(); return t1k_fail(ctx, T1K_ERR_DEVICE, std::string(#call) + ": " + hipGetErrorString(e_)); } } while (0)
  if ((rc = t1k_ensure(ctx, bKey, (size_t)Mx * 8)) || (rc = t1k_ensure(ctx, bKeyS, (size_t)Mx * 8)) || (rc = t1k_ensure(ctx, bVal, (size_t)Mx * 4)) ||
      (rc = t1k_ensure(ctx, bValS, (size_t)Mx * 4))) { freeScratch2(); return rc; }
  void *dPost, *dPostAllele, *dKStart, *dHas, *dMulti, *dHasPre, *dDirIdx;
  const int kp = std::max(1, k - 2);
  const size_t nPre = (size_t)1 << (2 * kp);
  if ((rc = keep(ctx, (size_t)Mx * sizeof(T1kPosting), &dPost)) || (rc = keep(ctx, (size_t)Mx * 4, &dPostAllele)) || (rc = keep(ctx, (nKeys + 2) * 4, &dKStart)) ||
      (rc = keep(ctx, (nKeys + 31) / 32 * 4, &dHas)) || (rc = keep(ctx, (nKeys + 31) / 32 * 4, &dMulti)) || (rc = keep(ctx, (nPre + 31) / 32 * 4, &dHasPre)) ||
      (rc = keep(ctx, nKeys * 4, &dDirIdx))) { freeScratch2(); return rc; }
  RU_HIP(hipMemsetAsync(dKStart, 0, (nKeys + 2) * 4, st));
  RU_HIP(hipMemsetAsync(dHas, 0, (nKeys + 31) / 32 * 4, st));
  RU_HIP(hipMemsetAsync(dMulti, 0, (nKeys + 31) / 32 * 4, st));
  RU_HIP(hipMemsetAsync(dHasPre, 0, (nPre + 31) / 32 * 4, st));
  if (M) {
    hipLaunchKernelGGL(k_ref_compact, dim3((unsigned)((total + 255) / 256)), dim3(256), 0, st, (const uint32_t *)bFlag.p, (const uint32_t *)bPos.p, (const uint32_t *)bCode.p,
                       (unsigned long long *)bKey.p, (uint32_t *)bVal.p, total);
    if ((rc = t1k_sort_pairs(ctx, (const unsigned long long *)bKey.p, (unsigned long long *)bKeyS.p, (const uint32_t *)bVal.p, (uint32_t *)bValS.p, M, 2 * k))) { freeScratch2(); return rc; }
    hipLaunchKernelGGL(k_ref_postings, dim3((M + 255) / 256), dim3(256), 0, st, (const unsigned long long *)bKeyS.p, (const uint32_t *)bValS.p, (const uint64_t *)dAlleleOff,
                       (const uint32_t *)bWordAllele.p, k, (T1kPosting *)dPost, (uint32_t *)dPostAllele, (uint32_t *)dKStart, M);
  }
  lap("window codes + sort + postings");
  if ((rc = t1k_exclusive_sum32(ctx, (const uint32_t *)dKStart, (uint32_t *)dKStart, nKeys + 1))) { freeScratch2(); return rc; }
  if ((rc = t1k_ensure(ctx, bNeed, (nKeys + 1) * 4)) || (rc = t1k_ensure(ctx, bRowOf, (nKeys + 1) * 4))) { freeScratch2(); return rc; }
  hipLaunchKernelGGL(k_ref_flags, dim3((unsigned)((nKeys + 255) / 256)), dim3(256), 0, st, (const uint32_t *)dKStart, (const uint32_t *)dPostAllele, nKeys, k, (uint32_t *)dHas,
                     (uint32_t *)dMulti, (uint32_t *)dHasPre, (uint32_t *)bNeed.p);
  if ((rc = t1k_inclusive_sum(ctx, (const uint32_t *)bNeed.p, (uint32_t *)bRowOf.p, nKeys))) { freeScratch2(); return rc; }
  uint32_t rows = 0;
  RU_HIP(hipMemcpyAsync(&rows, (uint32_t *)bRowOf.p + (nKeys - 1), 4, hipMemcpyDeviceToHost, st));
  RU_HIP(hipStreamSynchronize(st));
  const uint32_t stride = (nAlleles + T1K_SEED_CHUNK - 1) / T1K_SEED_CHUNK + 1;
  void *dDir;
  if ((rc = keep(ctx, (size_t)std::max(rows, 1u) * stride * 4, &dDir)) || (rc = t1k_ensure(ctx, bRowCode, (size_t)std::max(rows, 1u) * 4))) { freeScratch2(); return rc; }
  hipLaunchKernelGGL(k_ref_diridx, dim3((unsigned)((nKeys + 255) / 256)), dim3(256), 0, st, (const uint32_t *)bNeed.p, (const uint32_t *)bRowOf.p, (uint32_t *)dDirIdx,
                     (uint32_t *)bRowCode.p, nKeys);
  if (rows) {
    const uint64_t cells = (uint64_t)rows * stride;
    hipLaunchKernelGGL(k_ref_dir, dim3((unsigned)((cells + 255) / 256)), dim3(256), 0, st, (const uint32_t *)bRowCode.p, (const uint32_t *)dKStart, (const uint32_t *)dPostAllele, stride,
                       cells, (uint32_t *)dDir);
  } else RU_HIP(hipMemsetAsync(dDir, 0, (size_t)stride * 4, st));
  const uint32_t maskWords = std::max(1u, (stride - 1 + 63) / 64);
  void *dDirMask;
  if ((rc = keep(ctx, (size_t)std::max(rows, 1u) * maskWords * 8, &dDirMask))) { freeScratch2(); return rc; }
  if (rows) hipLaunchKernelGGL(k_ref_dirmask, dim3((unsigned)(((uint64_t)rows * maskWords + 255) / 256)), dim3(256), 0, st, (const uint32_t *)dDir, stride, rows, maskWords, (unsigned long long *)dDirMask);
  else RU_HIP(hipMemsetAsync(dDirMask, 0, (size_t)maskWords * 8, st));
  void *dCov;
  r.covStride = total + 2;
  if ((rc = keep(ctx, 3 * r.covStride * sizeof(int32_t), &dCov))) { freeScratch2(); return rc; }
  RU_HIP(hipMemsetAsync(dCov, 0, 3 * r.covStride * sizeof(int32_t), st));
  RU_HIP(hipStreamSynchronize(st));
  freeScratch2();
#undef RU_HIP
  r.basesT = (const uint64_t *)dBasesT; r.blockT = (const uint32_t *)dBlockT;
  r.bases = (const uint64_t *)dBases; r.nmask = (const uint64_t *)dN; r.exon = (const uint64_t *)dExon; r.posted = (const uint64_t *)dPosted;
  r.alleleOff = (const uint64_t *)dAlleleOff; r.alleleLen = (const uint32_t *)dAlleleLen; r.alleleHasN = (const uint8_t *)dHasN;
  r.anyN = 0;
  for (uint8_t h : alleleHasN) r.anyN |= h;
  r.sepStart = (const uint32_t *)dSepStart; r.sepPos = (const int32_t *)dSepPos;
  r.kStart = (const uint32_t *)dKStart; r.kHas = (const uint32_t *)dHas; r.kMulti = (const uint32_t *)dMulti; r.kHasPre = (const uint32_t *)dHasPre;
  r.kDirIdx = (const uint32_t *)dDirIdx; r.kDir = (const uint32_t *)dDir; r.kDirStride = stride;
  r.kDirMask = (const unsigned long long *)dDirMask; r.kDirMaskWords = maskWords;
  r.kPost = (const T1kPosting *)dPost; r.kPostAllele = (const uint32_t *)dPostAllele;
  r.covDiff = (int32_t *)dCov;
  ctx->ref = r;
  sizes.nWords = nWords; sizes.nPost = M; sizes.dirRows = rows;
  ctx->refSizes = sizes;
  ctx->covFullLen = 0; ctx->covFullDirty = false;
  lap("bucket starts + bitmaps + directory + coverage arrays");
  return T1K_OK;
}
```

Before: 4.107 million.

## Pack per-allele offset, length, N flag and separator range into one 64-bit record

Builds a packed 64-bit record per allele (word offset, length, has-N bit, separator count and start) on the device and makes the chain and assign kernels read it instead of four separate arrays. The three separator scans in the extension step are merged into one loop that computes seed, reach, left and right separators together. The intent is fewer scattered global loads per candidate. The packing assumes allele offsets are 32-aligned and fit in 26+5 bits, lengths fit in 20 bits, and it falls back to sepStart when the count or start overflows.

```diff
diff --git a/include/t1k_gpu.h b/include/t1k_gpu.h
--- a/include/t1k_gpu.h
+++ b/include/t1k_gpu.h
@@ -284,6 +284,7 @@
 } t1k_ref_geometry;
 int t1k_ref_view_geometry(t1k_ctx *ctx, t1k_ref_geometry *out);
 int t1k_ref_view_copy(t1k_ctx *ctx, int array, uint64_t first, uint64_t count, void *out);
+int t1k_ref_view_allele_rec(t1k_ctx *ctx, uint64_t first, uint64_t count, uint64_t *out);
 
 double t1k_alloc_ms(t1k_ctx *ctx, uint64_t *bytes);
 uint64_t t1k_ctx_mem_report(t1k_ctx *ctx, const char *tag, int print);
diff --git a/t1k_amd/capi.py b/t1k_amd/capi.py
--- a/t1k_amd/capi.py
+++ b/t1k_amd/capi.py
@@ -82,6 +82,12 @@
 REF_ARRAYS = (("bases", "<u8"), ("nmask", "<u8"), ("exon", "<u8"), ("posted", "<u8"), ("basesT", "<u8"), ("blockT", "<u4"), ("alleleOff", "<u8"), ("alleleLen", "<u4"),
               ("alleleHasN", "u1"), ("sepStart", "<u4"), ("sepPos", "<i4"), ("kStart", "<u4"), ("kHas", "<u4"), ("kMulti", "<u4"), ("kHasPre", "<u4"), ("kDirIdx", "<u4"),
               ("kDir", "<u4"), ("kDirMask", "<u8"), ("kPost", POSTING_DTYPE), ("kPostAllele", "<u4"))
+ALLELE_REC_CNT_MORE, ALLELE_REC_SEP_MORE = 31, 4095
+
+
+def allele_rec_fields(w):
+    w = int(w)
+    return (w & 0x3FFFFFF) << 5, (w >> 26) & 0xFFFFF, (w >> 46) & 1, (w >> 47) & 31, w >> 52
 
 
 class RefGeometry(C.Structure):
@@ -182,6 +188,7 @@
     L.t1k_seed_report_get.argtypes = [vp, vp, vp, vp, vp, C.c_uint64, u64p]
     L.t1k_ref_view_geometry.argtypes = [vp, vp]
     L.t1k_ref_view_copy.argtypes = [vp, C.c_int, C.c_uint64, C.c_uint64, vp]
+    L.t1k_ref_view_allele_rec.argtypes = [vp, C.c_uint64, C.c_uint64, vp]
     L.t1k_genotyper_main.argtypes = [C.c_int, C.POINTER(C.c_char_p)]
     L.t1k_job_params_default.argtypes = [C.POINTER(JobParams)]
     L.t1k_job_create.argtypes = [C.POINTER(JobParams), C.c_char_p, C.POINTER(vp)]
@@ -488,6 +495,13 @@
         self._check(lib().t1k_ref_view_copy(self.h, i, first, count, _ptr(out)), "t1k_ref_view_copy")
         return out
 
+    def ref_allele_recs(self, first=0, count=None):
+        if count is None:
+            count = self.ref_geometry()["n_alleles"] - first
+        out = np.zeros(max(count, 0), np.uint64)
+        self._check(lib().t1k_ref_view_allele_rec(self.h, first, count, _ptr(out)), "t1k_ref_view_allele_rec")
+        return out
+
     def align_batch(self, texts, pats, want_ops=True):
         n = len(texts)
         tb, toff = _concat(texts)
diff --git a/t1k_amd/csrc/t1k_assign.hip b/t1k_amd/csrc/t1k_assign.hip
--- a/t1k_amd/csrc/t1k_assign.hip
+++ b/t1k_amd/csrc/t1k_assign.hip
@@ -34,16 +34,26 @@
 }
 
 
-__device__ __forceinline__ bool sepInRange(const T1kRefDev &ref, uint32_t allele, int s, int e) {
-  int len = (int)ref.alleleLen[allele];
-  if (s <= -1 && e >= -1) return true;
-  if (s <= len && e >= len) return true;
-  uint32_t b = ref.sepStart[allele], en = ref.sepStart[allele + 1];
+struct SepScan {
+  bool inSeed, inReach;
+  int left, right;
+};
+__device__ __forceinline__ SepScan sepScan(const T1kRefDev &ref, const T1kAlleleRec &ar, uint32_t allele, int ss, int se, int s2, int e2, int lo, int ro) {
+  const int len = recLen(ar);
+  SepScan r;
+  r.inSeed = (ss <= -1 && se >= -1) || (ss <= len && se >= len);
+  r.inReach = (s2 <= -1 && e2 >= -1) || (s2 <= len && e2 >= len);
+  r.left = -1; r.right = 0x7FFFFFFF;
+  uint32_t b, en;
+  recSepRange(ref, ar, allele, &b, &en);
   for (uint32_t i = b; i < en; ++i) {
-    int p = ref.sepPos[i];
-    if (p >= s && p <= e) return true;
-  }
-  return false;
+    const int p = ref.sepPos[i];
+    if (p >= ss && p <= se) r.inSeed = true;
+    if (p >= s2 && p <= e2) r.inReach = true;
+    if (p < ss && p >= ss - lo && p > r.left) r.left = p;
+    if (p > se && p <= se + ro && p < r.right) r.right = p;
+  }
+  return r;
 }
 
 
@@ -60,23 +70,20 @@
   const int rs = (int)(c.readSE & 0xFFFF), re = (int)(c.readSE >> 16);
   const int ss = c.seqStart, se = c.seqEnd;
   const int matchCnt = (int)(c.match >> 16);
-  uint16_t flags = 0;
-  if (sepInRange(P.ref, allele, ss, se)) flags |= T1K_F_SEPSEED;
-  if (sepInRange(P.ref, allele, ss - rs, se + (len - re - 1))) flags |= T1K_F_NEEDCLIP;
-  if (flags & T1K_F_SEPSEED) { x.flags = flags; P.ext[gid] = x; return true; }
-  const int alleleLen = (int)P.ref.alleleLen[allele];
-  const int64_t goff = (int64_t)P.ref.alleleOff[allele];
+  const T1kAlleleRec ar = loadAlleleRec(P.ref, allele);
+  const int alleleLen = recLen(ar);
+  const int64_t goff = recOff(ar);
   int lo = rs < ss ? rs : ss;
   int leftClip = rs > ss ? rs - ss : 0, rightClip = 0;
-  {
-    uint32_t b = P.ref.sepStart[allele], en = P.ref.sepStart[allele + 1];
-    int bestP = -1;
-    for (uint32_t i = b; i < en; ++i) {
-      int p = P.ref.sepPos[i];
-      if (p < ss && p >= ss - lo && p > bestP) bestP = p;
-    }
-    if (bestP >= 0) { int i = ss - 1 - bestP; leftClip = lo - i; lo = i; }
-  }
+  int ro = (len - 1 - re) < (alleleLen - 1 - se) ? (len - 1 - re) : (alleleLen - 1 - se);
+  if (len - 1 - re > alleleLen - 1 - se) rightClip = len - 1 - re - (alleleLen - 1 - se);
+  const SepScan sc = sepScan(P.ref, ar, allele, ss, se, ss - rs, se + (len - re - 1), lo, ro);
+  uint16_t flags = 0;
+  if (sc.inSeed) flags |= T1K_F_SEPSEED;
+  if (sc.inReach) flags |= T1K_F_NEEDCLIP;
+  if (flags & T1K_F_SEPSEED) { x.flags = flags; P.ext[gid] = x; return true; }
+  if (sc.left >= 0) { int i = ss - 1 - sc.left; leftClip = lo - i; lo = i; }
+  if (sc.right != 0x7FFFFFFF) { int i = sc.right - se - 1; rightClip = ro - i; ro = i; }
   unsigned int dpLocal = 0;
   const ReadCtx rc{rb, rn, len, P.ref.bases, P.ref.nmask, goff, alleleLen, P.ref.anyN != 0};
   const GapSink sink{P.memo + (uint64_t)c.re * GAP_CACHE, P.jobStr, P.counters, c.re * GAP_CACHE, P.jobSegCap, T1K_AR_EXTJOBS};
@@ -84,17 +91,6 @@
   bool pending = false;
   int match = gapMatchesCached<DEFER>(rc, rs - lo, goff + ss - lo, lo, lo, pass, sink, &dpLocal, &slot);
   if (match < 0) { pending = true; match = 0; }
-  int ro = (len - 1 - re) < (alleleLen - 1 - se) ? (len - 1 - re) : (alleleLen - 1 - se);
-  if (len - 1 - re > alleleLen - 1 - se) rightClip = len - 1 - re - (alleleLen - 1 - se);
-  {
-    uint32_t b = P.ref.sepStart[allele], en = P.ref.sepStart[allele + 1];
-    int bestP = 0x7FFFFFFF;
-    for (uint32_t i = b; i < en; ++i) {
-      int p = P.ref.sepPos[i];
-      if (p > se && p <= se + ro && p < bestP) bestP = p;
-    }
-    if (bestP != 0x7FFFFFFF) { int i = bestP - se - 1; rightClip = ro - i; ro = i; }
-  }
   {
     const int mr = gapMatchesCached<DEFER>(rc, re + 1, goff + se + 1, ro, ro, pass, sink, &dpLocal, &slot);
     if (mr < 0) pending = true; else match += mr;
@@ -781,7 +777,8 @@
   const int S = P.reads.S;
   const uint64_t *rb = P.reads.bases + ((uint64_t)o.re * 2 + pass) * S;
   const uint64_t *rn = P.reads.nmask + ((uint64_t)o.re * 2 + pass) * S;
-  const int64_t goff = (int64_t)P.ref.alleleOff[o.allele];
+  const T1kAlleleRec ar = loadAlleleRec(P.ref, o.allele);
+  const int64_t goff = recOff(ar);
   const int L = o.readEnd - o.readStart + 1, Ls = o.seqEnd - o.seqStart + 1;
   const int w = P.noCov ? 0 : (P.undo ? -(int)P.reads.weight[o.re] : (int)P.reads.weight[o.re]);
   bool slow = (L != Ls) || L > T1K_MAX_READ_LEN;
@@ -793,7 +790,7 @@
     const int64_t gpos = goff + o.seqStart;
     const int64_t gw = gpos >> 5, rw = o.readStart >> 5;
     const int gsh = (int)(gpos & 31) * 2, rsh = (o.readStart & 31) * 2;
-    const bool hasN = P.ref.alleleHasN[o.allele] != 0;
+    const bool hasN = recHasN(ar);
 #pragma unroll
     for (int q = 0; q < 3; ++q) {
       const u64x2 a = *(const u64x2 *)(P.ref.bases + gw + 2 * q), b = *(const u64x2 *)(rb + rw + 2 * q), c = *(const u64x2 *)(rn + rw + 2 * q);
@@ -904,7 +901,8 @@
     const int S = P.reads.S;
     const uint64_t *rb = P.reads.bases + ((uint64_t)o.re * 2 + pass) * S;
     const uint64_t *rn = P.reads.nmask + ((uint64_t)o.re * 2 + pass) * S;
-    const int64_t goff = (int64_t)P.ref.alleleOff[o.allele];
+    const T1kAlleleRec ar = loadAlleleRec(P.ref, o.allele);
+    const int64_t goff = recOff(ar);
     const int lp = o.readEnd - o.readStart + 1, lt = o.seqEnd - o.seqStart + 1;
     const int w = P.noCov ? 0 : (int)P.reads.weight[o.re];
     if ((lp + 1) * (lt + 1) > P.maxCells || lt > GA_BIG_MAX) { atomicOr(&P.counters[T1K_CTR_ERR], (unsigned long long)ERR_SLOWCAP); continue; }
@@ -915,7 +913,7 @@
     int32_t *cov = P.ref.covDiff + goff;
     for (int i = 0; i < n; ++i) {
       int op = ops[i];
-      bool ex = refPos < (int)P.ref.alleleLen[o.allele] ? t1k_bit(P.ref.exon, goff + refPos) != 0 : false;
+      bool ex = refPos < recLen(ar) ? t1k_bit(P.ref.exon, goff + refPos) != 0 : false;
       if (P.relax) { if (ex) { if (op == 0) ++m; } else ++m; }
       if (op == 0 && w) {
         if (!t1k_bit(rn, readPos) && !t1k_bit(P.ref.nmask, goff + refPos)) { atomicAdd(&cov[refPos], w); atomicAdd(&cov[refPos + 1], -w); }
@@ -1006,12 +1004,13 @@
     const int S = P.reads.S;
     const uint64_t *rb = P.reads.bases + ((uint64_t)o.re * 2 + pass) * S;
     const uint64_t *rn = P.reads.nmask + ((uint64_t)o.re * 2 + pass) * S;
-    const int64_t goff = (int64_t)P.ref.alleleOff[o.allele];
+    const T1kAlleleRec ar = loadAlleleRec(P.ref, o.allele);
+    const int64_t goff = recOff(ar);
     const int L = o.readEnd - o.readStart + 1;
     const int w = P.noCov ? 0 : (int)P.reads.weight[o.re];
     int32_t *cov = P.ref.covDiff + goff;
     T1kWinBits exW(P.ref.exon, goff), gnW(P.ref.nmask, goff), rnW(rn, 0);
-    const int alleleLen = (int)P.ref.alleleLen[o.allele];
+    const int alleleLen = recLen(ar);
     int relaxed = 0;
     int runLo = -1, runHi = -1;
     int ti = L, tj = L, mat = 0;
@@ -1065,7 +1064,8 @@
     const int S = P.reads.S;
     const uint64_t *rb = P.reads.bases + ((uint64_t)o.re * 2 + pass) * S;
     const uint64_t *rn = P.reads.nmask + ((uint64_t)o.re * 2 + pass) * S;
-    const int64_t goff = (int64_t)P.ref.alleleOff[o.allele];
+    const T1kAlleleRec ar = loadAlleleRec(P.ref, o.allele);
+    const int64_t goff = recOff(ar);
     const int lp = o.readEnd - o.readStart + 1, lt = o.seqEnd - o.seqStart + 1;
     const int LB = 5 + (lp > lt ? lp - lt : 0);
     const int w = P.noCov ? 0 : (int)P.reads.weight[o.re];
@@ -1073,7 +1073,7 @@
     int32_t *cov = P.ref.covDiff + goff;
     T1kWinBits exW(P.ref.exon, goff), gnW(P.ref.nmask, goff), rnW(rn, 0);
     T1kWinCodes gbW(P.ref.bases, goff), rbW(rb, 0);
-    const int alleleLen = (int)P.ref.alleleLen[o.allele];
+    const int alleleLen = recLen(ar);
     int relaxed = 0, runLo = -1, runHi = -1;
     int ti = lp, tj = lt, mat = 0;
     while (ti > 0 || tj > 0) {
diff --git a/t1k_amd/csrc/t1k_capi.hip b/t1k_amd/csrc/t1k_capi.hip
--- a/t1k_amd/csrc/t1k_capi.hip
+++ b/t1k_amd/csrc/t1k_capi.hip
@@ -1212,4 +1212,20 @@
   return T1K_OK;
 }
 
-}
+int t1k_ref_view_allele_rec(t1k_ctx *ctx, uint64_t first, uint64_t count, uint64_t *out) {
+  static_assert(sizeof(uint64_t) == sizeof(T1kAlleleRec), "the record is exported as it lies on the device");
+  if (!ctx) return T1K_ERR_ARG;
+  if (!ctx->ref.bases || !ctx->ref.alleleRec) return t1k_fail(ctx, T1K_ERR_ARG, "t1k_ref_view_allele_rec: no reference uploaded");
+  const uint64_t A = ctx->ref.nAlleles;
+  if (first > A || count > A - first)
+    return t1k_fail(ctx, T1K_ERR_ARG, "t1k_ref_view_allele_rec: " + std::to_string(A) + " alleles, asked for [" + std::to_string(first) + ", " + std::to_string(first) + " + " +
+                                          std::to_string(count) + ")");
+  if (!count) return T1K_OK;
+  if (!out) return t1k_fail(ctx, T1K_ERR_ARG, "t1k_ref_view_allele_rec: no room given");
+  T1K_HIP(ctx, hipSetDevice(ctx->device));
+  T1K_HIP(ctx, hipMemcpyAsync(out, ctx->ref.alleleRec + first, count * sizeof(T1kAlleleRec), hipMemcpyDeviceToHost, ctx->stream));
+  T1K_HIP(ctx, hipStreamSynchronize(ctx->stream));
+  return T1K_OK;
+}
+
+}
diff --git a/t1k_amd/csrc/t1k_chain.hip b/t1k_amd/csrc/t1k_chain.hip
--- a/t1k_amd/csrc/t1k_chain.hip
+++ b/t1k_amd/csrc/t1k_chain.hip
@@ -389,13 +389,14 @@
 }
 
 
-__device__ __forceinline__ ReadCtx makeCtx(const ChainArgs &P, uint32_t re, int pass, uint32_t allele) {
+__device__ __forceinline__ ReadCtx makeCtx(const ChainArgs &P, uint32_t re, int pass, uint32_t allele, const T1kAlleleRec &ar) {
   const int S = P.reads.S;
   ReadCtx c{P.reads.bases + ((uint64_t)re * 2 + pass) * S, P.reads.nmask + ((uint64_t)re * 2 + pass) * S, (int)P.reads.len[re], P.ref.bases, P.ref.nmask,
-            (int64_t)P.ref.alleleOff[allele], (int)P.ref.alleleLen[allele], P.ref.anyN != 0};
+            recOff(ar), recLen(ar), P.ref.anyN != 0};
   if (P.ref.basesT) c.gT = P.ref.basesT + (uint64_t)P.ref.blockT[allele >> 6] + (allele & 63u);
   return c;
 }
+__device__ __forceinline__ ReadCtx makeCtx(const ChainArgs &P, uint32_t re, int pass, uint32_t allele) { return makeCtx(P, re, pass, allele, loadAlleleRec(P.ref, allele)); }
 
 template <int NW, int MODE>
 __global__ __launch_bounds__(WG) void k_chain_fast(ChainArgs P, const uint32_t *list, uint32_t nItems, const unsigned long long *nDev) {
@@ -430,14 +431,15 @@
       uint32_t Mw[NW];
 #pragma unroll
       for (int w = 0; w < NW; ++w) Mw[w] = rv[3 + w];
-      ReadCtx c = makeCtx(P, re, pass, allele);
+      const T1kAlleleRec ar = loadAlleleRec(P.ref, allele);
+      ReadCtx c = makeCtx(P, re, pass, allele, ar);
       if (MODE != 0) c.gT = nullptr;
       uint32_t cbuf[3];
       CandOut out{cbuf, 0};
       const GapSink sink{P.memo + (uint64_t)re * GAP_CACHE, P.jobStr, P.counters, re * GAP_CACHE, P.jobSegCap, T1K_AR_JOBS};
       uint32_t refs[2] = {0, 0};
       int nRefs = 0;
-      kind = groupFastPath<NW, DEFER, MODE == 0>(Mw, recDiag(rv[2]), c, P.ref.alleleHasN[allele] != 0, P.k, P.hitLenRequired, P.sim, out, &dpLocal, pass, sink, refs, &nRefs, P.earlyPrune);
+      kind = groupFastPath<NW, DEFER, MODE == 0>(Mw, recDiag(rv[2]), c, recHasN(ar), P.k, P.hitLenRequired, P.sim, out, &dpLocal, pass, sink, refs, &nRefs, P.earlyPrune);
       if (kind == 3) {
         ((uint2 *)rec)[1] = make_uint2((uint32_t)nRefs, cbuf[0]);
         ((uint2 *)rec)[2] = make_uint2(cbuf[1], cbuf[2]);
@@ -527,8 +529,9 @@
     uint32_t onDiag = 0;
 #pragma unroll
     for (int w = 0; w < NW; ++w) onDiag += __popc(rv[3 + w]);
-    const int64_t goff = (int64_t)P.ref.alleleOff[allele];
-    const int alleleLen = (int)P.ref.alleleLen[allele];
+    const T1kAlleleRec ar = loadAlleleRec(P.ref, allele);
+    const int64_t goff = recOff(ar);
+    const int alleleLen = recLen(ar);
     const int64_t W0 = goff - d0 - R;
     const int64_t lastWord = (W0 >> 5) + NQ + 2;
     bool ok = recFar(rv[2]) == 0 && nearCnt > 0 && nearCnt < 31 && R <= 15 && W0 >= 0 && (uint64_t)lastWord < (P.ref.totalBases >> 5) + 7;
diff --git a/t1k_amd/csrc/t1k_dev.h b/t1k_amd/csrc/t1k_dev.h
--- a/t1k_amd/csrc/t1k_dev.h
+++ b/t1k_amd/csrc/t1k_dev.h
@@ -71,6 +71,16 @@
 #endif
 #define T1K_DIR_MINLEN 32
 #define T1K_NO_DIR 0xFFFFFFFFu
+#define T1K_REC_CNT_MORE 31u
+#define T1K_REC_SEP_MORE 4095u
+struct T1kAlleleRec {
+  uint64_t w;
+};
+static_assert(sizeof(T1kAlleleRec) == 8, "one 64-bit load");
+__host__ __device__ __forceinline__ T1kAlleleRec t1k_allele_rec_pack(uint64_t off, uint32_t len, bool hasN, uint32_t cnt, uint32_t sepStart) {
+  return T1kAlleleRec{(off >> 5) | ((uint64_t)len << 26) | ((uint64_t)(hasN ? 1 : 0) << 46) | ((uint64_t)cnt << 47) | ((uint64_t)sepStart << 52)};
+}
+
 struct T1kRefDev {
   uint32_t nAlleles;
   uint64_t totalBases;
@@ -84,6 +94,7 @@
   uint32_t anyN;
   const uint32_t *sepStart;
   const int32_t *sepPos;
+  const T1kAlleleRec *alleleRec;
   const uint32_t *kStart;
   const uint32_t *kHas;
   const uint32_t *kMulti;
@@ -98,6 +109,16 @@
   int32_t *covDiff;
   uint64_t covStride;
 };
+
+__device__ __forceinline__ T1kAlleleRec loadAlleleRec(const T1kRefDev &ref, uint32_t allele) { return ref.alleleRec[allele]; }
+__host__ __device__ __forceinline__ int64_t recOff(const T1kAlleleRec &r) { return (int64_t)((r.w & 0x3FFFFFFull) << 5); }
+__host__ __device__ __forceinline__ int recLen(const T1kAlleleRec &r) { return (int)((r.w >> 26) & 0xFFFFFu); }
+__host__ __device__ __forceinline__ bool recHasN(const T1kAlleleRec &r) { return ((r.w >> 46) & 1u) != 0; }
+__device__ __forceinline__ void recSepRange(const T1kRefDev &ref, const T1kAlleleRec &r, uint32_t allele, uint32_t *b, uint32_t *e) {
+  const uint32_t cnt = (uint32_t)(r.w >> 47) & 31u, st = (uint32_t)(r.w >> 52);
+  if (cnt == T1K_REC_CNT_MORE || st == T1K_REC_SEP_MORE) { *b = ref.sepStart[allele]; *e = ref.sepStart[allele + 1]; }
+  else { *b = st; *e = st + cnt; }
+}
 
 struct T1kReadsDev {
   uint32_t nReadEnds;
diff --git a/t1k_amd/csrc/t1k_refindex.hip b/t1k_amd/csrc/t1k_refindex.hip
--- a/t1k_amd/csrc/t1k_refindex.hip
+++ b/t1k_amd/csrc/t1k_refindex.hip
@@ -139,6 +139,16 @@
     if (c + 1 < stride && d[c + 1] > d[c]) m |= 1ull << b;
   }
   mask[t] = m;
+}
+
+__global__ void k_ref_allele_rec(const uint64_t *alleleOff, const uint32_t *alleleLen, const uint8_t *hasN, const uint32_t *sepStart, uint32_t nAlleles, uint32_t cntMore,
+                                 uint32_t sepMore, T1kAlleleRec *rec) {
+  const uint32_t a = blockIdx.x * blockDim.x + threadIdx.x;
+  if (a >= nAlleles) return;
+  const uint32_t b = sepStart[a], n = sepStart[a + 1] - b;
+  const uint32_t cnt = n >= cntMore ? T1K_REC_CNT_MORE : n;
+  const uint32_t st = n == 0 ? 0u : b >= sepMore ? T1K_REC_SEP_MORE : b;
+  rec[a] = t1k_allele_rec_pack(alleleOff[a], alleleLen[a], hasN[a] != 0, cnt, st);
 }
 
 static inline int asciiCode(char c) { return c == 'A' ? 0 : c == 'C' ? 1 : c == 'G' ? 2 : c == 'T' ? 3 : 4; }
@@ -245,6 +255,17 @@
   hipLaunchKernelGGL(k_ref_pack, dim3((unsigned)((nWords + 255) / 256)), dim3(256), 0, st, (const char *)bText.p, exon ? (const uint8_t *)bExonB.p : nullptr,
                      (const uint64_t *)bSrcOff.p, (const uint64_t *)dAlleleOff, (const uint32_t *)dAlleleLen, (const uint32_t *)bWordAllele.p, nWords, (uint64_t *)dBases,
                      (uint64_t *)dN, (uint64_t *)dExon, nCode);
+  void *dAlleleRec;
+  if ((rc = keep(ctx, (size_t)nAlleles * sizeof(T1kAlleleRec), &dAlleleRec))) { freeScratch(); return rc; }
+  {
+    uint32_t cntMore = T1K_REC_CNT_MORE, sepMore = T1K_REC_SEP_MORE;
+    if (const char *e = getenv("T1K_ALLELE_REC_LIMITS")) {
+      unsigned c = 0, s = 0;
+      if (sscanf(e, "%u,%u", &c, &s) == 2) { cntMore = std::min(cntMore, std::max(c, 1u)); sepMore = std::min(sepMore, s); }
+    }
+    hipLaunchKernelGGL(k_ref_allele_rec, dim3((nAlleles + 255) / 256), dim3(256), 0, st, (const uint64_t *)dAlleleOff, (const uint32_t *)dAlleleLen, (const uint8_t *)dHasN,
+                       (const uint32_t *)dSepStart, nAlleles, cntMore, sepMore, (T1kAlleleRec *)dAlleleRec);
+  }
   void *dBasesT = nullptr, *dBlockT = nullptr;
   {
     static const bool on = [] { const char *e = getenv("T1K_REF_TRANSPOSE"); return !e || atoi(e) != 0; }();
@@ -337,7 +358,7 @@
   r.alleleOff = (const uint64_t *)dAlleleOff; r.alleleLen = (const uint32_t *)dAlleleLen; r.alleleHasN = (const uint8_t *)dHasN;
   r.anyN = 0;
   for (uint8_t h : alleleHasN) r.anyN |= h;
-  r.sepStart = (const uint32_t *)dSepStart; r.sepPos = (const int32_t *)dSepPos;
+  r.sepStart = (const uint32_t *)dSepStart; r.sepPos = (const int32_t *)dSepPos; r.alleleRec = (const T1kAlleleRec *)dAlleleRec;
   r.kStart = (const uint32_t *)dKStart; r.kHas = (const uint32_t *)dHas; r.kMulti = (const uint32_t *)dMulti; r.kHasPre = (const uint32_t *)dHasPre;
   r.kDirIdx = (const uint32_t *)dDirIdx; r.kDir = (const uint32_t *)dDir; r.kDirStride = stride;
   r.kDirMask = (const unsigned long long *)dDirMask; r.kDirMaskWords = maskWords;
```

Measured after the change: 4.125 million (median of 2 runs). No clear change (+0.4%).
